# borangundogan/PPO-2DGrid

Measured on AMD Instinct MI355X. Metric: env-steps/sec (rollout+GAE+PPO update), 4096 envs, 16x16 mediumhard, higher is better.
Workload: dtype fp32

## Files before the change

include/merlin_hip.h:

```cpp
#ifndef MERLIN_HIP_H
#define MERLIN_HIP_H

#include <stdint.h>

#ifdef __cplusplus
extern "C" {
#endif

#define MERLIN_ABI_VERSION 3

#define MERLIN_OK 0
#define MERLIN_E_INVALID 1
#define MERLIN_E_HIP 2
#define MERLIN_E_DEVICE 3
#define MERLIN_E_UNSUPPORTED 4

#define MERLIN_EASY 0
#define MERLIN_MEDIUM 1
#define MERLIN_MEDIUMHARD 2
#define MERLIN_HARD 3
#define MERLIN_HARDEST 4

#define MERLIN_DEVERR_BAD_ACTION 1u
#define MERLIN_DEVERR_PLACE_OBJ 2u
// ... 114 lines not shown
int merlin_tower_conv2_lut_fwd(const uint32_t *codes_dev, const int64_t *index_dev, int64_t n,
                               const float *tables_dev, int32_t towers, float *Z2_dev,
                               void *stream);
int merlin_tower_conv2_lut_bwd(const uint32_t *codes_dev, int64_t n, const float *dZ2c_dev,
                               const uint32_t *absmax_dev, int32_t towers, float *dtables_dev,
                               void *stream);
int merlin_tower_conv2_lut_fwd_grouped(const uint32_t *codes_dev, int64_t n, int64_t group_frames,
                                       const float *tables_dev, int32_t towers, float *Z2_dev, void *stream);
int64_t merlin_tower_conv2_lut_slab_bytes(int32_t towers, int64_t group_frames);
int merlin_tower_conv2_lut_bwd_grouped(const uint32_t *codes_dev, int64_t group_frames, const float *dZ2c_dev,
                                       const uint32_t *absmax_dev, int32_t towers, float *dtables_dev,
                                       void *slabs_dev, void *stream);

int merlin_tower_window_lut(const int32_t *rows_dev, int64_t n_windows, const float *tables_dev,
                            int32_t towers, float *Z2w_dev, void *stream);
int merlin_minibatch_patch_maps(const int32_t *kid_dev, const int64_t *group_keys_dev, int64_t n_groups,
                                int64_t n_frames, const int64_t *group_offsets_dev, int32_t n_patches, int32_t *kmap_dev,
                                int32_t *rmap_dev, int32_t *rep_row_dev, void *stream);
int merlin_tower_window_lut_bias_relu(const int32_t *rows_dev, int64_t n_windows, const float *tables_dev,
                                      int32_t towers, const float *b2_dev, float *a2w_dev, void *stream);
int merlin_tower_window_conv3(const float *Q_dev, int64_t n_windows, const int32_t *wid_dev,
                              const int64_t *groups_dev, int64_t n, const float *b3_dev,
                              int32_t towers, float *Y3_dev, void *stream);
int64_t merlin_tower_all_windows(void);
int merlin_tower_codes_conv3(const uint32_t *codes_dev, int64_t n, const float *Qall_dev,
                             const float *b3_dev, int32_t towers, float *Y3_dev, void *stream);
int merlin_tower_codes_conv3_amax(const uint32_t *codes_dev, int64_t n, const float *Qall_dev,
                                  const float *b3_dev, int32_t towers, float *Y3_dev, uint32_t *amax_dev,
                                  void *stream);
int merlin_tower_errors(uint32_t *flags, void *stream);
int merlin_tower_window_conv3_bits(const float *Q_dev, int64_t n_windows, const int32_t *wid_dev,
                                   const int64_t *groups_dev, int64_t n, const float *b3_dev,
                                   int32_t towers, float *Y3_dev, uint64_t *relu_bits_dev, uint32_t *amax_dev,
                                   void *stream);
int merlin_tower_window_conv3_reuse(const float *Q_dev, int64_t n_windows, const int32_t *wid_dev,
                                    const int64_t *groups_dev, int64_t n, const float *b3_dev,
                                    int32_t towers, float *Y3_dev, uint64_t *relu_bits_dev, uint32_t *amax_dev,
                                    const int32_t *rep_row_dev, int32_t copy, void *stream);
int merlin_tower_window_conv3_planes(const float *Q_dev, int64_t nw, const int32_t *wid_dev, const int64_t *groups_dev,
                                     int64_t n, const float *b3_dev, int32_t towers, void *Y3_planes_dev,
                                     uint64_t *relu_bits_dev, const int32_t *rep_row_dev, uint32_t *colmax_ws_dev,
                                     uint32_t *bound_dev, void *stream);
int merlin_segment_sum(const float *src_dev, int64_t src_rows, const int32_t *idx_dev,
                       const int32_t *key_dev, int64_t nnz, const int32_t *slot_dev, int32_t sub,
                       int64_t item_len, const int32_t *fix_dev, int64_t n_fix, int32_t towers,
                       float *out_dev, int64_t out_rows, float *carry_dev, int32_t accumulate,
                       void *stream);
#define MERLIN_SEG_ACCUMULATE 1
#define MERLIN_SEG_NO_FILL 2
#define MERLIN_SEG_MASK_BITS 4
#define MERLIN_SEG_ROLE_SHIFT 8
#define MERLIN_SEG_ROLE_MASK (7 << MERLIN_SEG_ROLE_SHIFT)
int merlin_segment_sum_masked(const float *src_dev, const void *mask_dev, int64_t src_rows,
                              const int32_t *idx_dev, const int32_t *key_dev, int64_t nnz,
                              const int32_t *slot_dev, int32_t sub, int64_t item_len,
                              const int32_t *fix_dev, int64_t n_fix, int32_t towers, float *out_dev,
                              int64_t out_rows, float *carry_dev, int32_t flags, void *stream);
int merlin_segment_sum_marked(const float *src_dev, const void *mask_dev, int64_t src_rows,
                              const int32_t *idx_dev, const int32_t *key_dev, int64_t nnz,
                              const int32_t *slot_dev, int32_t sub, int64_t item_len,
                              const int32_t *fix_dev, int64_t n_fix, int32_t towers, float *out_dev,
                              int64_t out_rows, float *carry_dev, int32_t flags, int32_t *mark_dev,
                              void *stream);
int merlin_segment_sum_fused(const float *src_dev, const void *mask_dev, int64_t src_rows,
                             const int32_t *idx_dev, const int32_t *key_dev, int64_t nnz,
                             const int32_t *slot_dev, int32_t sub, int64_t item_len,
                             const int32_t *fix_dev, int64_t n_fix, int32_t towers, float *out_dev,
                             int64_t out_rows, float *carry_dev, int32_t flags, int32_t *mark_dev,
                             const int32_t *head_fix_dev, int32_t *counters_dev, void *stream);
int merlin_segment_sum_mask_rows(const float *src_dev, const void *mask_dev, int64_t src_rows, const int32_t *idx_dev,
                                 const int32_t *key_dev, int64_t nnz, const int32_t *slot_dev, int32_t sub,
                                 int64_t item_len, const int32_t *fix_dev, int64_t n_fix, int32_t towers, float *out_dev,
                                 int64_t out_rows, float *carry_dev, int32_t flags, int32_t *mark_dev,
                                 const int32_t *head_fix_dev, int32_t *counters_dev, const int32_t *mask_rows_dev,
                                 void *stream);

int merlin_act_heads(const float *z_dev, const float *b4_dev, int64_t n, int32_t hidden,
                     const float *w_actor_dev, const float *b_actor_dev, const float *w_critic_dev,
                     const float *b_critic_dev, int32_t act_dim, int32_t deterministic, uint64_t seed,
                     const int64_t *epoch_dev, int64_t step, int64_t env_offset, int64_t *action_dev,
                     float *logp_dev,
                     float *value_dev, void *stream);

int64_t merlin_ppo_loss_workspace(int64_t n_samples);
int merlin_ppo_loss(const float *logits_dev, const float *value_dev, const float *bias_actor_dev,
                    const float *bias_critic_dev, int64_t n_frames, int32_t act_dim, const int32_t *offs_dev,
                    const int32_t *order_dev, const int64_t *frame_of_dev, int64_t n_samples,
                    const int64_t *sample_index_dev, const int64_t *actions_dev, const float *logp_old_dev,
                    const float *adv_dev, const float *ret_dev, double clip_eps, double vf_coef, double ent_coef,
                    float *dlogits_dev, float *dvalue_dev, float *dbias_actor_dev, float *dbias_critic_dev,
                    float *loss_dev, double *stats_dev, double *workspace_dev, void *stream);
int merlin_ppo_loss_absmax(const float *logits_dev, const float *value_dev, const float *bias_actor_dev,
                           const float *bias_critic_dev, int64_t n_frames, int32_t act_dim, const int32_t *offs_dev,
                           const int32_t *order_dev, const int64_t *frame_of_dev, int64_t n_samples,
                           const int64_t *sample_index_dev, const int64_t *actions_dev, const float *logp_old_dev,
                           const float *adv_dev, const float *ret_dev, double clip_eps, double vf_coef,
                           double ent_coef, float *dlogits_dev, float *dvalue_dev, float *dbias_actor_dev,
                           float *dbias_critic_dev, float *loss_dev, double *stats_dev, double *workspace_dev,
                           uint32_t *grad_absmax_dev, void *stream);

int merlin_tower_bias_relu(float *z_dev, const float *bias_dev, int64_t rows, int32_t cols, int32_t towers,
                           void *stream);
int merlin_tower_relu_bwd(const float *y_dev, const float *dy_dev, float *dz_dev, int64_t rows, int32_t cols,
                          int32_t towers, float *dbias_dev, void *stream);
int merlin_tower_colsum(const float *x_dev, int64_t rows, int32_t cols, int64_t row_stride, int64_t tower_stride,
                        int32_t towers, float *out_dev, void *stream);
int merlin_tower_head_bwd(const float *h_dev, const float *dlogits_dev, const float *dvalue_dev,
                          const float *w_actor_dev, const float *w_critic_dev, int64_t n, int32_t hidden,
                          int32_t act_dim, float *dz_dev, float *dbias_dev, float *dw_actor_dev,
                          float *dw_critic_dev, uint32_t *amax_dev, void *stream);
int merlin_tower_head_bwd_planes(const float *h_dev, const float *dlogits_dev, const float *dvalue_dev,
                                 const float *w_actor_dev, const float *w_critic_dev, int64_t n, int32_t hidden,
                                 int32_t act_dim, void *dz_planes_dev, float *dbias_dev, float *dw_actor_dev,
                                 float *dw_critic_dev, const uint32_t *grad_absmax_dev, uint32_t *dz_bound_dev,
                                 void *stream);
int merlin_tower_heads_fwd(const float *h_dev, int64_t n, int32_t hidden, const float *w_actor_dev,
                           int32_t act_dim, const float *w_critic_dev, const float *b_actor_dev,
                           const float *b_critic_dev, float *logits_dev, float *value_dev, void *stream);

int merlin_x6_split(const float *x_dev, int64_t n, void *planes_dev, void *stream);
int merlin_x6_join(const void *planes_dev, int64_t n, float *x_dev, void *stream);
int merlin_x6_gemm_nt(const float *A_dev, const void *B_dev, int64_t M, int32_t N, int32_t K, int32_t towers,
                      int64_t a_stride, int64_t b_stride, const float *bias_dev, float *C_dev, int64_t c_stride,
                      int32_t cfg, void *stream);
int64_t merlin_x6_tn_slab_floats(int32_t M, int32_t N, int32_t towers, int32_t splits);
int merlin_x6_gemm_tn(const float *A_dev, const float *B_dev, int64_t Kd, int32_t M, int32_t N, int32_t towers,
                      int64_t a_stride, int64_t b_stride, int32_t splits, float *slab_dev, float *out_dev, int32_t cfg,
                      void *stream);

int merlin_h3_amax(const float *x_dev, int64_t n, int32_t towers, int64_t stride, uint32_t *amax_dev, void *stream);
int merlin_h3_split(const float *x_dev, int64_t n, int32_t towers, const uint32_t *amax_dev, void *planes_dev,
                    void *stream);
int merlin_h3_gemm_nt(const float *A_dev, const uint32_t *amax_a_dev, const void *B_dev, const uint32_t *amax_b_dev,
                      int64_t M, int32_t N, int32_t K, int32_t towers, int64_t a_stride, int64_t b_stride,
                      const float *bias_dev, float *C_dev, int64_t c_stride, void *a_planes_dev, int32_t cfg,
                      void *stream);
int merlin_h3_gemm_tn(const float *A_dev, const uint32_t *amax_a_dev, const float *B_dev, const uint32_t *amax_b_dev,
                      int64_t Kd, int32_t M, int32_t N, int32_t towers, int64_t a_stride, int64_t b_stride,
                      int32_t splits, float *slab_dev, float *out_dev, int32_t cfg, void *stream);
int merlin_h3_gemm_tn_planes(const void *A_planes_dev, const uint32_t *amax_a_dev, const void *B_planes_dev,
                             const uint32_t *amax_b_dev, int64_t Kd, int32_t M, int32_t N, int32_t towers,
                             int64_t a_stride, int64_t b_stride, int32_t splits, float *slab_dev, float *out_dev,
                             int32_t cfg, void *stream);
int merlin_h3_gemm_nt_gather(const float *A_dev, const uint32_t *amax_a_dev, const void *B_dev,
                             const uint32_t *amax_b_dev, int64_t M, int32_t N, int32_t K, int32_t towers,
                             int64_t a_stride, int64_t b_stride, const float *bias_dev, float *C_dev, int64_t c_stride,
                             const int32_t *a_rows_dev, int32_t cfg, void *stream);
int merlin_h3_gemm_nt_heads(const float *A_dev, const uint32_t *amax_a_dev, const void *B_dev,
                            const uint32_t *amax_b_dev, int64_t M, int32_t N, int32_t K, int64_t a_stride,
                            int64_t b_stride, const float *bias_dev, float *C_dev, int64_t c_stride,
                            const int32_t *a_rows_dev, const float *head_w0_dev, int32_t n_actions,
                            const float *head_w1_dev, float *head_partials_dev, int32_t cfg, void *stream);
int32_t merlin_h3_heads_parts(int32_t N, int32_t cfg);
int merlin_h3_gemm_nt_planes(const void *A_planes_dev, const uint32_t *amax_a_dev, const void *B_dev,
                             const uint32_t *amax_b_dev, int64_t M, int32_t N, int32_t K, int32_t towers,
                             int64_t a_stride, int64_t b_stride, const float *bias_dev, float *C_dev, int64_t c_stride,
                             int32_t cfg, void *stream);
int merlin_h3_gemm_nt_heads_planes(const void *A_planes_dev, const uint32_t *amax_a_dev, const void *B_dev,
                                   const uint32_t *amax_b_dev, int64_t M, int32_t N, int32_t K, int64_t a_stride,
                                   int64_t b_stride, const float *bias_dev, float *C_dev, int64_t c_stride,
                                   const int32_t *a_rows_dev, const float *head_w0_dev, int32_t n_actions,
                                   const float *head_w1_dev, float *head_partials_dev, int32_t cfg, void *stream);
int merlin_h3_gemm_tn_gather_planes(const void *A_planes_dev, const uint32_t *amax_a_dev, const void *B_planes_dev,
                                    const uint32_t *amax_b_dev, int64_t Kd, int32_t M, int32_t N, int32_t towers,
                                    int64_t a_stride, int64_t b_stride, int32_t splits, float *slab_dev,
                                    float *out_dev, const int32_t *b_rows_dev, int32_t cfg, void *stream);
int merlin_h3_gemm_tn_gather_planes_a(const void *A_planes_dev, const uint32_t *amax_a_dev, const float *B_dev,
                                      const uint32_t *amax_b_dev, int64_t Kd, int32_t M, int32_t N, int32_t towers,
                                      int64_t a_stride, int64_t b_stride, int32_t splits, float *slab_dev,
                                      float *out_dev, const int32_t *b_rows_dev, int32_t cfg, void *stream);
int merlin_act_draw(const float *partials_dev, int32_t parts, int64_t n, const float *b_actor_dev,
                    const float *b_critic_dev, int32_t n_actions, int32_t deterministic, uint64_t seed,
                    const int64_t *epoch_dev, int64_t step, int64_t env_offset, int64_t *action_dev, float *logp_dev,
                    float *value_dev, void *stream);
int merlin_heads_combine(const float *partials_dev, int32_t parts, int64_t M, int32_t n_actions, float *logits_dev,
                         float *value_dev, void *stream);
int merlin_h3_gemm_tn_gather(const float *A_dev, const uint32_t *amax_a_dev, const float *B_dev,
                             const uint32_t *amax_b_dev, int64_t Kd, int32_t M, int32_t N, int32_t towers,
                             int64_t a_stride, int64_t b_stride, int32_t splits, float *slab_dev, float *out_dev,
                             const int32_t *b_rows_dev, int32_t cfg, void *stream);

int merlin_window_gemm_fwd(const float *a2w_dev, const float *W3r_dev, int32_t towers, int64_t nw, float *Q_dev,
                           void *stream);
int64_t merlin_window_gemm_bwd_work(int32_t towers, int64_t nw);
int merlin_window_gemm_bwd(const float *a2w_dev, const float *dQ_dev, const float *W3r_dev, int32_t towers, int64_t nw,
                           float *da2w_dev, float *db2_dev, float *dW3r_dev, float *db3_dev, float *work_dev,
                           int64_t work_floats, void *stream);
int merlin_stage_tables_fwd(const float *W1_dev, const float *b1_dev, const float *W2_dev, const float *atlas_dev,
                            const int16_t *idx_dev, int32_t towers, float *HT_dev, float *T2_dev, void *stream);
int merlin_stage_tables_bwd(const float *W2_dev, const float *HT_dev, const float *dT2_dev, const float *atlas_dev,
                            const int16_t *koff_dev, const int16_t *kv_dev, int32_t towers, float *dH_dev,
                            float *dW1_dev, float *db1_dev, float *dW2_dev, void *stream);

int64_t merlin_clip_adam_workspace(int32_t n_tensors, const int64_t *numel);
int merlin_clip_adam(int32_t n_tensors, float *const *params, float *const *grads, float *const *exp_avg,
                     float *const *exp_avg_sq, float *const *steps, const int64_t *numel, double lr, double beta1,
                     double beta2, double eps, float max_norm, float *norm_out, double *workspace, void *stream);

int64_t merlin_group_clip_sgd_workspace(int32_t n_tensors, const int64_t *numel, int32_t G);
int merlin_group_clip_sgd(int32_t n_tensors, float *const *params, float *const *grads, const int64_t *numel,
                          int32_t G, float lr, float max_norm, float *norm_out, double *workspace, void *stream);

int merlin_episode_loss(const float *reward_dev, const float *value_dev, const float *new_logp_dev,
                        const float *new_value_dev, const int32_t *length_dev, int32_t T, int32_t n, double gamma,
                        double lam, float *workspace_dev, float *loss_dev, void *stream);

int merlin_episode_class_stats(const float *done_dev, const double *ep_return_dev, const int32_t *ep_length_dev,
                               const uint8_t *class_dev, int32_t T, int32_t N, int32_t n_classes,
                               double *out_dev, int32_t accumulate, void *stream);

#ifdef __cplusplus
}
#endif
#endif
```

ppo-2dgrid_amd/csrc/merlin_capi.hip:

```cpp
#include <math.h>
#include <string.h>

#include <mutex>
#include <string>
#include <vector>

#include <algorithm>

#include "merlin_internal.h"

struct merlin_env {
    merlin::EnvDev dev;
    int device;
    bool has_state;
    int steps_since_refill;
    int refill_every;
    bool no_fallback = false;
    bool seed_slots_full = false;
    uint8_t *diff_buf = nullptr;
};

namespace {

thread_local std::string g_err;
// ... 1111 lines not shown
    return MERLIN_OK;
}

int merlin_tower_heads_fwd(const float *h, int64_t n, int32_t hidden, const float *w_actor, int32_t act_dim,
                           const float *w_critic, const float *b_actor, const float *b_critic, float *logits,
                           float *value, void *stream) {
    if ((!h || !w_actor || !w_critic || !logits || !value) && n > 0) return fail(MERLIN_E_INVALID, "null argument");
    if (n < 0) return fail(MERLIN_E_INVALID, "n must be >= 0");
    if (act_dim < 1 || act_dim > merlin::epilogue_max_act()) return fail(MERLIN_E_UNSUPPORTED, "act_dim must be 1..8");
    if (hidden != 512) return fail(MERLIN_E_UNSUPPORTED, "hidden must be 512");
    HIP_TRY(merlin::launch_heads_fwd(h, n, hidden, w_actor, act_dim, w_critic, b_actor, b_critic, logits, value,
                                     (hipStream_t)stream));
    return MERLIN_OK;
}

int merlin_x6_split(const float *x, int64_t n, void *planes, void *stream) {
    if ((!x || !planes) && n > 0) return fail(MERLIN_E_INVALID, "null argument");
    if (n < 0 || n % 8) return fail(MERLIN_E_INVALID, "n must be a non-negative multiple of 8");
    HIP_TRY(merlin::launch_x6_split(x, n, planes, (hipStream_t)stream));
    return MERLIN_OK;
}

int merlin_stage_tables_fwd(const float *W1, const float *b1, const float *W2, const float *atlas, const int16_t *idx,
                            int32_t towers, float *HT, float *T2, void *stream) {
    if (!W1 || !b1 || !W2 || !atlas || !idx || !HT || !T2) return fail(MERLIN_E_INVALID, "null argument");
    if (towers < 1 || towers > 2) return fail(MERLIN_E_INVALID, "towers must be 1 or 2");
    HIP_TRY(merlin::launch_stage_fwd(W1, b1, W2, atlas, idx, towers, HT, T2, (hipStream_t)stream));
    return MERLIN_OK;
}

int merlin_stage_tables_bwd(const float *W2, const float *HT, const float *dT2, const float *atlas,
                            const int16_t *koff, const int16_t *kv, int32_t towers, float *dH, float *dW1, float *db1,
                            float *dW2, void *stream) {
    if (!W2 || !HT || !dT2 || !atlas || !koff || !kv || !dH || !dW1 || !db1 || !dW2)
        return fail(MERLIN_E_INVALID, "null argument");
    if (towers < 1 || towers > 2) return fail(MERLIN_E_INVALID, "towers must be 1 or 2");
    DeviceWs *ws = nullptr;
    int rc = device_ws(&ws);
    if (rc != MERLIN_OK) return rc;
    HIP_TRY(merlin::launch_stage_bwd(W2, HT, dT2, atlas, koff, kv, towers, dH, dW1, db1, dW2, ws->stage_part,
                                     (hipStream_t)stream));
    return MERLIN_OK;
}

int merlin_window_gemm_fwd(const float *a2w, const float *W3r, int32_t towers, int64_t nw, float *Q, void *stream) {
    if (!a2w || !W3r || !Q) return fail(MERLIN_E_INVALID, "null argument");
    if (towers < 1 || towers > 2) return fail(MERLIN_E_INVALID, "towers must be 1 or 2");
    if (nw < 0) return fail(MERLIN_E_INVALID, "nw must be >= 0");
    HIP_TRY(merlin::launch_winfwd(a2w, W3r, towers, nw, Q, (hipStream_t)stream));
    return MERLIN_OK;
}

int64_t merlin_window_gemm_bwd_work(int32_t towers, int64_t nw) {
    if (towers < 1 || towers > 2 || nw <= 0) return -1;
    return merlin::winbwd_work_floats(towers, nw);
}

int merlin_window_gemm_bwd(const float *a2w, const float *dQ, const float *W3r, int32_t towers, int64_t nw,
                           float *da2w, float *db2, float *dW3r, float *db3, float *work, int64_t work_floats,
                           void *stream) {
    if (!a2w || !dQ || !W3r || !da2w || !db2 || !dW3r || !work) return fail(MERLIN_E_INVALID, "null argument");
    if (towers < 1 || towers > 2) return fail(MERLIN_E_INVALID, "towers must be 1 or 2");
    if (nw <= 0) return fail(MERLIN_E_INVALID, "nw must be > 0");
    if (work_floats < merlin::winbwd_work_floats(towers, nw)) return fail(MERLIN_E_INVALID, "work too small");
    HIP_TRY(merlin::launch_winbwd(a2w, dQ, W3r, towers, nw, da2w, db2, dW3r, work, (hipStream_t)stream, db3));
    return MERLIN_OK;
}

int merlin_x6_join(const void *planes, int64_t n, float *x, void *stream) {
    if ((!x || !planes) && n > 0) return fail(MERLIN_E_INVALID, "null argument");
    if (n < 0 || n % 8) return fail(MERLIN_E_INVALID, "n must be a non-negative multiple of 8");
    HIP_TRY(merlin::launch_x6_join(planes, n, x, (hipStream_t)stream));
    return MERLIN_OK;
}

int merlin_x6_gemm_nt(const float *A, const void *B, int64_t M, int32_t N, int32_t K, int32_t towers, int64_t a_stride,
                      int64_t b_stride, const float *bias, float *C, int64_t c_stride, int32_t cfg, void *stream) {
    if (M < 0 || N <= 0 || K <= 0) return fail(MERLIN_E_INVALID, "bad shape");
    if (M > 0 && (!A || !B || !C)) return fail(MERLIN_E_INVALID, "null argument");
    if (K % 32) return fail(MERLIN_E_UNSUPPORTED, "K must be a multiple of 32");
    if (towers < 1 || towers > 2) return fail(MERLIN_E_INVALID, "towers must be 1 or 2");
    if (a_stride % 4 || b_stride % 8) return fail(MERLIN_E_INVALID, "tower strides: A multiple of 4, B of 8");
    const hipError_t e = merlin::launch_x6_gemm_nt(A, B, M, N, K, towers, a_stride, b_stride, bias, C, c_stride, cfg,
                                                   (hipStream_t)stream);
    if (e == hipErrorInvalidValue) return fail(MERLIN_E_UNSUPPORTED, "N not a multiple of the tile width / bad cfg");
    HIP_TRY(e);
    return MERLIN_OK;
}

int64_t merlin_x6_tn_slab_floats(int32_t M, int32_t N, int32_t towers, int32_t splits) {
    return (int64_t)std::max(1, splits) * towers * M * N;
}

int merlin_x6_gemm_tn(const float *A, const float *B, int64_t Kd, int32_t M, int32_t N, int32_t towers, int64_t a_stride,
                      int64_t b_stride, int32_t splits, float *slab, float *out, int32_t cfg, void *stream) {
    if (Kd < 0 || M <= 0 || N <= 0) return fail(MERLIN_E_INVALID, "bad shape");
    if (!out || (Kd > 0 && (!A || !B || !slab))) return fail(MERLIN_E_INVALID, "null argument");
    if (towers < 1 || towers > 2) return fail(MERLIN_E_INVALID, "towers must be 1 or 2");
    if (splits < 1 || splits > merlin::x6_tn_max_splits()) return fail(MERLIN_E_INVALID, "splits out of range");
    if (M % 8 || N % 8 || a_stride % 4 || b_stride % 4) return fail(MERLIN_E_INVALID, "M, N: multiples of 8");
    const hipError_t e = merlin::launch_x6_gemm_tn(A, B, Kd, M, N, towers, a_stride, b_stride, splits, slab, out, cfg,
                                                   (hipStream_t)stream);
    if (e == hipErrorInvalidValue) return fail(MERLIN_E_UNSUPPORTED, "M / N not multiples of the tile / bad cfg");
    HIP_TRY(e);
    return MERLIN_OK;
}

int merlin_h3_amax(const float *x, int64_t n, int32_t towers, int64_t stride, uint32_t *amax, void *stream) {
    if (!amax || (n > 0 && !x)) return fail(MERLIN_E_INVALID, "null argument");
    if (towers < 1 || (n > 0 && towers > 2) || towers > (1 << 20))
        return fail(MERLIN_E_INVALID, "towers must be 1 or 2");
    if (n < 0 || n % 4 || stride % 4 || (towers > 1 && stride < n)) return fail(MERLIN_E_INVALID, "n, stride: multiples of 4");
    HIP_TRY(merlin::launch_h3_amax(x, n, towers, stride, amax, (hipStream_t)stream));
    return MERLIN_OK;
}

int merlin_h3_split(const float *x, int64_t n, int32_t towers, const uint32_t *amax, void *planes, void *stream) {
    if ((!x || !planes || !amax) && n > 0) return fail(MERLIN_E_INVALID, "null argument");
    if (towers < 1 || towers > 2) return fail(MERLIN_E_INVALID, "towers must be 1 or 2");
    if (n < 0 || n % 8) return fail(MERLIN_E_INVALID, "n must be a non-negative multiple of 8");
    HIP_TRY(merlin::launch_h3_split(x, n, towers, amax, planes, (hipStream_t)stream));
    return MERLIN_OK;
}

static int h3_gemm_nt(const float *A, const uint32_t *amax_a, const void *B, const uint32_t *amax_b, int64_t M,
                      int32_t N, int32_t K, int32_t towers, int64_t a_stride, int64_t b_stride, const float *bias,
                      float *C, int64_t c_stride, void *a_planes, const int32_t *a_rows, int32_t cfg, void *stream,
                      const float *head_w0 = nullptr, int32_t n_actions = 0, const float *head_w1 = nullptr,
                      float *head_part = nullptr, bool a_is_planes = false) {
    if (M < 0 || N <= 0 || K <= 0) return fail(MERLIN_E_INVALID, "bad shape");
    if (M > 0 && (!A || !B || (!C && !head_part) || !amax_a || !amax_b)) return fail(MERLIN_E_INVALID, "null argument");
    if (K % 32) return fail(MERLIN_E_UNSUPPORTED, "K must be a multiple of 32");
    if (towers < 1 || towers > 2) return fail(MERLIN_E_INVALID, "towers must be 1 or 2");
    if (a_stride % 4 || b_stride % 8) return fail(MERLIN_E_INVALID, "tower strides: A multiple of 4, B of 8");
    const hipError_t e = merlin::launch_h3_gemm_nt(A, amax_a, B, amax_b, M, N, K, towers, a_stride, b_stride, bias, C,
                                                   c_stride, a_planes, cfg, (hipStream_t)stream, a_rows, head_w0,
                                                   n_actions, head_w1, head_part, a_is_planes);
    if (e == hipErrorInvalidValue)
        return fail(MERLIN_E_UNSUPPORTED, "N not a multiple of the tile width / bad cfg / unsupported gather");
    HIP_TRY(e);
    return MERLIN_OK;
}

int merlin_h3_gemm_nt(const float *A, const uint32_t *amax_a, const void *B, const uint32_t *amax_b, int64_t M,
                      int32_t N, int32_t K, int32_t towers, int64_t a_stride, int64_t b_stride, const float *bias,
                      float *C, int64_t c_stride, void *a_planes, int32_t cfg, void *stream) {
    return h3_gemm_nt(A, amax_a, B, amax_b, M, N, K, towers, a_stride, b_stride, bias, C, c_stride, a_planes, nullptr,
                      cfg, stream);
}

int merlin_h3_gemm_nt_planes(const void *A_planes, const uint32_t *amax_a, const void *B, const uint32_t *amax_b,
                             int64_t M, int32_t N, int32_t K, int32_t towers, int64_t a_stride, int64_t b_stride,
                             const float *bias, float *C, int64_t c_stride, int32_t cfg, void *stream) {
    if (cfg < 60 || cfg >= 70) return fail(MERLIN_E_UNSUPPORTED, "plane-operand cfgs are 60..69");
    return h3_gemm_nt(static_cast<const float *>(A_planes), amax_a, B, amax_b, M, N, K, towers, a_stride, b_stride,
                      bias, C, c_stride, nullptr, nullptr, cfg, stream);
}

int merlin_h3_gemm_nt_gather(const float *A, const uint32_t *amax_a, const void *B, const uint32_t *amax_b, int64_t M,
                             int32_t N, int32_t K, int32_t towers, int64_t a_stride, int64_t b_stride,
                             const float *bias, float *C, int64_t c_stride, const int32_t *a_rows, int32_t cfg,
                             void *stream) {
    if (M > 0 && !a_rows) return fail(MERLIN_E_INVALID, "null argument");
    if (K % 64) return fail(MERLIN_E_UNSUPPORTED, "gathered rows: K must be a multiple of 64");
    return h3_gemm_nt(A, amax_a, B, amax_b, M, N, K, towers, a_stride, b_stride, bias, C, c_stride, nullptr, a_rows,
                      cfg, stream);
}

static int h3_gemm_tn(const void *A, const uint32_t *amax_a, const void *B, const uint32_t *amax_b, int64_t Kd,
                      int32_t M, int32_t N, int32_t towers, int64_t a_stride, int64_t b_stride, int32_t splits,
                      float *slab, float *out, bool planes, int32_t cfg, void *stream, const int32_t *b_rows = nullptr,
                      bool a_planes = false, bool b_planes = false) {
    if (Kd < 0 || M <= 0 || N <= 0) return fail(MERLIN_E_INVALID, "bad shape");
    if (!out || (Kd > 0 && (!A || !B || !slab || !amax_a || !amax_b))) return fail(MERLIN_E_INVALID, "null argument");
    if (towers < 1 || towers > 2) return fail(MERLIN_E_INVALID, "towers must be 1 or 2");
    if (splits < 1 || splits > merlin::x6_tn_max_splits()) return fail(MERLIN_E_INVALID, "splits out of range");
    if (M % 8 || N % 8 || a_stride % 4 || b_stride % 4) return fail(MERLIN_E_INVALID, "M, N: multiples of 8");
    const hipError_t e = merlin::launch_h3_gemm_tn(A, amax_a, B, amax_b, Kd, M, N, towers, a_stride, b_stride, splits,
                                                   slab, out, planes, cfg, (hipStream_t)stream, b_rows, a_planes,
                                                   b_planes);
    if (e == hipErrorInvalidValue) return fail(MERLIN_E_UNSUPPORTED, "M / N not multiples of the tile / bad cfg");
    HIP_TRY(e);
    return MERLIN_OK;
}

int merlin_h3_gemm_tn(const float *A, const uint32_t *amax_a, const float *B, const uint32_t *amax_b, int64_t Kd,
                      int32_t M, int32_t N, int32_t towers, int64_t a_stride, int64_t b_stride, int32_t splits,
                      float *slab, float *out, int32_t cfg, void *stream) {
    return h3_gemm_tn(A, amax_a, B, amax_b, Kd, M, N, towers, a_stride, b_stride, splits, slab, out, false, cfg,
                      stream);
}

int merlin_h3_gemm_nt_heads(const float *A, const uint32_t *amax_a, const void *B, const uint32_t *amax_b, int64_t M,
                            int32_t N, int32_t K, int64_t a_stride, int64_t b_stride, const float *bias, float *C,
                            int64_t c_stride, const int32_t *a_rows, const float *head_w0, int32_t n_actions,
                            const float *head_w1, float *head_partials, int32_t cfg, void *stream) {
    if (M > 0 && (!bias || !head_w0 || !head_w1 || !head_partials)) return fail(MERLIN_E_INVALID, "null argument");
    if (n_actions < 1 || n_actions > 4) return fail(MERLIN_E_UNSUPPORTED, "heads epilogue: 1..4 actions");
    if (merlin::h3_heads_parts(N, cfg) == 0) return fail(MERLIN_E_UNSUPPORTED, "heads epilogue: cfg 10, 12 or 13");
    if (a_rows && K % 64) return fail(MERLIN_E_UNSUPPORTED, "gathered rows: K must be a multiple of 64");
    return h3_gemm_nt(A, amax_a, B, amax_b, M, N, K, 2, a_stride, b_stride, bias, C, c_stride, nullptr, a_rows, cfg,
                      stream, head_w0, n_actions, head_w1, head_partials);
}

int32_t merlin_h3_heads_parts(int32_t N, int32_t cfg) { return merlin::h3_heads_parts(N, cfg); }

int merlin_act_draw(const float *partials, int32_t parts, int64_t n, const float *b_actor, const float *b_critic,
                    int32_t n_actions, int32_t deterministic, uint64_t seed, const int64_t *epoch, int64_t step,
                    int64_t env_offset, int64_t *action, float *logp, float *value, void *stream) {
    if (n < 0 || parts < 1 || n_actions < 1 || n_actions > 4) return fail(MERLIN_E_INVALID, "bad shape");
    if (n > 0 && (!partials || !b_actor || !b_critic || !action || !logp || !value))
        return fail(MERLIN_E_INVALID, "null argument");
    HIP_TRY(merlin::launch_act_draw(partials, parts, n, b_actor, b_critic, n_actions, deterministic, seed, epoch, step,
                                    env_offset, action, logp, value, (hipStream_t)stream));
    return MERLIN_OK;
}

int merlin_heads_combine(const float *partials, int32_t parts, int64_t M, int32_t n_actions, float *logits,
                         float *value, void *stream) {
    if (M < 0 || parts < 1 || n_actions < 1 || n_actions > 4) return fail(MERLIN_E_INVALID, "bad shape");
    if (M > 0 && (!partials || !logits || !value)) return fail(MERLIN_E_INVALID, "null argument");
    HIP_TRY(merlin::launch_heads_combine(partials, parts, M, n_actions, logits, value, (hipStream_t)stream));
    return MERLIN_OK;
}

int merlin_h3_gemm_tn_gather(const float *A, const uint32_t *amax_a, const float *B, const uint32_t *amax_b, int64_t Kd,
                             int32_t M, int32_t N, int32_t towers, int64_t a_stride, int64_t b_stride, int32_t splits,
                             float *slab, float *out, const int32_t *b_rows, int32_t cfg, void *stream) {
    if (Kd > 0 && !b_rows) return fail(MERLIN_E_INVALID, "null argument");
    if (N % 64) return fail(MERLIN_E_UNSUPPORTED, "gathered rows: N must be a multiple of 64");
    return h3_gemm_tn(A, amax_a, B, amax_b, Kd, M, N, towers, a_stride, b_stride, splits, slab, out, false, cfg, stream,
                      b_rows);
}

int merlin_h3_gemm_nt_heads_planes(const void *A_planes, const uint32_t *amax_a, const void *B,
                                   const uint32_t *amax_b, int64_t M, int32_t N, int32_t K, int64_t a_stride,
                                   int64_t b_stride, const float *bias, float *C, int64_t c_stride,
                                   const int32_t *a_rows, const float *head_w0, int32_t n_actions,
                                   const float *head_w1, float *head_partials, int32_t cfg, void *stream) {
    if (M > 0 && (!bias || !C || !a_rows || (head_partials && (!head_w0 || !head_w1))))
        return fail(MERLIN_E_INVALID, "null argument");
    if (head_partials && (n_actions < 1 || n_actions > 4))
        return fail(MERLIN_E_UNSUPPORTED, "heads epilogue: 1..4 actions");
    if (merlin::h3_heads_parts(N, cfg) == 0) return fail(MERLIN_E_UNSUPPORTED, "planes forward: cfg 10, 12 or 13");
    if (K % 64) return fail(MERLIN_E_UNSUPPORTED, "gathered rows: K must be a multiple of 64");
    return h3_gemm_nt(static_cast<const float *>(A_planes), amax_a, B, amax_b, M, N, K, 2, a_stride, b_stride, bias,
                      C, c_stride, nullptr, a_rows, cfg, stream, head_w0, n_actions, head_w1, head_partials, true);
}

int merlin_h3_gemm_tn_gather_planes(const void *A_planes, const uint32_t *amax_a, const void *B_planes,
                                    const uint32_t *amax_b, int64_t Kd, int32_t M, int32_t N, int32_t towers,
                                    int64_t a_stride, int64_t b_stride, int32_t splits, float *slab, float *out,
                                    const int32_t *b_rows, int32_t cfg, void *stream) {
    if (Kd > 0 && !b_rows) return fail(MERLIN_E_INVALID, "null argument");
    if (N % 64) return fail(MERLIN_E_UNSUPPORTED, "gathered rows: N must be a multiple of 64");
    return h3_gemm_tn(A_planes, amax_a, B_planes, amax_b, Kd, M, N, towers, a_stride, b_stride, splits, slab, out,
                      false, cfg, stream, b_rows, true, true);
}

int merlin_h3_gemm_tn_gather_planes_a(const void *A_planes, const uint32_t *amax_a, const float *B,
                                      const uint32_t *amax_b, int64_t Kd, int32_t M, int32_t N, int32_t towers,
                                      int64_t a_stride, int64_t b_stride, int32_t splits, float *slab, float *out,
                                      const int32_t *b_rows, int32_t cfg, void *stream) {
    if (Kd > 0 && !b_rows) return fail(MERLIN_E_INVALID, "null argument");
    if (N % 64) return fail(MERLIN_E_UNSUPPORTED, "gathered rows: N must be a multiple of 64");
    return h3_gemm_tn(A_planes, amax_a, B, amax_b, Kd, M, N, towers, a_stride, b_stride, splits, slab, out, false, cfg,
                      stream, b_rows, true);
}

int merlin_h3_gemm_tn_planes(const void *A, const uint32_t *amax_a, const void *B, const uint32_t *amax_b, int64_t Kd,
                             int32_t M, int32_t N, int32_t towers, int64_t a_stride, int64_t b_stride, int32_t splits,
                             float *slab, float *out, int32_t cfg, void *stream) {
    return h3_gemm_tn(A, amax_a, B, amax_b, Kd, M, N, towers, a_stride, b_stride, splits, slab, out, true, cfg,
                      stream);
}

int64_t merlin_clip_adam_workspace(int32_t n_tensors, const int64_t *numel) {
    if (n_tensors < 0 || n_tensors > merlin::OPT_MAX_TENSORS || (n_tensors > 0 && !numel)) return -1;
    return std::max<int64_t>(1, merlin::opt_blocks(n_tensors, numel));
}

int merlin_clip_adam(int32_t n_tensors, float *const *params, float *const *grads, float *const *exp_avg,
                     float *const *exp_avg_sq, float *const *steps, const int64_t *numel, double lr, double beta1,
                     double beta2, double eps, float max_norm, float *norm_out, double *workspace, void *stream) {
    if (n_tensors < 1 || n_tensors > merlin::OPT_MAX_TENSORS)
        return fail(MERLIN_E_INVALID, "n_tensors must be in [1, 32]");
    if (!params || !grads || !exp_avg || !exp_avg_sq || !steps || !numel || !workspace)
        return fail(MERLIN_E_INVALID, "null argument");
    int64_t blocks = 0;
    for (int i = 0; i < n_tensors; i++) {
        if (numel[i] <= 0) return fail(MERLIN_E_INVALID, "every tensor needs numel > 0");
        if (!params[i] || !grads[i] || !exp_avg[i] || !exp_avg_sq[i] || !steps[i])
            return fail(MERLIN_E_INVALID, "null tensor pointer");
    }
    blocks = merlin::opt_blocks(n_tensors, numel);
    if (blocks > INT32_MAX / 2) return fail(MERLIN_E_INVALID, "too many elements");
    HIP_TRY(merlin::launch_clip_adam(n_tensors, params, grads, exp_avg, exp_avg_sq, steps, numel, lr, beta1, beta2, eps,
                                     max_norm, norm_out, workspace, (hipStream_t)stream));
    return MERLIN_OK;
}

int64_t merlin_group_clip_sgd_workspace(int32_t n_tensors, const int64_t *numel, int32_t G) {
    if (n_tensors < 0 || n_tensors > merlin::OPT_MAX_TENSORS || G < 0 || (n_tensors > 0 && !numel)) return -1;
    for (int i = 0; i < n_tensors; i++)
        if (numel[i] <= 0) return -1;
    return std::max<int64_t>(1, merlin::group_blocks(n_tensors, numel) * (int64_t)G);
}

int merlin_group_clip_sgd(int32_t n_tensors, float *const *params, float *const *grads, const int64_t *numel,
                          int32_t G, float lr, float max_norm, float *norm_out, double *workspace, void *stream) {
    if (n_tensors < 0 || n_tensors > merlin::OPT_MAX_TENSORS)
        return fail(MERLIN_E_INVALID, "n_tensors must be in [0, 32]");
    if (G < 0 || G > 65535) return fail(MERLIN_E_INVALID, "G must be in [0, 65535]");
    if (n_tensors == 0 || G == 0) return MERLIN_OK;
    if (!params || !grads || !numel || !workspace) return fail(MERLIN_E_INVALID, "null argument");
    for (int i = 0; i < n_tensors; i++) {
        if (numel[i] <= 0) return fail(MERLIN_E_INVALID, "every tensor needs numel > 0");
        if (!params[i] || !grads[i]) return fail(MERLIN_E_INVALID, "null tensor pointer");
    }
    if (merlin::group_blocks(n_tensors, numel) > INT32_MAX / 2) return fail(MERLIN_E_INVALID, "too many elements");
    HIP_TRY(merlin::launch_group_clip_sgd(n_tensors, params, grads, numel, G, lr, max_norm, norm_out, workspace,
                                          (hipStream_t)stream));
    return MERLIN_OK;
}

int merlin_episode_loss(const float *reward, const float *value, const float *new_logp, const float *new_value,
                        const int32_t *length, int32_t T, int32_t n, double gamma, double lam, float *workspace,
                        float *loss, void *stream) {
    if (T < 1 || n < 0) return fail(MERLIN_E_INVALID, "episode_loss needs T >= 1 and n >= 0");
    if (n == 0) return MERLIN_OK;
    if (!reward || !value || !new_logp || !new_value || !length || !workspace || !loss)
        return fail(MERLIN_E_INVALID, "null argument");
    HIP_TRY(merlin::launch_episode_loss(reward, value, new_logp, new_value, length, T, n, gamma, lam, workspace, loss,
                                        (hipStream_t)stream));
    return MERLIN_OK;
}

int merlin_episode_class_stats(const float *done, const double *ep_return, const int32_t *ep_length,
                               const uint8_t *cls, int32_t T, int32_t N, int32_t n_classes, double *out,
                               int32_t accumulate, void *stream) {
    if (T < 0 || N < 0) return fail(MERLIN_E_INVALID, "episode_class_stats needs T >= 0 and N >= 0");
    if (n_classes < 1 || n_classes > merlin::EPS_MAX_CLASSES)
        return fail(MERLIN_E_INVALID, "episode_class_stats needs n_classes in [1, 8]");
    if (!out) return fail(MERLIN_E_INVALID, "null argument");
    if (T > 0 && N > 0 && (!done || !ep_return || !ep_length || !cls)) return fail(MERLIN_E_INVALID, "null argument");
    DeviceWs *ws = nullptr;
    int rc = device_ws(&ws);
    if (rc) return rc;
    HIP_TRY(merlin::launch_episode_class_stats(done, ep_return, ep_length, cls, T, N, n_classes, out, accumulate,
                                               ws->eps_part, (hipStream_t)stream));
    return MERLIN_OK;
}

}
```

ppo-2dgrid_amd/csrc/merlin_h3.hip:

```cpp
#include <algorithm>

#include "merlin_internal.h"

namespace merlin {
namespace {

typedef _Float16 f16x8 __attribute__((ext_vector_type(8)));
typedef _Float16 f16x2 __attribute__((ext_vector_type(2)));
typedef __bf16 bf16x4 __attribute__((ext_vector_type(4)));
typedef __bf16 bf16x8 __attribute__((ext_vector_type(8)));
typedef float f32x16 __attribute__((ext_vector_type(16)));
typedef uint32_t u32x4 __attribute__((ext_vector_type(4)));
typedef __attribute__((address_space(3))) bf16x4 lds_bf16x4;
typedef __attribute__((address_space(3))) char lds_char;

constexpr int BK = 32;
constexpr float LO_INV = 1.0f / 2048.0f;

__device__ __forceinline__ f32x16 mfma16(const u32x4 a, const u32x4 b, f32x16 c) {
    return __builtin_amdgcn_mfma_f32_32x32x16_f16(__builtin_bit_cast(f16x8, a), __builtin_bit_cast(f16x8, b), c, 0, 0,
                                                   0);
}

__device__ __forceinline__ float relu_nan(float v) { return v != v ? v : fmaxf(v, 0.0f); }
// ... 1295 lines not shown
    if (hd.part) {
        if constexpr (!PIPE || BN / WGN != 64) {
            return hipErrorInvalidValue;
        } else {
            if (!bias || T != 2 || Pout || hd.na < 1 || hd.na > 4 || !hd.w0 || !hd.w1) return hipErrorInvalidValue;
            if (amap) {
                if (K % 64 || K > 64 * GA_CHUNKS || !C) return hipErrorInvalidValue;
                hipLaunchKernelGGL((k_h3_ntpg<BM, BN, WGM, WGN, 2>), grid, block, 0, s, A, B, amaxA, amaxB, M, N, K,
                                   sA, sB, bias, C, sC, tiles_n, amap, hd);
            } else if (C) {
                hipLaunchKernelGGL((k_h3_ntp<BM, BN, WGM, WGN, 2>), grid, block, 0, s, A, B, amaxA, amaxB, M, N, K, sA,
                                   sB, bias, C, sC, tiles_n, nullptr, hd);
            } else {
                hipLaunchKernelGGL((k_h3_ntp<BM, BN, WGM, WGN, 3>), grid, block, 0, s, A, B, amaxA, amaxB, M, N, K, sA,
                                   sB, bias, nullptr, sC, tiles_n, nullptr, hd);
            }
            return hipGetLastError();
        }
    }
    if (amap) {
        if (!PIPE || Pout || K % 64 || K > 64 * GA_CHUNKS) return hipErrorInvalidValue;
        if (bias)
            hipLaunchKernelGGL((k_h3_ntpg<BM, BN, WGM, WGN, 1>), grid, block, 0, s, A, B, amaxA, amaxB, M, N, K, sA,
                               sB, bias, C, sC, tiles_n, amap, hd);
        else
            hipLaunchKernelGGL((k_h3_ntpg<BM, BN, WGM, WGN, 0>), grid, block, 0, s, A, B, amaxA, amaxB, M, N, K, sA,
                               sB, nullptr, C, sC, tiles_n, amap, hd);
        return hipGetLastError();
    }
    if (PIPE) {
        if (bias)
            hipLaunchKernelGGL((k_h3_ntp<BM, BN, WGM, WGN, 1>), grid, block, 0, s, A, B, amaxA, amaxB, M, N, K, sA, sB,
                               bias, C, sC, tiles_n, Pout, hd);
        else
            hipLaunchKernelGGL((k_h3_ntp<BM, BN, WGM, WGN, 0>), grid, block, 0, s, A, B, amaxA, amaxB, M, N, K, sA, sB,
                               nullptr, C, sC, tiles_n, Pout, hd);
    } else {
        if (bias)
            hipLaunchKernelGGL((k_h3_nt<BM, BN, WGM, WGN, 1>), grid, block, 0, s, A, B, amaxA, amaxB, M, N, K, sA, sB,
                               bias, C, sC, tiles_n, Pout);
        else
            hipLaunchKernelGGL((k_h3_nt<BM, BN, WGM, WGN, 0>), grid, block, 0, s, A, B, amaxA, amaxB, M, N, K, sA, sB,
                               nullptr, C, sC, tiles_n, Pout);
    }
    return hipGetLastError();
}

template <int BM, int BN, int WGM, int WGN, bool KP>
hipError_t ntg_launch(const float *A, const u32x4 *B, const uint32_t *amaxA, const uint32_t *amaxB, int64_t M, int N,
                      int K, int T, int64_t sA, int64_t sB, const float *bias, float *C, int64_t sC, u32x4 *Pout,
                      hipStream_t s) {
    if (N % BN || Pout) return hipErrorInvalidValue;
    if ((int64_t)N * (K / 8) * 2 > INT32_MAX) return hipErrorInvalidValue;
    const int64_t tiles_m = (M + BM - 1) / BM;
    const int tiles_n = N / BN;
    if (tiles_m * tiles_n > INT32_MAX) return hipErrorInvalidValue;
    const dim3 grid((unsigned)(tiles_m * tiles_n), T), block(64 * WGM * WGN);
    if (bias)
        hipLaunchKernelGGL((k_h3_ntg<BM, BN, WGM, WGN, 1, KP>), grid, block, 0, s, A, B, amaxA, amaxB, M, N, K, sA, sB,
                           bias, C, sC, tiles_n);
    else
        hipLaunchKernelGGL((k_h3_ntg<BM, BN, WGM, WGN, 0, KP>), grid, block, 0, s, A, B, amaxA, amaxB, M, N, K, sA, sB,
                           nullptr, C, sC, tiles_n);
    return hipGetLastError();
}

template <int BM, int BN, int WGM, int WGN, int Q>
hipError_t tn_launch(const void *A, const void *B, const uint32_t *amaxA, const uint32_t *amaxB, int64_t Kd, int M,
                     int N, int T, int64_t sA, int64_t sB, int splits, float *slab, int *S_out, const int32_t *bmap,
                     hipStream_t s) {
    if (M % BM || N % BN) return hipErrorInvalidValue;
    if (bmap && ((Q != 0 && Q != 3 && Q != 4) || N % 64)) return hipErrorInvalidValue;
    if (Q >= 3 && !bmap) return hipErrorInvalidValue;
    const int tiles_n = N / BN, tiles = (M / BM) * tiles_n;
    int S = std::max(1, splits);
    int64_t kc = (Kd + S - 1) / S;
    kc = (kc + BK - 1) / BK * BK;
    S = (int)std::max<int64_t>(1, (Kd + kc - 1) / kc);
    *S_out = S;
    if (Q == 1)
        hipLaunchKernelGGL((k_h3_tnq<BM, BN, WGM, WGN>), dim3(tiles * S * T), dim3(64 * WGM * WGN), 0, s,
                           static_cast<const u32x4 *>(A), static_cast<const u32x4 *>(B), amaxA, amaxB, Kd, M, N,
                           sA / 4, sB / 4, kc, tiles_n, tiles, S, slab);
    else if (Q == 2)
        hipLaunchKernelGGL((k_h3_tnp<BM, BN, WGM, WGN>), dim3(tiles * S * T), dim3(64 * WGM * WGN), 0, s,
                           static_cast<const float4 *>(A), static_cast<const float4 *>(B), amaxA, amaxB, Kd, M, N,
                           sA / 4, sB / 4, kc, tiles_n, tiles, S, slab);
    else if (Q == 4)
        hipLaunchKernelGGL((k_h3_tng<BM, BN, WGM, WGN, true, true>), dim3(tiles * S * T), dim3(64 * WGM * WGN), 0, s,
                           static_cast<const float4 *>(A), static_cast<const float4 *>(B), amaxA, amaxB, Kd, M, N,
                           sA / 4, sB / 4, kc, tiles_n, tiles, S, slab, bmap);
    else if (Q == 3)
        hipLaunchKernelGGL((k_h3_tng<BM, BN, WGM, WGN, true>), dim3(tiles * S * T), dim3(64 * WGM * WGN), 0, s,
                           static_cast<const float4 *>(A), static_cast<const float4 *>(B), amaxA, amaxB, Kd, M, N,
                           sA / 4, sB / 4, kc, tiles_n, tiles, S, slab, bmap);
    else if (bmap)
        hipLaunchKernelGGL((k_h3_tng<BM, BN, WGM, WGN>), dim3(tiles * S * T), dim3(64 * WGM * WGN), 0, s,
                           static_cast<const float4 *>(A), static_cast<const float4 *>(B), amaxA, amaxB, Kd, M, N,
                           sA / 4, sB / 4, kc, tiles_n, tiles, S, slab, bmap);
    else
        hipLaunchKernelGGL((k_h3_tn<BM, BN, WGM, WGN>), dim3(tiles * S * T), dim3(64 * WGM * WGN), 0, s,
                           static_cast<const float4 *>(A), static_cast<const float4 *>(B), amaxA, amaxB, Kd, M, N,
                           sA / 4, sB / 4, kc, tiles_n, tiles, S, slab);
    return hipGetLastError();
}

__global__ void k_h3_fill0(float4 *__restrict__ out, int64_t n4) {
    for (int64_t e = (int64_t)blockIdx.x * 256 + threadIdx.x; e < n4; e += (int64_t)gridDim.x * 256)
        out[e] = make_float4(0.0f, 0.0f, 0.0f, 0.0f);
}

}

hipError_t launch_h3_amax(const float *x, int64_t n, int T, int64_t stride, uint32_t *amax, hipStream_t s) {
    hipLaunchKernelGGL(k_h3_zero, dim3((T + 63) / 64), dim3(64), 0, s, amax, T);
    hipError_t e = hipGetLastError();
    if (e != hipSuccess || n <= 0) return e;
    if (n % 4 || stride % 4) return hipErrorInvalidValue;
    const int64_t n4 = n / 4;
    const int grid = (int)std::min<int64_t>((n4 + 255) / 256, 1024);
    hipLaunchKernelGGL(k_h3_amax, dim3(grid, T), dim3(256), 0, s, reinterpret_cast<const float4 *>(x), n4, stride / 4,
                       amax);
    return hipGetLastError();
}

hipError_t launch_h3_split(const float *x, int64_t n, int T, const uint32_t *amax, void *planes, hipStream_t s) {
    if (n % 8) return hipErrorInvalidValue;
    if (n <= 0) return hipSuccess;
    const int64_t g8 = n / 8;
    const int grid = (int)std::min<int64_t>((g8 + 255) / 256, 2048);
    hipLaunchKernelGGL(k_h3_split, dim3(grid, T), dim3(256), 0, s, reinterpret_cast<const float4 *>(x), g8, amax,
                       static_cast<u32x4 *>(planes));
    return hipGetLastError();
}

hipError_t launch_h3_gemm_nt(const float *A, const uint32_t *amaxA, const void *B, const uint32_t *amaxB, int64_t M,
                             int N, int K, int T, int64_t a_stride, int64_t b_stride, const float *bias, float *C,
                             int64_t c_stride, void *a_planes, int cfg, hipStream_t s, const int32_t *a_rows,
                             const float *head_w0, int n_actions, const float *head_w1, float *head_part,
                             bool a_is_planes) {
    const HeadsArg hd{head_w0, head_w1, n_actions, head_part};
    if (M <= 0) return hipSuccess;
    if (K % BK || N <= 0 || a_stride % 4 || b_stride % 8) return hipErrorInvalidValue;
    const u32x4 *b = static_cast<const u32x4 *>(B);
    u32x4 *P = static_cast<u32x4 *>(a_planes);
    const int64_t sB = b_stride / 8 * 2;
#define H3_NT(BM, BN, WM, WN, PIPE) \
    nt_launch<BM, BN, WM, WN, PIPE>(A, b, amaxA, amaxB, M, N, K, T, a_stride, sB, bias, C, c_stride, P, a_rows, hd, s, \
                                    a_is_planes)
#define H3_NTG(BM, BN, WM, WN, KP)                         \
    ((a_rows || head_part) ? hipErrorInvalidValue          \
                           : ntg_launch<BM, BN, WM, WN, KP>(A, b, amaxA, amaxB, M, N, K, T, a_stride, sB, bias, C, \
                                                            c_stride, P, s))
    if (a_is_planes && (cfg < 10 || cfg > 14) && cfg != 60) return hipErrorInvalidValue;
    if (cfg >= 60 && cfg < 70) {
        if (P || ((a_rows || head_part) && !a_is_planes)) return hipErrorInvalidValue;
        return launch_h3p_gemm_nt(A, amaxA, B, amaxB, M, N, K, T, a_stride, b_stride, bias, C, c_stride, cfg, s, a_rows,
                                  head_w0, n_actions, head_w1, head_part);
    }
    switch (cfg) {
        case 0: return H3_NT(256, 128, 4, 2, false);
        case 1: return H3_NT(128, 192, 4, 2, false);
        case 2: return H3_NT(128, 128, 2, 2, false);
        case 3: return H3_NT(128, 256, 2, 4, false);
        case 5: return H3_NT(128, 64, 4, 1, false);
        case 10: return H3_NT(256, 128, 4, 2, true);
        case 11: return H3_NT(128, 192, 4, 2, true);
        case 12: return H3_NT(128, 128, 2, 2, true);
        case 13: return H3_NT(128, 256, 2, 4, true);
        case 14: return H3_NT(64, 128, 2, 2, true);
        case 20: return H3_NTG(256, 128, 4, 2, false);
        case 21: return H3_NTG(128, 192, 4, 2, false);
        case 30: return H3_NTG(256, 128, 4, 2, true);
        case 31: return H3_NTG(128, 192, 4, 2, true);
        default: return hipErrorInvalidValue;
    }
#undef H3_NT
#undef H3_NTG
}

hipError_t launch_h3_gemm_tn(const void *A, const uint32_t *amaxA, const void *B, const uint32_t *amaxB, int64_t Kd,
                             int M, int N, int T, int64_t a_stride, int64_t b_stride, int splits, float *slab,
                             float *out, bool planes, int cfg, hipStream_t s, const int32_t *b_rows, bool a_planes,
                             bool b_planes) {
    if (b_planes && !a_planes) return hipErrorInvalidValue;
    if (M <= 0 || N <= 0) return hipSuccess;
    if (M % 8 || N % 8 || a_stride % 4 || b_stride % 4) return hipErrorInvalidValue;
    const int64_t total = (int64_t)T * M * N;
    if (Kd <= 0) {
        hipLaunchKernelGGL(k_h3_fill0, dim3((unsigned)std::min<int64_t>((total / 4 + 255) / 256, 2048)), dim3(256),
                           0, s, reinterpret_cast<float4 *>(out), total / 4);
        return hipGetLastError();
    }
    int S = 1;
    hipError_t e;
    if (cfg == 20 || cfg == 21) {
        if (!(a_planes && b_planes)) return hipErrorInvalidValue;
        e = launch_h3p_gemm_tn_gather(A, amaxA, B, amaxB, Kd, M, N, T, a_stride, b_stride, splits, slab, b_rows, cfg,
                                      &S, s);
        if (e != hipSuccess) return e;
        return launch_x6_fold(slab, S, total, out, s);
    }
#define H3_TN(BM, BN, WM, WN, PIPE)                                                                              \
    (planes ? tn_launch<BM, BN, WM, WN, 1>(A, B, amaxA, amaxB, Kd, M, N, T, a_stride, b_stride, splits, slab, &S,   \
                                           b_rows, s)                                                              \
     : a_planes ? (b_planes ? tn_launch<BM, BN, WM, WN, 4>(A, B, amaxA, amaxB, Kd, M, N, T, a_stride, b_stride,    \
                                                           splits, slab, &S, b_rows, s)                            \
                           : tn_launch<BM, BN, WM, WN, 3>(A, B, amaxA, amaxB, Kd, M, N, T, a_stride, b_stride,    \
                                                          splits, slab, &S, b_rows, s))                            \
            : tn_launch<BM, BN, WM, WN, PIPE>(A, B, amaxA, amaxB, Kd, M, N, T, a_stride, b_stride, splits, slab, &S, \
                                              b_rows, s))
    switch (cfg) {
        case 0: e = H3_TN(128, 192, 4, 2, 0); break;
        case 1: e = H3_TN(128, 192, 2, 2, 0); break;
        case 2: e = H3_TN(64, 192, 2, 2, 0); break;
        case 10: e = H3_TN(128, 192, 4, 2, 2); break;
        case 11: e = H3_TN(128, 192, 2, 2, 2); break;
        default: return hipErrorInvalidValue;
    }
#undef H3_TN
    if (e != hipSuccess) return e;
    return launch_x6_fold(slab, S, total, out, s);
}

namespace {
__global__ __launch_bounds__(256) void k_heads_combine(const float4 *__restrict__ part, int P, int64_t M, int na,
                                                       float *__restrict__ logits, float *__restrict__ value) {
    const int64_t r = (int64_t)blockIdx.x * 256 + threadIdx.x;
    if (r >= M) return;
    float4 a = part[r], v = part[(int64_t)P * M + r];
    for (int p = 1; p < P; p++) {
        const float4 x = part[(int64_t)p * M + r], y = part[(int64_t)(P + p) * M + r];
        a.x += x.x;
        a.y += x.y;
        a.z += x.z;
        a.w += x.w;
        v.x += y.x;
    }
    const float av[4] = {a.x, a.y, a.z, a.w};
    for (int o = 0; o < na; o++) logits[r * na + o] = av[o];
    value[r] = v.x;
}
}

int h3_heads_parts(int N, int cfg) {
    switch (cfg) {
        case 10: return N % 128 ? 0 : N / 128 * 2;
        case 12: return N % 128 ? 0 : N / 128 * 2;
        case 13: return N % 256 ? 0 : N / 256 * 4;
        case 14: return N % 128 ? 0 : N / 128 * 2;
        case 60: return N % 256 ? 0 : N / 256 * 4;
        default: return 0;
    }
}

hipError_t launch_heads_combine(const float *part, int P, int64_t M, int na, float *logits, float *value,
                                hipStream_t s) {
    if (M <= 0) return hipSuccess;
    if (P < 1 || na < 1 || na > 4) return hipErrorInvalidValue;
    hipLaunchKernelGGL(k_heads_combine, dim3((unsigned)((M + 255) / 256)), dim3(256), 0, s,
                       reinterpret_cast<const float4 *>(part), P, M, na, logits, value);
    return hipGetLastError();
}

}
```

ppo-2dgrid_amd/csrc/merlin_h3p.hip:

```cpp
#include <algorithm>
#include <type_traits>

#include "merlin_internal.h"

namespace merlin {
namespace {

typedef _Float16 p_f16x8 __attribute__((ext_vector_type(8)));
typedef float p_f32x16 __attribute__((ext_vector_type(16)));
typedef uint32_t p_u32x4 __attribute__((ext_vector_type(4)));

constexpr float P_LO_INV = 1.0f / 2048.0f;

__device__ __forceinline__ p_f32x16 p_mfma(const p_u32x4 a, const p_u32x4 b, p_f32x16 c) {
    return __builtin_amdgcn_mfma_f32_32x32x16_f16(__builtin_bit_cast(p_f16x8, a), __builtin_bit_cast(p_f16x8, b), c, 0,
                                                   0, 0);
}
__device__ __forceinline__ float p_relu(float v) { return v != v ? v : fmaxf(v, 0.0f); }
__device__ __forceinline__ int p_xcd_tile(int b, int nb) {
    const int xcd = b & 7, q = nb >> 3, r = nb & 7;
    return (xcd < r ? xcd * (q + 1) : r * (q + 1) + (xcd - r) * q) + (b >> 3);
}
__device__ __forceinline__ int p_exp(uint32_t amax) {
    if (amax == 0u) return 0;
    const int e = (int)((amax >> 23) & 0xffu) - 127;
    return std::min(std::max(14 - e, -120), 115);
}
__device__ __forceinline__ float p_pow2(int e) { return __uint_as_float((uint32_t)(e + 127) << 23); }
__device__ __forceinline__ uint32_t p_amax(const uint32_t *p) {
    return __hip_atomic_load(p, __ATOMIC_RELAXED, __HIP_MEMORY_SCOPE_AGENT);
}
__device__ __forceinline__ int p_swz(int r) { return (r >> 1) & 7; }
__device__ __forceinline__ p_u32x4 p_unscale(const p_u32x4 x) {
    return __builtin_bit_cast(p_u32x4, __builtin_bit_cast(p_f16x8, x) * (_Float16)(1.0f / 2048.0f));
}

template <int V>
using IC = std::integral_constant<int, V>;
template <int N, int I = 0, class F>
__device__ __forceinline__ void static_for(F &&f) {
    if constexpr (I < N) {
        f(IC<I>{});
        static_for<N, I + 1>(f);
    }
}

typedef __attribute__((address_space(3))) p_u32x4 lds_u32x4;
__device__ __forceinline__ void lds_rd(p_u32x4 &d, uint32_t addr) { d = *(const lds_u32x4 *)(uintptr_t)addr; }

template <int BM, int BN, int WGM, int WGN, int EPI, int NK, int NS = 3, bool ONE = false, int ORD = 0>
__global__ __launch_bounds__(64 * WGM * WGN) void k_h3_pq(const p_u32x4 *__restrict__ A, const p_u32x4 *__restrict__ B,
                                                          const uint32_t *__restrict__ amaxA,
                                                          const uint32_t *__restrict__ amaxB, int64_t M, int N, int K,
                                                          int64_t sA, int64_t sB, const float *__restrict__ bias,
                                                          float *__restrict__ C, int64_t sC, int tiles_n) {
    constexpr int NT = 64 * WGM * WGN;
    constexpr int WTM = BM / WGM, WTN = BN / WGN;
    constexpr int TM = WTM / 32, TN = WTN / 32;
    constexpr int NR = 2 * (TM + TN), NM = 3 * TM * TN;
    static_assert(NM >= NR, "a read behind every MFMA");
    constexpr int G = (BM + BN) * 8 / NT;
    static_assert((BM * 8) % NT == 0 && (BN * 8) % NT == 0, "whole DMA instructions per thread");
    constexpr int STG = (BM + BN) * 8;
    constexpr uint32_t STG_B = STG * 16;
    static_assert(NS >= 2 && NS <= 4, "ring depth");
    __shared__ p_u32x4 lds[NS * STG];

    const int t = blockIdx.y;
    const int L = p_xcd_tile(blockIdx.x, gridDim.x);
    const int tm = L / tiles_n, tn = L - tm * tiles_n;
    const int64_t m0 = (int64_t)tm * BM;
    const int n0 = tn * BN;
    const int tid = threadIdx.x, lane = tid & 63, w = tid >> 6;
    const int wm = w / WGN, wn = w - (w / WGN) * WGN;
    const int64_t row_ch = K / 4;

    const int eA = p_exp(p_amax(amaxA + t)), eB = p_exp(p_amax(amaxB + t));
    const p_u32x4 *baseA = A + t * sA + m0 * row_ch, *baseB = B + t * sB + (int64_t)n0 * row_ch;
    uint32_t off[G];
#pragma unroll
    for (int i = 0; i < G; i++) {
        const int q = i * NT + tid, r = q >> 3, c = (q & 7) ^ p_swz(r);
        off[i] = r < BM ? (uint32_t)(std::min<int64_t>(r, M - 1 - m0) * row_ch + c) : (uint32_t)((r - BM) * row_ch + c);
    }
    typedef __attribute__((address_space(3))) void lds_void;
    typedef __attribute__((address_space(1))) void gbl_void;
    auto issue = [&](int kt, int st) __attribute__((always_inline)) {
        p_u32x4 *base = lds + st * STG + w * 64;
#pragma unroll
        for (int i = 0; i < G; i++) {
            const int q0 = i * NT;
            const p_u32x4 *b = (q0 >> 3) < BM ? baseA : baseB;
            __builtin_amdgcn_global_load_lds((gbl_void *)(b + off[i] + kt * 8), (lds_void *)(base + i * NT), 16, 0, 0);
        }
    };

    const int fr = lane & 31, fh = lane >> 5;
    const uint32_t lds0 = (uint32_t)(uintptr_t)(__attribute__((address_space(3))) p_u32x4 *)lds;
    uint32_t adA[2][2], adB[2][2];
    {
        const int ra = wm * WTM + fr, rb = BM + wn * WTN + fr;
#pragma unroll
        for (int kh = 0; kh < 2; kh++)
#pragma unroll
            for (int p = 0; p < 2; p++) {
                const int c = 2 * (2 * kh + fh) + p;
                adA[kh][p] = lds0 + (uint32_t)(ra * 8 + (c ^ p_swz(ra))) * 16u;
                adB[kh][p] = lds0 + (uint32_t)(rb * 8 + (c ^ p_swz(rb))) * 16u;
            }
    }
    struct Frag {
        p_u32x4 a[TM][2], b[TN][2];
    };
    p_f32x16 hi[TM][TN], lo[TM][TN];
#pragma unroll
    for (int i = 0; i < TM; i++)
#pragma unroll
        for (int j = 0; j < TN; j++) {
            hi[i][j] = p_f32x16{};
            lo[i][j] = p_f32x16{};
        }
    auto rd = [&](Frag &g, auto K_, uint32_t so, auto KH) __attribute__((always_inline)) {
        constexpr int k = decltype(K_)::value, kh = decltype(KH)::value;
        if constexpr (k < 2 * TM)
            lds_rd(g.a[k >> 1][k & 1], adA[kh][k & 1] + so + (k >> 1) * 32 * 128);
        else
            lds_rd(g.b[(k - 2 * TM) >> 1][k & 1], adB[kh][k & 1] + so + ((k - 2 * TM) >> 1) * 32 * 128);
    };
    auto mf = [&](const Frag &f, const Frag &u, auto M_) __attribute__((always_inline)) {
        constexpr int m = decltype(M_)::value, tl = ORD ? m % (TM * TN) : m / 3, pr = ORD ? m / (TM * TN) : m % 3;
        constexpr int i = tl / TN, j = tl % TN;
        if constexpr (ONE) {
            if constexpr (pr == 0)
                hi[i][j] = p_mfma(u.a[i][1], f.b[j][0], hi[i][j]);
            else if constexpr (pr == 1)
                hi[i][j] = p_mfma(f.a[i][0], u.b[j][1], hi[i][j]);
            else
                hi[i][j] = p_mfma(f.a[i][0], f.b[j][0], hi[i][j]);
        } else if constexpr (pr == 0)
            lo[i][j] = p_mfma(f.a[i][1], f.b[j][0], lo[i][j]);
        else if constexpr (pr == 1)
            lo[i][j] = p_mfma(f.a[i][0], f.b[j][1], lo[i][j]);
        else
            hi[i][j] = p_mfma(f.a[i][0], f.b[j][0], hi[i][j]);
    };
    auto half = [&](const Frag &f, Frag &g, uint32_t so, auto KH, auto READS) __attribute__((always_inline)) {
        Frag u;
        if constexpr (ONE) {
#pragma unroll
            for (int i = 0; i < TM; i++) u.a[i][1] = p_unscale(f.a[i][1]);
#pragma unroll
            for (int j = 0; j < TN; j++) u.b[j][1] = p_unscale(f.b[j][1]);
        }
        static_for<NM>([&](auto M_) __attribute__((always_inline)) {
            mf(f, u, M_);
            if constexpr (decltype(READS)::value && decltype(M_)::value < NR) rd(g, M_, so, KH);
        });
        if constexpr (decltype(READS)::value) {
            static_for<NR>([&](auto) __attribute__((always_inline)) {
                __builtin_amdgcn_sched_group_barrier(0x008, 1, 0);
                __builtin_amdgcn_sched_group_barrier(0x100, 1, 0);
            });
            if constexpr (NM > NR) __builtin_amdgcn_sched_group_barrier(0x008, NM - NR, 0);
        }
        __builtin_amdgcn_sched_barrier(0);
    };
    auto touch = [&](const Frag &f) __attribute__((always_inline)) {
#pragma unroll
        for (int i = 0; i < TM; i++) asm volatile("" ::"v"(f.a[i][0]), "v"(f.a[i][1]));
#pragma unroll
        for (int j = 0; j < TN; j++) asm volatile("" ::"v"(f.b[j][0]), "v"(f.b[j][1]));
    };

    static_assert(NK >= NS - 1, "the prologue's k steps");
    constexpr int D = NS - 1;
    static_for<D>([&](auto KT) __attribute__((always_inline)) { issue(decltype(KT)::value, decltype(KT)::value); });
    asm volatile("s_waitcnt vmcnt(%0)" ::"n"(G * (D - 1)) : "memory");
    __builtin_amdgcn_s_barrier();
    __builtin_amdgcn_sched_barrier(0);
    Frag f0, f1;
    static_for<NR>([&](auto K_) __attribute__((always_inline)) { rd(f0, K_, 0, IC<0>{}); });
    static_for<NK>([&](auto KT) __attribute__((always_inline)) {
        constexpr int kt = decltype(KT)::value, st = kt % NS, sn = (kt + 1) % NS;
        if constexpr (kt + D < NK) issue(kt + D, (kt + D) % NS);
        __builtin_amdgcn_sched_barrier(0);
        half(f0, f1, (uint32_t)st * STG_B, IC<1>{}, IC<1>{});
        if constexpr (kt + 1 < NK) {
            touch(f1);
            constexpr int later = (NK - 1 < kt + D ? NK - 1 : kt + D) - (kt + 1);
            asm volatile("s_waitcnt vmcnt(%0)" ::"n"(G * later) : "memory");
            __builtin_amdgcn_s_barrier();
            __builtin_amdgcn_sched_barrier(0);
            half(f1, f0, (uint32_t)sn * STG_B, IC<0>{}, IC<1>{});
        } else {
            half(f1, f0, 0u, IC<0>{}, IC<0>{});
        }
    });

    const float inv = p_pow2(-eA), invB = p_pow2(-eB);
    float *Ct = C + t * sC;
#pragma unroll
    for (int j = 0; j < TN; j++) {
        const int col = n0 + wn * WTN + j * 32 + fr;
        const float bv = EPI == 1 ? bias[(int64_t)t * N + col] : 0.0f;
#pragma unroll
        for (int i = 0; i < TM; i++) {
#pragma unroll
            for (int r = 0; r < 16; r++) {
                const int64_t row = m0 + wm * WTM + i * 32 + (r & 3) + 8 * (r >> 2) + 4 * fh;
                if (row < M) {
                    const float v = (ONE ? hi[i][j][r] : hi[i][j][r] + lo[i][j][r] * P_LO_INV) * inv * invB;
                    Ct[row * N + col] = EPI == 1 ? p_relu(v + bv) : v;
                }
            }
        }
    }
}

template <int BM, int BN, int WGM, int WGN, int NS = 3, bool ONE = false, int ORD = 0>
hipError_t pq_launch(const void *A, const void *B, const uint32_t *amaxA, const uint32_t *amaxB, int64_t M, int N,
                     int K, int T, int64_t sA, int64_t sB, const float *bias, float *C, int64_t sC, hipStream_t s) {
    if (N % BN || K % 32 || K < 64) return hipErrorInvalidValue;
    const int64_t tiles_m = (M + BM - 1) / BM;
    const int tiles_n = N / BN;
    if (tiles_m * tiles_n > INT32_MAX) return hipErrorInvalidValue;
    const dim3 grid((unsigned)(tiles_m * tiles_n), T), block(64 * WGM * WGN);
    const auto *a = static_cast<const p_u32x4 *>(A);
    const auto *b = static_cast<const p_u32x4 *>(B);
#define PQ_K(NK)                                                                                                   \
    do {                                                                                                           \
        if (bias)                                                                                                  \
            hipLaunchKernelGGL((k_h3_pq<BM, BN, WGM, WGN, 1, NK, NS, ONE, ORD>), grid, block, 0, s, a, b, amaxA, amaxB, M, N, K, \
                               sA / 4, sB / 4, bias, C, sC, tiles_n);                                              \
        else                                                                                                       \
            hipLaunchKernelGGL((k_h3_pq<BM, BN, WGM, WGN, 0, NK, NS, ONE, ORD>), grid, block, 0, s, a, b, amaxA, amaxB, M, N, K, \
                               sA / 4, sB / 4, nullptr, C, sC, tiles_n);                                           \
    } while (0)
    switch (K) {
        case 576: PQ_K(18); break;
        case 512: PQ_K(16); break;
        default: return hipErrorInvalidValue;
    }
#undef PQ_K
    return hipGetLastError();
}


__device__ uint4 p_zero16[1] = {{0u, 0u, 0u, 0u}};

__device__ __forceinline__ void p_dma16(const void *src, uint32_t lds) {
    uint32_t keep;
    asm volatile("s_mov_b32 %0, m0\n\ts_mov_b32 m0, %2\n\tglobal_load_lds_dwordx4 %1, off\n\ts_mov_b32 m0, %0"
                 : "=&s"(keep)
                 : "v"(src), "s"(lds)
                 : "memory");
}
__device__ __forceinline__ void p_dma4(const void *src, uint32_t lds) {
    uint32_t keep;
    asm volatile("s_mov_b32 %0, m0\n\ts_mov_b32 m0, %2\n\tglobal_load_lds_dword %1, off\n\ts_mov_b32 m0, %0"
                 : "=&s"(keep)
                 : "v"(src), "s"(lds)
                 : "memory");
}

template <int RC>
__device__ __forceinline__ int p_tr_swz(int row) {
    static_assert(RC % 16 == 0 || RC == 24 || RC == 8, "row chunks");
    return RC % 16 == 0 ? (row & 3) << 2 : ((row >> 1) & 1) << 2;
}
typedef __bf16 p_bf16x4 __attribute__((ext_vector_type(4)));
typedef __bf16 p_bf16x8 __attribute__((ext_vector_type(8)));
typedef __attribute__((address_space(3))) p_bf16x4 lds_p_bf16x4;
typedef __attribute__((address_space(3))) int32_t lds_i32;

template <int BM, int BN, int WGM, int WGN>
__global__ __launch_bounds__(64 * WGM * WGN) void k_h3_tq(const p_u32x4 *__restrict__ A, const p_u32x4 *__restrict__ B,
                                                          const uint32_t *__restrict__ amaxA,
                                                          const uint32_t *__restrict__ amaxB, int64_t Kd, int M,
                                                          int N, int64_t sA, int64_t sB, int64_t kc, int tiles_n,
                                                          int tiles, int S, float *__restrict__ slab,
                                                          const int32_t *__restrict__ bmap) {
    constexpr int NT = 64 * WGM * WGN, NW = NT / 64;
    constexpr int WTM = BM / WGM, WTN = BN / WGN;
    constexpr int TM = WTM / 32, TN = WTN / 32;
    constexpr int RCA = BM / 8, RCB = BN / 8;
    constexpr int PSA = 32 * RCA, PSB = 32 * RCB;
    constexpr int STG = 2 * (PSA + PSB);
    constexpr uint32_t STG_B = STG * 16;
    static_assert((2 * PSA) % NT == 0 && (2 * PSB) % NT == 0, "whole DMA instructions per operand");
    constexpr int GA = 2 * PSA / NT, GB = 2 * PSB / NT, G = GA + GB + 1;
    constexpr int JB = BN / 64;
    constexpr int XS = 64 * NW;
    static_assert(32 * JB <= XS, "index slot");
    constexpr int NF = 2 * (TM + TN);
    constexpr int NR = 2 * NF, NM = 3 * TM * TN;
    __shared__ p_u32x4 lds[3 * STG];
    __shared__ int32_t ixr[3 * XS];

    const int P = p_xcd_tile(blockIdx.x, gridDim.x);
    const int t = P / (S * tiles), s = (P / tiles) % S, Lt = P % tiles;
    const int tm = Lt / tiles_n, tn = Lt - tm * tiles_n;
    const int m0 = tm * BM, n0 = tn * BN;
    const int64_t k0 = (int64_t)s * kc, k1 = std::min<int64_t>(Kd, k0 + kc);
    const int eA = p_exp(p_amax(amaxA + t)), eB = p_exp(p_amax(amaxB + t));
    const int tid = threadIdx.x, lane = tid & 63, w = tid >> 6;
    const int wm = w / WGN, wn = w - (w / WGN) * WGN;
    const int nc = N / 64, j0 = n0 / 64;
    const int64_t rowA = M / 4;
    const p_u32x4 *At = A + t * sA, *Bt = B + t * sB;
    const uint32_t lds0 = (uint32_t)(uintptr_t)(__attribute__((address_space(3))) p_u32x4 *)lds;
    const uint32_t ix0 = (uint32_t)(uintptr_t)(__attribute__((address_space(3))) int32_t *)ixr;
    const uint32_t wbase = (uint32_t)__builtin_amdgcn_readfirstlane(w) * 64u;

    int ra[GA], rb[GB], xb[GB];
    uint32_t oa[GA], gp[GB];
#pragma unroll
    for (int i = 0; i < GA; i++) {
        const int q = i * NT + tid, p = q / PSA, rem = q - p * PSA, r = rem / RCA, cs = rem - r * RCA;
        const int c = cs ^ p_tr_swz<RCA>(r);
        ra[i] = r;
        oa[i] = (uint32_t)((m0 / 8 + c) * 2 + p);
    }
#pragma unroll
    for (int i = 0; i < GB; i++) {
        const int q = (GA + i) * NT + tid - 2 * PSA, p = q / PSB, rem = q - p * PSB, r = rem / RCB,
                  cs = rem - r * RCB;
        const int c = cs ^ p_tr_swz<RCB>(r), col = 8 * c;
        rb[i] = r;
        xb[i] = r * JB + (col >> 6);
        gp[i] = (uint32_t)(((col & 63) >> 3) * 2 + p);
    }
    const int xr = tid / JB, xj = j0 + tid % JB;
    const int64_t nk = (k1 - k0 + 31) / 32, nk3 = (nk + 2) / 3 * 3;

    auto issue_ix = [&](int64_t kt, int slot) __attribute__((always_inline)) {
        const int64_t row = std::min<int64_t>(k0 + kt * 32 + (tid < 32 * JB ? xr : 0), k1 - 1);
        p_dma4(bmap + row * nc + (tid < 32 * JB ? xj : j0), ix0 + (uint32_t)(slot * XS) * 4u + wbase * 4u);
    };
    auto read_ix = [&](int slot, int32_t (&x)[GB]) __attribute__((always_inline)) {
        const lds_i32 *xs = (const lds_i32 *)(uintptr_t)(ix0 + (uint32_t)(slot * XS) * 4u);
#pragma unroll
        for (int i = 0; i < GB; i++) x[i] = xs[xb[i]];
    };
    auto issue = [&](int64_t kt, int st, const int32_t (&x)[GB]) __attribute__((always_inline)) {
        const uint32_t base = lds0 + (uint32_t)(st * STG) * 16u + wbase * 16u;
        const int64_t kk = k0 + kt * 32;
        const bool full = kk + 32 <= k1;
#pragma unroll
        for (int i = 0; i < GA; i++) {
            const p_u32x4 *src = full || kk + ra[i] < k1 ? At + (kk + ra[i]) * rowA + oa[i]
                                                          : reinterpret_cast<const p_u32x4 *>(p_zero16);
            p_dma16(src, base + (uint32_t)(i * NT) * 16u);
        }
#pragma unroll
        for (int i = 0; i < GB; i++) {
            const p_u32x4 *src = full || kk + rb[i] < k1 ? Bt + (int64_t)x[i] * 16 + gp[i]
                                                          : reinterpret_cast<const p_u32x4 *>(p_zero16);
            p_dma16(src, base + (uint32_t)((GA + i) * NT) * 16u);
        }
    };

    const int fg = lane >> 4, fq = (lane >> 2) & 3, fp = lane & 3;
    struct Frag {
        p_bf16x4 v[NF][2];
    };
    auto rd = [&](Frag &g, auto K_, uint32_t so, auto KH) __attribute__((always_inline)) {
        constexpr int k = decltype(K_)::value, kh = decltype(KH)::value, f = k >> 1, h2 = k & 1;
        constexpr bool isA = f < 2 * TM;
        constexpr int tile = isA ? f >> 1 : (f - 2 * TM) >> 1, pl = f & 1;
        constexpr int RC = isA ? RCA : RCB;
        const int col0 = isA ? wm * WTM + tile * 32 : wn * WTN + tile * 32;
        const uint32_t img = lds0 + so + (uint32_t)(isA ? pl * PSA : 2 * PSA + pl * PSB) * 16u;
        const int chunk = ((col0 + 16 * (fg & 1)) >> 3) + (fp >> 1);
        const int row = 16 * kh + 8 * (fg >> 1) + 4 * h2 + fq;
        const uint32_t off = img + (uint32_t)((row * RC + (chunk ^ p_tr_swz<RC>(row))) * 16 + (fp & 1) * 8);
        g.v[f][h2] = __builtin_amdgcn_ds_read_tr16_b64_v4bf16((lds_p_bf16x4 *)(uintptr_t)off);
    };
    auto frag = [](const Frag &g, int f) __attribute__((always_inline)) {
        return __builtin_bit_cast(p_u32x4, p_bf16x8{g.v[f][0][0], g.v[f][0][1], g.v[f][0][2], g.v[f][0][3],
                                                   g.v[f][1][0], g.v[f][1][1], g.v[f][1][2], g.v[f][1][3]});
    };
    p_f32x16 hi[TM][TN], lo[TM][TN];
#pragma unroll
    for (int i = 0; i < TM; i++)
#pragma unroll
        for (int j = 0; j < TN; j++) {
            hi[i][j] = p_f32x16{};
            lo[i][j] = p_f32x16{};
        }
    auto mf = [&](const Frag &f, auto M_) __attribute__((always_inline)) {
        constexpr int m = decltype(M_)::value, i = m / (3 * TN), j = (m / 3) % TN, pr = m % 3;
        constexpr int fa0 = 2 * i, fa1 = 2 * i + 1, fb0 = 2 * TM + 2 * j, fb1 = 2 * TM + 2 * j + 1;
        if constexpr (pr == 0)
            lo[i][j] = p_mfma(frag(f, fa1), frag(f, fb0), lo[i][j]);
        else if constexpr (pr == 1)
            lo[i][j] = p_mfma(frag(f, fa0), frag(f, fb1), lo[i][j]);
        else
            hi[i][j] = p_mfma(frag(f, fa0), frag(f, fb0), hi[i][j]);
    };
    constexpr int RPM = (NR + NM - 1) / NM;
    auto half = [&](const Frag &f, Frag &g, uint32_t so, auto KH) __attribute__((always_inline)) {
        static_for<NM>([&](auto M_) __attribute__((always_inline)) {
            mf(f, M_);
            static_for<RPM>([&](auto R_) __attribute__((always_inline)) {
                constexpr int k = decltype(M_)::value * RPM + decltype(R_)::value;
                if constexpr (k < NR) rd(g, IC<k>{}, so, KH);
            });
        });
        static_for<NM>([&](auto M_) __attribute__((always_inline)) {
            constexpr int left = NR - decltype(M_)::value * RPM;
            __builtin_amdgcn_sched_group_barrier(0x008, 1, 0);
            if constexpr (left > 0) __builtin_amdgcn_sched_group_barrier(0x100, left < RPM ? left : RPM, 0);
        });
        __builtin_amdgcn_sched_barrier(0);
    };
    auto touch = [&](const Frag &f) __attribute__((always_inline)) {
#pragma unroll
        for (int q = 0; q < NF; q++) asm volatile("" ::"v"(f.v[q][0]), "v"(f.v[q][1]));
    };
    auto publish = [&](auto CNT) __attribute__((always_inline)) {
        asm volatile("s_waitcnt vmcnt(%0)" ::"n"(decltype(CNT)::value) : "memory");
        __builtin_amdgcn_s_barrier();
        asm volatile("" ::: "memory");
        __builtin_amdgcn_sched_barrier(0);
    };

    int32_t x0[GB], x1[GB], x2[GB];
    issue_ix(0, 0);
    issue_ix(1, 1);
    issue_ix(2, 2);
    publish(IC<0>{});
    read_ix(0, x0);
    read_ix(1, x1);
    read_ix(2, x2);
    issue(0, 0, x0);
    issue(1, 1, x1);
    publish(IC<G - 1>{});
    issue_ix(3, 0);
    Frag f0, f1;
    static_for<NR>([&](auto K_) __attribute__((always_inline)) { rd(f0, K_, 0u, IC<0>{}); });
    auto step = [&](int64_t kt, auto ST, int32_t (&xu)[GB], int32_t (&xn)[GB]) __attribute__((always_inline)) {
        constexpr int st = decltype(ST)::value, sn = (st + 1) % 3, s2 = (st + 2) % 3;
        issue_ix(kt + 4, sn);
        issue(kt + 2, s2, xu);
        __builtin_amdgcn_sched_barrier(0);
        half(f0, f1, (uint32_t)st * STG_B, IC<1>{});
        touch(f1);
        publish(IC<G>{});
        read_ix(st, xn);
        half(f1, f0, (uint32_t)sn * STG_B, IC<0>{});
    };
    for (int64_t kt = 0; kt < nk3; kt += 3) {
        step(kt, IC<0>{}, x2, x0);
        step(kt + 1, IC<1>{}, x0, x1);
        step(kt + 2, IC<2>{}, x1, x2);
    }
    asm volatile("s_waitcnt vmcnt(0)" ::: "memory");

    const float inv = p_pow2(-eA), invB = p_pow2(-eB);
    float *St = slab + ((int64_t)s * (gridDim.x / (S * tiles)) + t) * (int64_t)M * N;
    const int fr = lane & 31, fh = lane >> 5;
#pragma unroll
    for (int i = 0; i < TM; i++)
#pragma unroll
        for (int j = 0; j < TN; j++)
#pragma unroll
            for (int r = 0; r < 16; r++) {
                const int row = m0 + wm * WTM + i * 32 + (r & 3) + 8 * (r >> 2) + 4 * fh;
                St[(int64_t)row * N + n0 + wn * WTN + j * 32 + fr] = (hi[i][j][r] + lo[i][j][r] * P_LO_INV) * inv * invB;
            }
}


template <int BM, int BN, int WGM, int WGN, int EPI>
__global__ __launch_bounds__(64 * WGM * WGN) void k_h3_pqg(const p_u32x4 *__restrict__ A, const p_u32x4 *__restrict__ B,
                                                           const uint32_t *__restrict__ amaxA,
                                                           const uint32_t *__restrict__ amaxB, int64_t M, int N,
                                                           int64_t sA, int64_t sB, const float *__restrict__ bias,
                                                           float *__restrict__ C, int64_t sC, int tiles_n,
                                                           const int32_t *__restrict__ amap,
                                                           const float *__restrict__ hw0, const float *__restrict__ hw1,
                                                           int na, float *__restrict__ hpart) {
    constexpr int K = 576, NK = 18, KC = K / 64;
    constexpr int NT = 64 * WGM * WGN;
    constexpr int WTM = BM / WGM, WTN = BN / WGN;
    constexpr int TM = WTM / 32, TN = WTN / 32;
    constexpr int NR = 2 * (TM + TN), NM = 3 * TM * TN;
    static_assert(NM >= NR, "a read behind every MFMA");
    constexpr int GA = BM * 8 / NT, GB = BN * 8 / NT, G = GA + GB;
    static_assert((BM * 8) % NT == 0 && (BN * 8) % NT == 0, "whole DMA instructions per thread");
    constexpr int STG = (BM + BN) * 8;
    constexpr uint32_t STG_B = STG * 16;
    __shared__ p_u32x4 lds[3 * STG];
    __shared__ int32_t gmap[BM * KC];

    const int t = blockIdx.y;
    const int L = p_xcd_tile(blockIdx.x, gridDim.x);
    const int tm = L / tiles_n, tn = L - tm * tiles_n;
    const int64_t m0 = (int64_t)tm * BM;
    const int n0 = tn * BN;
    const int tid = threadIdx.x, lane = tid & 63, w = tid >> 6;
    const int wm = w / WGN, wn = w - (w / WGN) * WGN;
    const int eA = p_exp(p_amax(amaxA + t)), eB = p_exp(p_amax(amaxB + t));
    for (int e = tid; e < BM * KC; e += NT) {
        const int r = e / KC;
        gmap[e] = amap[std::min<int64_t>(m0 + r, M - 1) * KC + (e - r * KC)];
    }
    __syncthreads();
    const p_u32x4 *At = A + t * sA, *baseB = B + t * sB + (int64_t)n0 * (K / 4);
    int ga[GA];
    uint32_t ca[GA];
    uint32_t offB[GB];
#pragma unroll
    for (int i = 0; i < GA; i++) {
        const int q = i * NT + tid, r = q >> 3;
        ga[i] = r * KC;
        ca[i] = (uint32_t)((q & 7) ^ p_swz(r));
    }
#pragma unroll
    for (int i = 0; i < GB; i++) {
        const int q = i * NT + tid, r = q >> 3;
        offB[i] = (uint32_t)(r * (K / 4) + ((q & 7) ^ p_swz(r)));
    }
    const uint32_t lds0 = (uint32_t)(uintptr_t)(__attribute__((address_space(3))) p_u32x4 *)lds;
    const uint32_t gm0 = (uint32_t)(uintptr_t)(__attribute__((address_space(3))) int32_t *)gmap;
    const uint32_t wbase = (uint32_t)__builtin_amdgcn_readfirstlane(w) * 64u;
    auto read_g = [&](int kt, int32_t (&g)[GA]) __attribute__((always_inline)) {
#pragma unroll
        for (int i = 0; i < GA; i++) g[i] = *(const lds_i32 *)(uintptr_t)(gm0 + (uint32_t)(ga[i] + kt / 2) * 4u);
    };
    auto issue = [&](int kt, int st, const int32_t (&g)[GA]) __attribute__((always_inline)) {
        const uint32_t base = lds0 + (uint32_t)(st * STG) * 16u + wbase * 16u;
#pragma unroll
        for (int i = 0; i < GA; i++)
            p_dma16(At + (int64_t)g[i] * 16 + 8 * (kt & 1) + ca[i], base + (uint32_t)(i * NT) * 16u);
#pragma unroll
        for (int i = 0; i < GB; i++) p_dma16(baseB + offB[i] + kt * 8, base + (uint32_t)((GA + i) * NT) * 16u);
    };

    const int fr = lane & 31, fh = lane >> 5;
    uint32_t adA[2][2], adB[2][2];
    {
        const int ra = wm * WTM + fr, rb = BM + wn * WTN + fr;
#pragma unroll
        for (int kh = 0; kh < 2; kh++)
#pragma unroll
            for (int p = 0; p < 2; p++) {
                const int c = 2 * (2 * kh + fh) + p;
                adA[kh][p] = lds0 + (uint32_t)(ra * 8 + (c ^ p_swz(ra))) * 16u;
                adB[kh][p] = lds0 + (uint32_t)(rb * 8 + (c ^ p_swz(rb))) * 16u;
            }
    }
    struct Frag {
        p_u32x4 a[TM][2], b[TN][2];
    };
    p_f32x16 hi[TM][TN], lo[TM][TN];
#pragma unroll
    for (int i = 0; i < TM; i++)
#pragma unroll
        for (int j = 0; j < TN; j++) {
            hi[i][j] = p_f32x16{};
            lo[i][j] = p_f32x16{};
        }
    auto rd = [&](Frag &g, auto K_, uint32_t so, auto KH) __attribute__((always_inline)) {
        constexpr int k = decltype(K_)::value, kh = decltype(KH)::value;
        if constexpr (k < 2 * TM)
            lds_rd(g.a[k >> 1][k & 1], adA[kh][k & 1] + so + (k >> 1) * 32 * 128);
        else
            lds_rd(g.b[(k - 2 * TM) >> 1][k & 1], adB[kh][k & 1] + so + ((k - 2 * TM) >> 1) * 32 * 128);
    };
    auto mf = [&](const Frag &f, auto M_) __attribute__((always_inline)) {
        constexpr int m = decltype(M_)::value, i = m / (3 * TN), j = (m / 3) % TN, pr = m % 3;
        if constexpr (pr == 0)
            lo[i][j] = p_mfma(f.a[i][1], f.b[j][0], lo[i][j]);
        else if constexpr (pr == 1)
            lo[i][j] = p_mfma(f.a[i][0], f.b[j][1], lo[i][j]);
        else
            hi[i][j] = p_mfma(f.a[i][0], f.b[j][0], hi[i][j]);
    };
    auto half = [&](const Frag &f, Frag &g, uint32_t so, auto KH, auto READS) __attribute__((always_inline)) {
        static_for<NM>([&](auto M_) __attribute__((always_inline)) {
            mf(f, M_);
            if constexpr (decltype(READS)::value && decltype(M_)::value < NR) rd(g, M_, so, KH);
        });
        if constexpr (decltype(READS)::value) {
            static_for<NR>([&](auto) __attribute__((always_inline)) {
                __builtin_amdgcn_sched_group_barrier(0x008, 1, 0);
                __builtin_amdgcn_sched_group_barrier(0x100, 1, 0);
            });
            if constexpr (NM > NR) __builtin_amdgcn_sched_group_barrier(0x008, NM - NR, 0);
        }
        __builtin_amdgcn_sched_barrier(0);
    };
    auto touch = [&](const Frag &f) __attribute__((always_inline)) {
#pragma unroll
        for (int i = 0; i < TM; i++) asm volatile("" ::"v"(f.a[i][0]), "v"(f.a[i][1]));
#pragma unroll
        for (int j = 0; j < TN; j++) asm volatile("" ::"v"(f.b[j][0]), "v"(f.b[j][1]));
    };

    int32_t g0[GA], g1[GA];
    read_g(0, g0);
    issue(0, 0, g0);
    read_g(1, g1);
    issue(1, 1, g1);
    read_g(2, g0);
    asm volatile("s_waitcnt vmcnt(%0)" ::"n"(G) : "memory");
    __builtin_amdgcn_s_barrier();
    asm volatile("" ::: "memory");
    __builtin_amdgcn_sched_barrier(0);
    Frag f0, f1;
    static_for<NR>([&](auto K_) __attribute__((always_inline)) { rd(f0, K_, 0, IC<0>{}); });
    static_for<NK>([&](auto KT) __attribute__((always_inline)) {
        constexpr int kt = decltype(KT)::value, st = kt % 3, sn = (kt + 1) % 3;
        int32_t(&gu)[GA] = (kt % 2 == 0) ? g0 : g1;
        int32_t(&gn)[GA] = (kt % 2 == 0) ? g1 : g0;
        if constexpr (kt + 2 < NK) issue(kt + 2, (kt + 2) % 3, gu);
        __builtin_amdgcn_sched_barrier(0);
        half(f0, f1, (uint32_t)st * STG_B, IC<1>{}, IC<1>{});
        if constexpr (kt + 1 < NK) {
            touch(f1);
            if constexpr (kt + 2 < NK)
                asm volatile("s_waitcnt vmcnt(%0)" ::"n"(G) : "memory");
            else
                asm volatile("s_waitcnt vmcnt(0)" ::: "memory");
            __builtin_amdgcn_s_barrier();
            asm volatile("" ::: "memory");
            __builtin_amdgcn_sched_barrier(0);
            if constexpr (kt + 3 < NK) read_g(kt + 3, gn);
            half(f1, f0, (uint32_t)sn * STG_B, IC<0>{}, IC<1>{});
        } else {
            half(f1, f0, 0u, IC<0>{}, IC<0>{});
        }
    });

    const float inv = p_pow2(-eA), invB = p_pow2(-eB);
    float *Ct = C + t * sC;
    if constexpr (EPI == 2) {
        static_assert(TN == 2 && WTN == 64, "heads epilogue: a wave tile 64 columns wide");
        const float *hw = t == 0 ? hw0 : hw1;
        const int nh = t == 0 ? na : 1;
        float wv[4][TN], bv[TN];
#pragma unroll
        for (int j = 0; j < TN; j++) {
            const int col = n0 + wn * WTN + j * 32 + fr;
            bv[j] = bias[(int64_t)t * N + col];
#pragma unroll
            for (int o = 0; o < 4; o++) {
                const float x = hw[(int64_t)(o < nh ? o : 0) * N + col];
                wv[o][j] = o < nh ? x : 0.0f;
            }
        }
        float *part = hpart + ((int64_t)(t * tiles_n + tn) * WGN + wn) * M * 4;
#pragma unroll
        for (int i = 0; i < TM; i++) {
            float pv[64];
#pragma unroll
            for (int q = 0; q < 64; q++) pv[q] = 0.0f;
#pragma unroll
            for (int j = 0; j < TN; j++) {
                const int col = n0 + wn * WTN + j * 32 + fr;
#pragma unroll
                for (int r = 0; r < 16; r++) {
                    const int64_t row = m0 + wm * WTM + i * 32 + (r & 3) + 8 * (r >> 2) + 4 * fh;
                    const float v = p_relu((hi[i][j][r] + lo[i][j][r] * P_LO_INV) * inv * invB + bv[j]);
                    if (row < M) Ct[row * N + col] = v;
#pragma unroll
                    for (int o = 0; o < 4; o++) pv[o * 16 + r] += v * wv[o][j];
                }
            }
#pragma unroll
            for (int c = 64, off = 16; off >= 1; c >>= 1, off >>= 1) {
                const bool up = (fr & off) != 0;
#pragma unroll
                for (int k = 0; k < c / 2; k++) {
                    const float send = up ? pv[k] : pv[k + c / 2], keep = up ? pv[k + c / 2] : pv[k];
                    pv[k] = keep + __shfl_xor(send, off);
                }
            }
            const int o = fr >> 3;
#pragma unroll
            for (int k = 0; k < 2; k++) {
                const int r = 2 * (fr & 7) + k;
                const int64_t row = m0 + wm * WTM + i * 32 + (r & 3) + 8 * (r >> 2) + 4 * fh;
                if (row < M) part[row * 4 + o] = pv[k];
            }
        }
        return;
    }
#pragma unroll
    for (int j = 0; j < TN; j++) {
        const int col = n0 + wn * WTN + j * 32 + fr;
        const float bv = EPI == 1 ? bias[(int64_t)t * N + col] : 0.0f;
#pragma unroll
        for (int i = 0; i < TM; i++) {
#pragma unroll
            for (int r = 0; r < 16; r++) {
                const int64_t row = m0 + wm * WTM + i * 32 + (r & 3) + 8 * (r >> 2) + 4 * fh;
                if (row < M) {
                    const float v = (hi[i][j][r] + lo[i][j][r] * P_LO_INV) * inv * invB;
                    Ct[row * N + col] = EPI == 1 ? p_relu(v + bv) : v;
                }
            }
        }
    }
}

}

hipError_t launch_h3p_gemm_nt(const void *A, const uint32_t *amaxA, const void *B, const uint32_t *amaxB, int64_t M,
                              int N, int K, int T, int64_t a_stride, int64_t b_stride, const float *bias, float *C,
                              int64_t c_stride, int cfg, hipStream_t s, const int32_t *a_rows, const float *head_w0,
                              int n_actions, const float *head_w1, float *head_part) {
    if (M <= 0) return hipSuccess;
    if (a_stride % 4 || b_stride % 4) return hipErrorInvalidValue;
    if (a_rows) {
        constexpr int BM = 128, BN = 256;
        if (cfg != 60 || K != 576 || N % BN || !bias || !C) return hipErrorInvalidValue;
        if (head_part && (T != 2 || n_actions < 1 || n_actions > 4 || !head_w0 || !head_w1)) return hipErrorInvalidValue;
        const int64_t tiles_m = (M + BM - 1) / BM;
        const int tiles_n = N / BN;
        const dim3 grid((unsigned)(tiles_m * tiles_n), T), block(512);
        const auto *a = static_cast<const p_u32x4 *>(A);
        const auto *b = static_cast<const p_u32x4 *>(B);
        if (head_part)
            hipLaunchKernelGGL((k_h3_pqg<BM, BN, 2, 4, 2>), grid, block, 0, s, a, b, amaxA, amaxB, M, N, a_stride / 4,
                               b_stride / 4, bias, C, c_stride, tiles_n, a_rows, head_w0, head_w1, n_actions,
                               head_part);
        else
            hipLaunchKernelGGL((k_h3_pqg<BM, BN, 2, 4, 1>), grid, block, 0, s, a, b, amaxA, amaxB, M, N, a_stride / 4,
                               b_stride / 4, bias, C, c_stride, tiles_n, a_rows, nullptr, nullptr, 0, nullptr);
        return hipGetLastError();
    }
    switch (cfg) {
        case 60: return pq_launch<128, 256, 2, 4>(A, B, amaxA, amaxB, M, N, K, T, a_stride, b_stride, bias, C, c_stride, s);
        case 62: return pq_launch<128, 192, 4, 2>(A, B, amaxA, amaxB, M, N, K, T, a_stride, b_stride, bias, C, c_stride, s);
        case 63: return pq_launch<128, 192, 4, 2, 4>(A, B, amaxA, amaxB, M, N, K, T, a_stride, b_stride, bias, C, c_stride, s);
        case 65: return pq_launch<256, 192, 4, 2, 2, true>(A, B, amaxA, amaxB, M, N, K, T, a_stride, b_stride, bias, C, c_stride, s);
        case 66: return pq_launch<128, 192, 4, 2, 3, false, 1>(A, B, amaxA, amaxB, M, N, K, T, a_stride, b_stride, bias, C, c_stride, s);
        case 68: return pq_launch<256, 256, 2, 2, 2, true>(A, B, amaxA, amaxB, M, N, K, T, a_stride, b_stride, bias, C, c_stride, s);
        case 69: return pq_launch<192, 192, 3, 2, 3, true>(A, B, amaxA, amaxB, M, N, K, T, a_stride, b_stride, bias, C, c_stride, s);
        default: return hipErrorInvalidValue;
    }
}


hipError_t launch_h3p_gemm_tn_gather(const void *A, const uint32_t *amaxA, const void *B, const uint32_t *amaxB,
                                     int64_t Kd, int M, int N, int T, int64_t a_stride, int64_t b_stride, int splits,
                                     float *slab, const int32_t *b_rows, int cfg, int *S_out, hipStream_t s) {
    const int BM = cfg == 21 ? 64 : 128;
    constexpr int BN = 192, BK = 32;
    if ((cfg != 20 && cfg != 21) || M % BM || N % BN || N % 64 || a_stride % 4 || b_stride % 4 || !b_rows)
        return hipErrorInvalidValue;
    const int tiles_n = N / BN, tiles = (M / BM) * tiles_n;
    int S = std::max(1, splits);
    int64_t kc = (Kd + S - 1) / S;
    kc = (kc + BK - 1) / BK * BK;
    S = (int)std::max<int64_t>(1, (Kd + kc - 1) / kc);
    *S_out = S;
    if (cfg == 21)
        hipLaunchKernelGGL((k_h3_tq<64, BN, 2, 2>), dim3(tiles * S * T), dim3(256), 0, s,
                           static_cast<const p_u32x4 *>(A), static_cast<const p_u32x4 *>(B), amaxA, amaxB, Kd, M, N,
                           a_stride / 4, b_stride / 4, kc, tiles_n, tiles, S, slab, b_rows);
    else
        hipLaunchKernelGGL((k_h3_tq<128, BN, 4, 2>), dim3(tiles * S * T), dim3(512), 0, s,
                           static_cast<const p_u32x4 *>(A), static_cast<const p_u32x4 *>(B), amaxA, amaxB, Kd, M, N,
                           a_stride / 4, b_stride / 4, kc, tiles_n, tiles, S, slab, b_rows);
    return hipGetLastError();
}

}
```

ppo-2dgrid_amd/csrc/merlin_internal.h:

```cpp
#pragma once

#include <hip/hip_runtime.h>
#include <stdint.h>

#include "merlin_hip.h"

namespace merlin {

struct EnvDev {
    int n, size, sp, difficulty, max_steps;
    int stuck_on, max_stay;
    double penalty;
    int explore_on;
    double bonus;
    int reseed;
    uint32_t *walls;
    uint4 *agent;
    ulonglong2 *rng_s;
    ulonglong2 *rng_i;
    uint2 *rng_b;
    double *ep_ret;
    int32_t *ep_len;
    uint32_t *visited;
    uint32_t *err;
// ... 75 lines not shown
    if (!isfinite(lse)) a = -1;
    action[k] = a;
    logp[k] = la;
    value[k] = acc[ACT_MAXA] + bc[0];
    return a;
}


struct ActIn {
    const float4 *part;
    int P;
    const float *ba, *bc;
    int A, det;
    uint64_t seed;
    const int64_t *epoch;
    int64_t step, env_offset;
    int64_t *action;
    float *logp, *value;
};

__device__ __forceinline__ int act_from_parts(const ActIn &c, int64_t n, int64_t k) {
    float4 a, v;
    if (c.P <= ACT_PARTS_UNROLL) {
        float4 xs[ACT_PARTS_UNROLL];
        float ys[ACT_PARTS_UNROLL];
#pragma unroll
        for (int p = 0; p < ACT_PARTS_UNROLL; p++) {
            const int q = p < c.P ? p : 0;
            xs[p] = c.part[(int64_t)q * n + k];
            ys[p] = reinterpret_cast<const float *>(c.part + (int64_t)(c.P + q) * n + k)[0];
        }
        a = xs[0];
        v = make_float4(ys[0], 0.0f, 0.0f, 0.0f);
#pragma unroll
        for (int p = 1; p < ACT_PARTS_UNROLL; p++) {
            if (p < c.P) {
                a.x += xs[p].x;
                a.y += xs[p].y;
                a.z += xs[p].z;
                a.w += xs[p].w;
                v.x += ys[p];
            }
        }
    } else {
        a = c.part[k];
        v = c.part[(int64_t)c.P * n + k];
        for (int p = 1; p < c.P; p++) {
            const float4 x = c.part[(int64_t)p * n + k], y = c.part[(int64_t)(c.P + p) * n + k];
            a.x += x.x;
            a.y += x.y;
            a.z += x.z;
            a.w += x.w;
            v.x += y.x;
        }
    }
    float acc[ACT_MAXA + 1];
#pragma unroll
    for (int j = 0; j <= ACT_MAXA; j++) acc[j] = 0.0f;
    acc[0] = a.x;
    acc[1] = a.y;
    acc[2] = a.z;
    acc[3] = a.w;
    acc[ACT_MAXA] = v.x;
    const uint64_t ep = c.epoch ? (uint64_t)c.epoch[0] : 0ull;
    return act_finish(acc, c.ba, c.bc, c.A, c.det, c.seed, ep, c.step, c.env_offset, k, c.action, c.logp, c.value);
}

__device__ __forceinline__ uint32_t bitrev7(uint32_t v) { return __brev(v) >> 25; }

template <class RowFn>
__device__ __forceinline__ void view_mask(RowFn row, int S, int ax, int ay, int dir, uint32_t V[7], uint32_t m[7]) {
    int tx, ty;
    if (dir == 0) {
        tx = ax;
        ty = ay - 3;
    } else if (dir == 1) {
        tx = ax - 3;
        ty = ay;
    } else if (dir == 2) {
        tx = ax - 6;
        ty = ay - 3;
    } else {
        tx = ax - 3;
        ty = ay - 6;
    }
    const uint64_t hi_ones = ~0ULL << (S + 8);
    uint32_t win[7];
#pragma unroll
    for (int r = 0; r < 7; r++) {
        const int y = ty + r;
        const bool in = (y >= 0) && (y < S);
        const uint32_t bits = in ? row(in ? y : 0) : 0xffffffffu;
        const uint64_t w = ((uint64_t)bits << 8) | 0xffULL | hi_ones;
        win[r] = (uint32_t)(w >> (tx + 8)) & 0x7fu;
    }
    uint32_t tr[7];
#pragma unroll
    for (int x = 0; x < 7; x++) {
        uint32_t v = 0u;
#pragma unroll
        for (int y = 0; y < 7; y++) v |= ((win[y] >> x) & 1u) << y;
        tr[x] = v;
    }
    const int k = (dir + 1) & 3;
    const bool odd = k & 1, flip = (k == 1) || (k == 2), rev = (k >= 2);
#pragma unroll
    for (int b = 0; b < 7; b++) {
        uint32_t t = flip ? (odd ? tr[6 - b] : win[6 - b]) : (odd ? tr[b] : win[b]);
        V[b] = rev ? bitrev7(t) : t;
    }
#pragma unroll
    for (int j = 0; j < 7; j++) m[j] = 0u;
    m[6] = 1u << 3;
#pragma unroll
    for (int j = 6; j >= 0; j--) {
        const uint32_t T = ~V[j] & 0x7fu;
        uint32_t M = m[j];
#pragma unroll
        for (int s = 0; s < 6; s++) M |= (M & T & 0x3fu) << 1;
        const uint32_t e1 = M & T & 0x3fu;
#pragma unroll
        for (int s = 0; s < 6; s++) M |= (M & T & 0x7eu) >> 1;
        const uint32_t e2 = M & T & 0x7eu;
        m[j] = M;
        if (j > 0) m[j - 1] |= e1 | (e1 << 1) | e2 | (e2 >> 1);
    }
}

struct StepOut {
    const int64_t *actions;
    int64_t action_stride;
    int n_steps;
    int autoreset;
    uint32_t *obs;
    float *reward;
    uint8_t *term;
    uint8_t *trunc;
    float *done;
    double *ep_ret_out;
    int32_t *ep_len_out;
    ActIn act;
    int no_fallback;
};

hipError_t zero_async(void *p, size_t bytes, hipStream_t s);
hipError_t launch_group_act(const uint32_t *codes, int G, const float *T2, const float *b2, const float *W3t,
                            const float *b3, const float *W4p, const float *b4, const float *Wa, const float *ba,
                            const float *Wc, const float *bc, int A, float *a3, float *part, bool shared, hipStream_t s);
hipError_t launch_h3p_gemm_nt(const void *A, const uint32_t *amaxA, const void *B, const uint32_t *amaxB, int64_t M,
                              int N, int K, int T, int64_t a_stride, int64_t b_stride, const float *bias, float *C,
                              int64_t c_stride, int cfg, hipStream_t s, const int32_t *a_rows = nullptr,
                              const float *head_w0 = nullptr, int n_actions = 0, const float *head_w1 = nullptr,
                              float *head_part = nullptr);
hipError_t launch_h3p_gemm_tn_gather(const void *A, const uint32_t *amaxA, const void *B, const uint32_t *amaxB,
                                     int64_t Kd, int M, int N, int T, int64_t a_stride, int64_t b_stride, int splits,
                                     float *slab, const int32_t *b_rows, int cfg, int *S_out, hipStream_t s);
hipError_t launch_env_reset(const EnvDev &E, const uint8_t *mask, uint32_t *obs, hipStream_t s);
hipError_t launch_env_step(const EnvDev &E, const StepOut &O, bool refill, hipStream_t s);
hipError_t launch_env_full_obs(const EnvDev &E, uint8_t *out, hipStream_t s);
hipError_t launch_env_refill(const EnvDev &E, bool full, hipStream_t s);
hipError_t upload_atlas(const uint8_t *atlas_host);
hipError_t launch_render_frames(const uint32_t *walls, const int32_t *goal, const int32_t *agent,
                                const int32_t *map_index, int64_t n_frames, int size, int ts, int highlight,
                                const uint8_t *atlas, uint8_t *out, uint32_t *err, hipStream_t s);
hipError_t launch_env_render(const EnvDev &E, const int64_t *index, int64_t n_frames, int ts, int highlight,
                             const uint8_t *atlas, uint8_t *out, hipStream_t s);
hipError_t launch_env_snapshot(const EnvDev &E, uint32_t *walls, int32_t *goal, int32_t *agent, hipStream_t s);
hipError_t launch_shortest_paths(const uint32_t *walls, const int32_t *goal, const int32_t *agent,
                                 const int32_t *map_index, int64_t n, int size, int32_t *dist, int16_t *field,
                                 hipStream_t s);
hipError_t launch_env_optimal_steps(const EnvDev &E, int32_t *dist, int16_t *field, hipStream_t s);
void shortest_paths_host(const uint32_t *walls, const int32_t *goal, const int32_t *agent, int64_t n, int S,
                         int32_t *dist, int16_t *field);
hipError_t launch_obs_expand_f32(const uint32_t *codes, const int64_t *index, int64_t n, float *out,
                                 float scale, int layout, hipStream_t s);
hipError_t launch_obs_expand_u8(const uint32_t *codes, const int64_t *index, int64_t n, uint8_t *out,
                                hipStream_t s);
hipError_t launch_gae(const float *rew, const float *val, const float *done, const float *last,
                      float *adv, float *ret, int T, int N, double gamma, double lam, double *stats,
                      double *partials, int max_partials, hipStream_t s);
hipError_t launch_adv_normalize(const float *adv, int64_t n, const double *stats, float *out,
                                hipStream_t s);
int gae_partials_needed(int T, int N);
int conv1_slab_floats(int towers);
hipError_t launch_conv1_lut_fwd(const uint32_t *codes, const int64_t *index, int64_t n, const float *tables,
                                const float *bias, int towers, float *out, hipStream_t s);
hipError_t launch_conv1_lut_bwd(const uint32_t *codes, const int64_t *index, int64_t n, const float *act,
                                const float *grad, int towers, float *dtables, float *dbias, float *slabs,
                                int max_slabs, hipStream_t s);
hipError_t launch_conv1_im2col_fwd(const uint32_t *codes, const int64_t *index, int64_t n, const float *tables,
                                   const float *bias, int T, float *A2, hipStream_t s);
hipError_t launch_conv1_im2col_bwd(const uint32_t *codes, const int64_t *index, int64_t n, const float *tables,
                                   const float *bias, const float *dA2, int T, float *dtables, float *dbias,
                                   float *slabs, int max_slabs, hipStream_t s);
hipError_t launch_im2col3_fwd(const float *Z2, const float *b2, int64_t n, int T, float *A3, hipStream_t s);
hipError_t launch_col2im3_bwd(const float *dA3, const float *Z2, const float *b2, int64_t n, int T, int chunked,
                              float *dZ2, uint32_t *absmax, hipStream_t s);
int conv2_lut_rows();
int conv2_lut_fblocks(int64_t n);
size_t conv2_lut_slab_bytes(int towers, int fblocks);
hipError_t launch_conv2_lut_fwd(const uint32_t *codes, const int64_t *index, int64_t n, const float *tables,
                                int towers, float *Z2, hipStream_t s, int64_t gstride = 0);
hipError_t launch_conv2_lut_bwd(const uint32_t *codes, int64_t n, const float *dZ2c, const uint32_t *absmax,
                                int towers, float *dT, void *slabs, hipStream_t s, int64_t gstride = 0);

hipError_t launch_patch_maps(const int32_t *kid, const int64_t *gkey, int64_t G, int64_t F, const int64_t *goff, int K,
                             int32_t *kmap, int32_t *rmap, int32_t *rep_row, hipStream_t s);
hipError_t launch_window_lut(const int32_t *rows, int64_t nw, const float *tab, int T, float *Z2w, hipStream_t s,
                             const float *b2 = nullptr);
hipError_t launch_window_conv3(const float *Q, int64_t nw, const int32_t *wid, const int64_t *groups, int64_t n,
                               const float *b3, int T, float *Y3, uint64_t *bits, uint32_t *amax,
                               const int32_t *rrow, int copy, hipStream_t s, uint32_t *colmax = nullptr,
                               uint32_t *bound = nullptr);
hipError_t launch_act_heads(const float *z, const float *b4, int64_t n, int H, const float *wa, const float *ba,
                            const float *wc, const float *bc, int A, int det, uint64_t seed, const int64_t *epoch,
                            int64_t step, int64_t env_offset, int64_t *action, float *logp, float *value,
                            hipStream_t s);
hipError_t launch_act_draw(const float *part, int P, int64_t n, const float *ba, const float *bc, int A, int det,
                           uint64_t seed, const int64_t *epoch, int64_t step, int64_t env_offset, int64_t *action,
                           float *logp, float *value, hipStream_t s);
int64_t ppo_loss_workspace_doubles(int64_t n_samples);
hipError_t launch_ppo_loss(const float *logits, const float *value, const float *bias_a, const float *bias_c,
                           int64_t U, int A, const int32_t *offs, const int32_t *order, const int64_t *inv, int64_t n,
                           const int64_t *sample_index, const int64_t *actions, const float *lp_old, const float *adv,
                           const float *ret, double clip_eps, double vf_coef, double ent_coef, float *dlogits,
                           float *dvalue, float *dbias_a, float *dbias_c, float *loss, double *stats,
                           double *workspace, hipStream_t s, uint32_t *dmax = nullptr);
hipError_t launch_codes_conv3(const uint32_t *codes, int64_t n, const float *Q, const float *b3, int T, float *Y3,
                              uint32_t *amax, uint32_t *err, hipStream_t s);
hipError_t launch_x6_gemm_nt32(const float *A, const void *B, int64_t M, int N, int K, int T, int64_t a_stride,
                               int64_t b_stride, const float *bias, float *C, int64_t c_stride, int cfg, hipStream_t s);
hipError_t launch_x6_gemm_tn32(const float *A, const float *B, int64_t Kd, int M, int N, int T, int64_t a_stride,
                               int64_t b_stride, int splits, float *slab, int cfg, hipStream_t s, int *S_out);
hipError_t launch_stage_fwd(const float *W1, const float *b1, const float *W2, const float *atlas, const int16_t *idx,
                            int T, float *HT, float *T2, hipStream_t s);
hipError_t launch_stage_bwd(const float *W2, const float *HT, const float *dT2, const float *atlas,
                            const int16_t *koff, const int16_t *kv, int T, float *dH, float *dW1, float *db1,
                            float *dW2, double *ws, hipStream_t s);
int64_t winbwd_work_floats(int T, int64_t nw);
hipError_t launch_winbwd(const float *a2w, const float *dQ, const float *W3r, int T, int64_t nw, float *da2w,
                         float *db2, float *dW3r, float *work, hipStream_t s, float *db3 = nullptr);
hipError_t launch_winfwd(const float *a2w, const float *W3r, int T, int64_t nw, float *Q, hipStream_t s);
constexpr size_t STAGE_WS_DOUBLES = 2 * 4 * 10 * 2048;
hipError_t launch_heads_fwd(const float *h, int64_t n, int H, const float *wa, int A, const float *wc, const float *ba,
                            const float *bc, float *logits, float *value, hipStream_t s);
hipError_t launch_seg_sum(const float *src, const void *mask, int mask_bits, int64_t src_rows, const int32_t *idx,
                          const int32_t *key, int64_t nnz, const int32_t *slot, int S, int64_t L, const int32_t *fix,
                          int64_t nfix, int T, float *out, int64_t out_rows, float *carry, int acc_out, int fill, int role,
                          int32_t *mark, const int32_t *hfix, int32_t *cnt, hipStream_t s,
                          const int32_t *mrow = nullptr);

constexpr int EPI_MAX_BLOCKS = 512;
size_t epilogue_work_floats();
bool epilogue_cols_ok(int cols);
int epilogue_max_act();
hipError_t launch_bias_relu(float *Z, const float *b, int64_t rows, int cols, int T, hipStream_t s);
hipError_t launch_relu_bwd_colsum(const float *Y, const float *dY, float *dZ, int64_t rows, int cols, int T,
                                  float *dbias, float *work, hipStream_t s);
hipError_t launch_colsum(const float *X, int64_t rows, int cols, int64_t row_stride, int64_t tower_stride, int T,
                         float *out, float *work, hipStream_t s);
hipError_t launch_head_bwd(const float *h, const float *dlogits, const float *dvalue, const float *wa,
                           const float *wc, int64_t n, int H, int A, float *dz, float *db4, float *dwa, float *dwc,
                           float *work, uint32_t *amax, hipStream_t s, const uint32_t *dmax = nullptr,
                           void *dz_planes = nullptr);

__device__ __forceinline__ void block_amax2(const uint32_t mx[2], int T, uint32_t *amax) {
    __shared__ uint32_t red[2][4];
    uint32_t m0 = mx[0], m1 = mx[1];
    for (int o = 32; o > 0; o >>= 1) {
        m0 = max(m0, (uint32_t)__shfl_xor((int)m0, o));
        m1 = max(m1, (uint32_t)__shfl_xor((int)m1, o));
    }
    if ((threadIdx.x & 63) == 0) {
        red[0][threadIdx.x >> 6] = m0;
        red[1][threadIdx.x >> 6] = m1;
    }
    __syncthreads();
    if (threadIdx.x < (unsigned)T) {
        const uint32_t *r = red[threadIdx.x];
        const uint32_t m = max(max(r[0], r[1]), max(r[2], r[3]));
        if (m && m > __hip_atomic_load(amax + threadIdx.x, __ATOMIC_RELAXED, __HIP_MEMORY_SCOPE_AGENT))
            atomicMax(amax + threadIdx.x, m);
    }
}

constexpr float H3_LO_SCALE = 2048.0f;
__device__ __forceinline__ int h3_exp(uint32_t amax) {
    if (amax == 0u) return 0;
    const int e = (int)((amax >> 23) & 0xffu) - 127;
    return min(max(14 - e, -120), 115);
}
__device__ __forceinline__ float pow2f(int e) { return __uint_as_float((uint32_t)(e + 127) << 23); }

__device__ __forceinline__ void h3_pair(float a, float b, float sc, float sc2, uint32_t &hi, uint32_t &lo) {
    const float m2048 = -H3_LO_SCALE, za = a * sc2, zb = b * sc2;
    uint32_t h, l;
    asm("v_fma_mixlo_f16 %0, %1, %2, 0" : "=v"(h) : "v"(a), "v"(sc));
    asm("v_fma_mixhi_f16 %0, %1, %2, 0" : "+v"(h) : "v"(b), "v"(sc));
    asm("v_fma_mixlo_f16 %0, %1, %2, %3 op_sel_hi:[1,0,0]" : "=v"(l) : "v"(h), "v"(m2048), "v"(za));
    asm("v_fma_mixhi_f16 %0, %1, %2, %3 op_sel:[1,0,0] op_sel_hi:[1,0,0]" : "+v"(l) : "v"(h), "v"(m2048), "v"(zb));
    hi = h;
    lo = l;
}

__device__ __forceinline__ void h3_store4(uint2 *__restrict__ row, int q, const float4 v, float sc, float sc2) {
    uint32_t h0, h1, l0, l1;
// ... 61 lines not shown
```

ppo-2dgrid_amd/merlin/_native.py:

```python
from __future__ import annotations

import contextlib
import ctypes as C
import gc
import os

import torch

PKG_ROOT = os.path.dirname(os.path.dirname(os.path.abspath(__file__)))
LIB_PATH = os.environ.get("MERLIN_HIP_LIB", os.path.join(PKG_ROOT, "lib", "libmerlin_hip.so"))

MERLIN_OK = 0
E_INVALID, E_HIP, E_DEVICE, E_UNSUPPORTED = 1, 2, 3, 4
LAYOUT_NCHW = 0
LAYOUT_NHWC = 1
OBS_WORDS = 8
DEVERR_BAD_ACTION = 1
DEVERR_PLACE_OBJ = 2
DEVERR_BAD_TILE = 4
DEVERR_SLOT_EMPTY = 8
DEVERR_BAD_FRAME = 16
FRAME_TILES = 22

DIFFICULTY_IDS = {"easy": 0, "medium": 1, "mediumhard": 2, "hard": 3, "hardest": 4}
# ... 58 lines not shown
    L.merlin_env_get_state.argtypes = [vp, vp, vp, vp, vp]
    L.merlin_env_full_obs.argtypes = [vp, vp, vp]
    L.merlin_env_errors.argtypes = [vp, C.POINTER(C.c_uint32), C.POINTER(C.c_uint32), vp]
    L.merlin_obs_expand_f32.argtypes = [vp, vp, i64, vp, C.c_float, i32, vp]
    L.merlin_obs_expand_u8.argtypes = [vp, vp, i64, vp, vp]
    L.merlin_gae.argtypes = [vp, vp, vp, vp, vp, vp, i32, i32, C.c_double, C.c_double, vp, vp]
    L.merlin_adv_normalize.argtypes = [vp, i64, vp, vp, vp]
    L.merlin_conv1_lut_fwd.argtypes = [vp, vp, i64, vp, vp, i32, vp, vp]
    L.merlin_conv1_lut_bwd.argtypes = [vp, vp, i64, vp, vp, i32, vp, vp, vp]
    L.merlin_tower_conv2_im2col_fwd.argtypes = [vp, vp, i64, vp, vp, i32, vp, vp]
    L.merlin_tower_conv2_im2col_bwd.argtypes = [vp, vp, i64, vp, vp, vp, i32, vp, vp, vp]
    L.merlin_tower_conv3_im2col_fwd.argtypes = [vp, vp, i64, i32, vp, vp]
    L.merlin_tower_conv3_col2im_bwd.argtypes = [vp, vp, vp, i64, i32, vp, vp]
    L.merlin_tower_conv3_col2im_bwd_chunked.argtypes = [vp, vp, vp, i64, i32, vp, vp, vp]
    L.merlin_tower_conv2_lut_rows.restype = C.c_int
    L.merlin_tower_conv2_lut_fwd.argtypes = [vp, vp, i64, vp, i32, vp, vp]
    L.merlin_tower_conv2_lut_bwd.argtypes = [vp, i64, vp, vp, i32, vp, vp]
    L.merlin_tower_conv2_lut_fwd_grouped.argtypes = [vp, i64, i64, vp, i32, vp, vp]
    L.merlin_tower_conv2_lut_slab_bytes.argtypes = [i32, i64]
    L.merlin_tower_conv2_lut_slab_bytes.restype = i64
    L.merlin_tower_conv2_lut_bwd_grouped.argtypes = [vp, i64, vp, vp, i32, vp, vp, vp]
    L.merlin_tower_window_lut.argtypes = [vp, i64, vp, i32, vp, vp]
    L.merlin_tower_window_conv3.argtypes = [vp, i64, vp, vp, i64, vp, i32, vp, vp]
    L.merlin_tower_window_lut_bias_relu.argtypes = [vp, i64, vp, i32, vp, vp, vp]
    L.merlin_minibatch_patch_maps.argtypes = [vp, vp, i64, i64, vp, i32, vp, vp, vp, vp]
    L.merlin_tower_window_conv3_bits.argtypes = [vp, i64, vp, vp, i64, vp, i32, vp, vp, vp, vp]
    L.merlin_tower_window_conv3_reuse.argtypes = [vp, i64, vp, vp, i64, vp, i32, vp, vp, vp, vp, i32, vp]
    L.merlin_tower_all_windows.restype = i64
    L.merlin_tower_codes_conv3.argtypes = [vp, i64, vp, vp, i32, vp, vp]
    L.merlin_tower_codes_conv3_amax.argtypes = [vp, i64, vp, vp, i32, vp, vp, vp]
    L.merlin_tower_errors.argtypes = [C.POINTER(C.c_uint32), vp]
    L.merlin_segment_sum.argtypes = [vp, i64, vp, vp, i64, vp, i32, i64, vp, i64, i32, vp, i64, vp, i32, vp]
    L.merlin_segment_sum_masked.argtypes = [vp, vp, i64, vp, vp, i64, vp, i32, i64, vp, i64, i32, vp, i64, vp, i32,
                                            vp]
    L.merlin_tower_heads_fwd.argtypes = [vp, i64, i32, vp, i32, vp, vp, vp, vp, vp, vp]
    L.merlin_segment_sum_marked.argtypes = [vp, vp, i64, vp, vp, i64, vp, i32, i64, vp, i64, i32, vp, i64, vp, i32,
                                            vp, vp]
    L.merlin_segment_sum_fused.argtypes = [vp, vp, i64, vp, vp, i64, vp, i32, i64, vp, i64, i32, vp, i64, vp, i32,
                                           vp, vp, vp, vp]
    L.merlin_segment_sum_mask_rows.argtypes = [vp, vp, i64, vp, vp, i64, vp, i32, i64, vp, i64, i32, vp, i64, vp, i32,
                                               vp, vp, vp, vp, vp]
    L.merlin_tower_bias_relu.argtypes = [vp, vp, i64, i32, i32, vp]
    L.merlin_tower_relu_bwd.argtypes = [vp, vp, vp, i64, i32, i32, vp, vp]
    L.merlin_tower_colsum.argtypes = [vp, i64, i32, i64, i64, i32, vp, vp]
    L.merlin_tower_head_bwd.argtypes = [vp, vp, vp, vp, vp, i64, i32, i32, vp, vp, vp, vp, vp, vp]
    L.merlin_tower_head_bwd_planes.argtypes = [vp, vp, vp, vp, vp, i64, i32, i32, vp, vp, vp, vp, vp, vp, vp]
    L.merlin_act_heads.argtypes = [vp, vp, i64, i32, vp, vp, vp, vp, i32, i32, C.c_uint64, vp, i64, i64, vp, vp, vp,
                                   vp]
    L.merlin_ppo_loss_workspace.argtypes = [i64]
    L.merlin_ppo_loss_workspace.restype = i64
    L.merlin_clip_adam_workspace.argtypes = [i32, vp]
    L.merlin_clip_adam_workspace.restype = i64
    L.merlin_clip_adam.argtypes = [i32, vp, vp, vp, vp, vp, vp, C.c_double, C.c_double, C.c_double, C.c_double, C.c_float,
                                   vp, vp, vp]
    L.merlin_ppo_loss.argtypes = [vp, vp, vp, vp, i64, i32, vp, vp, vp, i64, vp, vp, vp, vp, vp, C.c_double,
                                  C.c_double, C.c_double, vp, vp, vp, vp, vp, vp, vp, vp]
    L.merlin_ppo_loss_absmax.argtypes = [vp, vp, vp, vp, i64, i32, vp, vp, vp, i64, vp, vp, vp, vp, vp, C.c_double,
                                         C.c_double, C.c_double, vp, vp, vp, vp, vp, vp, vp, vp, vp]
    L.merlin_x6_split.argtypes = [vp, i64, vp, vp]
    L.merlin_x6_join.argtypes = [vp, i64, vp, vp]
    L.merlin_x6_gemm_nt.argtypes = [vp, vp, i64, i32, i32, i32, i64, i64, vp, vp, i64, i32, vp]
    L.merlin_x6_tn_slab_floats.argtypes = [i32, i32, i32, i32]
    L.merlin_x6_tn_slab_floats.restype = i64
    L.merlin_x6_gemm_tn.argtypes = [vp, vp, i64, i32, i32, i32, i64, i64, i32, vp, vp, i32, vp]
    L.merlin_h3_amax.argtypes = [vp, i64, i32, i64, vp, vp]
    L.merlin_h3_split.argtypes = [vp, i64, i32, vp, vp, vp]
    L.merlin_h3_gemm_nt.argtypes = [vp, vp, vp, vp, i64, i32, i32, i32, i64, i64, vp, vp, i64, vp, i32, vp]
    L.merlin_h3_gemm_tn.argtypes = [vp, vp, vp, vp, i64, i32, i32, i32, i64, i64, i32, vp, vp, i32, vp]
    L.merlin_h3_gemm_tn_planes.argtypes = [vp, vp, vp, vp, i64, i32, i32, i32, i64, i64, i32, vp, vp, i32, vp]
    L.merlin_h3_gemm_nt_gather.argtypes = [vp, vp, vp, vp, i64, i32, i32, i32, i64, i64, vp, vp, i64, vp, i32, vp]
    L.merlin_h3_gemm_tn_gather.argtypes = [vp, vp, vp, vp, i64, i32, i32, i32, i64, i64, i32, vp, vp, vp, i32, vp]
    L.merlin_h3_gemm_tn_gather_planes_a.argtypes = [vp, vp, vp, vp, i64, i32, i32, i32, i64, i64, i32, vp, vp, vp, i32,
                                                    vp]
    L.merlin_h3_gemm_nt_planes.argtypes = [vp, vp, vp, vp, i64, i32, i32, i32, i64, i64, vp, vp, i64, i32, vp]
    L.merlin_h3_gemm_nt_heads_planes.argtypes = [vp, vp, vp, vp, i64, i32, i32, i64, i64, vp, vp, i64, vp, vp, i32,
                                                 vp, vp, i32, vp]
    L.merlin_h3_gemm_tn_gather_planes.argtypes = [vp, vp, vp, vp, i64, i32, i32, i32, i64, i64, i32, vp, vp, vp, i32,
                                                  vp]
    L.merlin_tower_window_conv3_planes.argtypes = [vp, i64, vp, vp, i64, vp, i32, vp, vp, vp, vp, vp, vp]
    L.merlin_h3_gemm_nt_heads.argtypes = [vp, vp, vp, vp, i64, i32, i32, i64, i64, vp, vp, i64, vp, vp, i32, vp, vp,
                                          i32, vp]
    L.merlin_h3_heads_parts.argtypes = [i32, i32]
    L.merlin_h3_heads_parts.restype = i32
    L.merlin_heads_combine.argtypes = [vp, i32, i64, i32, vp, vp, vp]
    L.merlin_act_draw.argtypes = [vp, i32, i64, vp, vp, i32, i32, C.c_uint64, vp, i64, i64, vp, vp, vp, vp]
    L.merlin_stage_tables_fwd.argtypes = [vp, vp, vp, vp, vp, i32, vp, vp, vp]
    L.merlin_stage_tables_bwd.argtypes = [vp, vp, vp, vp, vp, vp, i32, vp, vp, vp, vp, vp]
    L.merlin_window_gemm_fwd.argtypes = [vp, vp, i32, i64, vp, vp]
    L.merlin_window_gemm_bwd_work.argtypes = [i32, i64]
    L.merlin_window_gemm_bwd_work.restype = i64
    L.merlin_window_gemm_bwd.argtypes = [vp, vp, vp, i32, i64, vp, vp, vp, vp, vp, i64, vp]
    L.merlin_group_clip_sgd_workspace.argtypes = [i32, vp, i32]
    L.merlin_group_clip_sgd_workspace.restype = i64
    L.merlin_group_clip_sgd.argtypes = [i32, vp, vp, vp, i32, C.c_float, C.c_float, vp, vp, vp]
    L.merlin_episode_loss.argtypes = [vp, vp, vp, vp, vp, i32, i32, C.c_double, C.c_double, vp, vp, vp]
    L.merlin_episode_class_stats.argtypes = [vp, vp, vp, vp, i32, i32, i32, vp, i32, vp]
    L.merlin_frame_atlas.argtypes = [i32, vp]
    L.merlin_render_frames.argtypes = [vp, vp, vp, vp, i64, i32, i32, i32, vp, vp]
    L.merlin_env_render.argtypes = [vp, vp, i64, i32, i32, vp, vp]
    L.merlin_env_snapshot.argtypes = [vp, vp, vp, vp, vp]
    L.merlin_shortest_paths.argtypes = [vp, vp, vp, vp, i64, i32, vp, vp, vp]
    L.merlin_env_optimal_steps.argtypes = [vp, vp, vp, vp]
    L.merlin_shortest_paths_host.argtypes = [vp, vp, vp, i64, i32, vp, vp]
    check_env_config_layout(L)
    _lib = L
    return L


def env_config_layout(L=None):
    L = L or lib()
    nf = len(EnvConfig._fields_)
    offs = (C.c_int64 * nf)()
    size = int(L.merlin_env_config_layout(offs, nf))
    return size, [int(o) for o in offs]


def check_env_config_layout(L) -> None:
    size, offs = env_config_layout(L)
    mine = [getattr(EnvConfig, f).offset for f, _ in EnvConfig._fields_]
    if size != C.sizeof(EnvConfig) or offs != mine:
        raise MerlinNativeError(f"EnvConfig layout mismatch: C sizeof {size} offsets {offs}, "
                                f"ctypes sizeof {C.sizeof(EnvConfig)} offsets {mine}")


EXPORTED_SYMBOLS = (
    "merlin_version", "merlin_last_error", "merlin_tile_atlas", "merlin_env_config_layout", "merlin_env_create",
    "merlin_env_destroy", "merlin_env_seed", "merlin_env_reset", "merlin_env_step", "merlin_env_act_step", "merlin_group_act",
    "merlin_env_set_refill_interval", "merlin_env_refill",
    "merlin_env_get_state", "merlin_env_full_obs", "merlin_env_errors", "merlin_env_set_step_fallback", "merlin_env_num_envs", "merlin_env_size",
    "merlin_obs_expand_f32", "merlin_obs_expand_u8", "merlin_gae", "merlin_adv_normalize",
    "merlin_conv1_lut_fwd", "merlin_conv1_lut_bwd", "merlin_tower_conv2_im2col_fwd",
    "merlin_tower_conv2_im2col_bwd", "merlin_tower_conv3_im2col_fwd", "merlin_tower_conv3_col2im_bwd",
    "merlin_tower_conv3_col2im_bwd_chunked", "merlin_tower_conv2_lut_rows", "merlin_tower_conv2_lut_fwd",
    "merlin_tower_conv2_lut_bwd", "merlin_tower_conv2_lut_fwd_grouped", "merlin_tower_conv2_lut_slab_bytes",
    "merlin_tower_conv2_lut_bwd_grouped", "merlin_tower_window_lut", "merlin_tower_window_lut_bias_relu", "merlin_minibatch_patch_maps", "merlin_segment_sum_mask_rows", "merlin_tower_window_conv3",
    "merlin_tower_window_conv3_bits", "merlin_tower_window_conv3_reuse", "merlin_tower_all_windows", "merlin_tower_codes_conv3",
    "merlin_tower_codes_conv3_amax", "merlin_tower_errors",
    "merlin_segment_sum", "merlin_segment_sum_masked", "merlin_segment_sum_marked", "merlin_segment_sum_fused", "merlin_tower_heads_fwd", "merlin_tower_bias_relu", "merlin_tower_relu_bwd", "merlin_tower_head_bwd",
    "merlin_tower_colsum",
    "merlin_ppo_loss_workspace", "merlin_ppo_loss", "merlin_act_heads",
    "merlin_x6_split", "merlin_x6_join", "merlin_x6_gemm_nt", "merlin_x6_tn_slab_floats", "merlin_x6_gemm_tn",
    "merlin_clip_adam_workspace", "merlin_clip_adam",
    "merlin_h3_amax", "merlin_h3_split", "merlin_h3_gemm_nt", "merlin_h3_gemm_tn",
    "merlin_h3_gemm_tn_planes", "merlin_h3_gemm_nt_gather", "merlin_h3_gemm_tn_gather",
    "merlin_h3_gemm_nt_heads", "merlin_h3_heads_parts", "merlin_heads_combine", "merlin_act_draw",
    "merlin_ppo_loss_absmax", "merlin_tower_head_bwd_planes", "merlin_h3_gemm_nt_planes",
    "merlin_h3_gemm_tn_gather_planes_a", "merlin_h3_gemm_nt_heads_planes", "merlin_h3_gemm_tn_gather_planes",
    "merlin_tower_window_conv3_planes", "merlin_window_gemm_bwd_work", "merlin_window_gemm_bwd",
    "merlin_window_gemm_fwd",
    "merlin_group_clip_sgd_workspace", "merlin_group_clip_sgd", "merlin_episode_loss",
    "merlin_env_set_difficulties", "merlin_episode_class_stats",
    "merlin_frame_atlas", "merlin_render_frames", "merlin_env_render", "merlin_env_snapshot",
    "merlin_shortest_paths", "merlin_env_optimal_steps", "merlin_shortest_paths_host",
)


_CAPTURE_DEPTH = 0
_DEFERRED: list = []

_hip_rt = None
_cu_streams = []


def cu_masked_stream(device, keep) -> torch.cuda.ExternalStream:
    global _hip_rt
    if _hip_rt is None:
        _hip_rt = C.CDLL("libamdhip64.so")
        _hip_rt.hipExtStreamCreateWithCUMask.argtypes = [C.POINTER(C.c_void_p), C.c_uint32, C.POINTER(C.c_uint32)]
    dev = torch.device(device)
    n = torch.cuda.get_device_properties(dev).multi_processor_count
    words = (n + 31) // 32
    mask = (C.c_uint32 * words)()
    for i in range(n):
        if keep(i):
            mask[i // 32] |= 1 << (i % 32)
    if not any(mask):
        raise MerlinNativeError("cu_masked_stream: empty CU mask")
    h = C.c_void_p()
    with torch.cuda.device(dev):
        err = _hip_rt.hipExtStreamCreateWithCUMask(C.byref(h), words, mask)
    if err != 0:
        raise MerlinNativeError(f"hipExtStreamCreateWithCUMask failed ({err})")
    _cu_streams.append(h.value)
    return torch.cuda.ExternalStream(h.value, device=dev)



@contextlib.contextmanager
def capture_guard():
    global _CAPTURE_DEPTH
    drain_deferred()
    gc.collect()
    was_enabled = gc.isenabled()
    gc.disable()
    _CAPTURE_DEPTH += 1
    try:
        yield
    finally:
        _CAPTURE_DEPTH -= 1
        if _CAPTURE_DEPTH == 0:
            if was_enabled:
                gc.enable()
            run_deferred()


def capturing() -> bool:
    if _CAPTURE_DEPTH > 0:
        return True
    try:
        return torch.cuda.is_available() and torch.cuda.is_current_stream_capturing()
    except Exception:
        return False


def defer_release(fn) -> None:
    if capturing():
        _DEFERRED.append(fn)
    else:
        run_deferred()
        fn()


def run_deferred() -> None:
    while _DEFERRED:
        _DEFERRED.pop(0)()


def drain_deferred() -> None:
    if _DEFERRED and not capturing():
        run_deferred()


H3_SPANS: set = set()
X6_SPANS: set = set()


class KernelTimer:

    records: list | None = None
    every = 1
    counts: dict = {}

    @classmethod
    def start(cls, every: int = 1):
        cls.records, cls.every, cls.counts = [], max(1, int(every)), {}

    @classmethod
    def stop(cls):
        recs, cls.records = cls.records, None
        return [(n, e0, e1, nb() if callable(nb) else nb, fl) for n, e0, e1, nb, fl in (recs or [])]

    @classmethod
    def active(cls) -> bool:
        return cls.records is not None

    @classmethod
    def span(cls, name: str, nbytes: int, flops: int = 0):
        if cls.records is None or torch.cuda.is_current_stream_capturing():
            return _NULL_SPAN
        c = cls.counts.get(name, 0)
        cls.counts[name] = c + 1
        if c % cls.every:
            return _NULL_SPAN
        return _Span(name, nbytes, flops)


class _Span:
    def __init__(self, name, nbytes, flops=0):
        self.name, self.nbytes, self.flops = name, nbytes, flops

    def __enter__(self):
        self.e0 = torch.cuda.Event(enable_timing=True)
        self.e0.record()
        return self

    def __exit__(self, *exc):
        e1 = torch.cuda.Event(enable_timing=True)
        e1.record()
        KernelTimer.records.append((self.name, self.e0, e1, self.nbytes, self.flops))
        return False


class _NullSpan:
    def __enter__(self):
        return self

    def __exit__(self, *exc):
        return False


_NULL_SPAN = _NullSpan()


def check(rc: int, what: str = "") -> None:
    if rc != MERLIN_OK:
        msg = lib().merlin_last_error().decode(errors="replace")
        err = MerlinNativeError(f"{what or 'merlin call'} failed (code {rc}): {msg}")
        err.code = int(rc)
        raise err


def ptr(t: torch.Tensor | None):
    if t is None:
        return None
    if not t.is_cuda:
        raise MerlinNativeError("merlin HIP kernels need device (cuda/hip) tensors; got a CPU tensor")
# ... 672 lines not shown
X6_TN_SPLITS = 32


def x6_split(x: torch.Tensor, out: torch.Tensor | None = None) -> torch.Tensor:
    assert x.dtype == torch.float32 and x.shape[-1] % 8 == 0
    x = x.contiguous()
    if out is None:
        out = torch.empty((*x.shape[:-1], 3 * x.shape[-1]), dtype=torch.int16, device=x.device)
    with KernelTimer.span("k_x6_split", x.numel() * 10):
        check(lib().merlin_x6_split(ptr(x), x.numel(), ptr(out), stream_of(x)), "merlin_x6_split")
    return out


def x6_join(planes: torch.Tensor) -> torch.Tensor:
    assert planes.dtype == torch.int16 and planes.shape[-1] % 24 == 0
    out = torch.empty((*planes.shape[:-1], planes.shape[-1] // 3), dtype=torch.float32, device=planes.device)
    check(lib().merlin_x6_join(ptr(planes), out.numel(), ptr(out), stream_of(planes)), "merlin_x6_join")
    return out


def x6_gemm_nt(A: torch.Tensor, B: torch.Tensor, bias: torch.Tensor | None = None, cfg: int = 0,
               out: torch.Tensor | None = None, name: str = "x6_gemm_nt") -> torch.Tensor:
    X6_SPANS.add(name)
    T, M, K = (int(v) for v in A.shape)
    assert A.dtype == torch.float32
    N = int(B.shape[1])
    assert B.dtype == torch.int16 and B.shape == (T, N, 3 * K)
    assert A.is_contiguous() and B.is_contiguous()
    if bias is not None:
        assert bias.shape == (T, N) and bias.dtype == torch.float32
        bias = bias.detach().contiguous()
    if out is None:
        out = torch.empty((T, M, N), dtype=torch.float32, device=A.device)
    assert out.shape == (T, M, N) and out.is_contiguous()
    with KernelTimer.span(name, 0, 2 * T * M * N * K):
        check(lib().merlin_x6_gemm_nt(ptr(A), ptr(B), M, N, K, T, M * K, N * K, ptr(bias), ptr(out), M * N, int(cfg),
                                      stream_of(A)), "merlin_x6_gemm_nt")
    return out


def x6_gemm_tn(A: torch.Tensor, B: torch.Tensor, splits: int | None = None, cfg: int | None = None,
               name: str = "x6_gemm_tn", out: torch.Tensor | None = None) -> torch.Tensor:
    X6_SPANS.add(name)
    splits = X6_TN_SPLITS if splits is None else splits
    cfg = X6_TN_CFG if cfg is None else cfg
    T, Kd, M = (int(v) for v in A.shape)
    N = int(B.shape[2])
    assert A.dtype == B.dtype == torch.float32
    assert B.shape[:2] == (T, Kd)
    assert A.is_contiguous() and B.is_contiguous()
    if out is None:
        out = torch.empty((T, M, N), dtype=torch.float32, device=A.device)
    assert out.shape == (T, M, N) and out.dtype == torch.float32 and out.is_contiguous()
    slab = torch.empty(int(lib().merlin_x6_tn_slab_floats(M, N, T, int(splits))), dtype=torch.float32,
                       device=A.device)
    with KernelTimer.span(name, 0, 2 * T * M * N * Kd):
        check(lib().merlin_x6_gemm_tn(ptr(A), ptr(B), Kd, M, N, T, Kd * M, Kd * N, int(splits), ptr(slab), ptr(out),
                                      int(cfg), stream_of(A)), "merlin_x6_gemm_tn")
    return out


H3_NT_CFG = {"fwd": 13, "dgrad": 11, "rollout": 12, "qall": 1, "qwin": 11, "qwin_dgrad": 5, "dgrad_planes": 62, "fwd_planes": 60}
H3_TN_CFG = 0
H3_TN_CFG_PLANES = 20
H3_HEADS_EPILOGUE = True
H3_TN_CFG_WIN = 2
H3_TN_SPLITS = 32


def group_act(codes, T2, b2, W3t, b3, W4p, b4, Wa, ba, Wc, bc, a3_ws=None, part=None):
    G = int(codes.shape[0])
    A = int(Wa.shape[1])
    W = int(T2.shape[0]) // 2
    shared = W == 1 and G > 1
    assert W == G or shared
    assert codes.dtype == torch.int32 and codes.shape == (G, OBS_WORDS) and codes.is_contiguous()
    assert T2.shape == (2 * W, 2720, 64) and W3t.shape == (2 * W, 576, 64) and W4p.shape == (2 * W, 512, 576)
    assert b2.numel() == 2 * W * 64 and b3.numel() == 2 * W * 64 and b4.numel() == 2 * W * 512
    assert Wa.shape == (W, A, 512) and ba.numel() == W * A and Wc.numel() == W * 512 and bc.numel() == W
    for t in (T2, b2, W3t, b3, W4p, b4, Wa, ba, Wc, bc):
        assert t.dtype == torch.float32 and t.is_contiguous()
    if a3_ws is None:
        a3_ws = torch.empty((2 * G, 576), dtype=torch.float32, device=codes.device)
    if part is None:
        part = torch.empty((2, 8, G, 4), dtype=torch.float32, device=codes.device)
    with KernelTimer.span("k_group_act", G * 2 * (25 * 16 * 256 + 576 * 64 * 4 + 512 * 576 * 4)):
        check(lib().merlin_group_act(ptr(codes), G, ptr(T2), ptr(b2), ptr(W3t), ptr(b3), ptr(W4p), ptr(b4), ptr(Wa),
                                     ptr(ba), ptr(Wc), ptr(bc), A, ptr(a3_ws), ptr(part), int(shared),
                                     stream_of(codes)),
              "merlin_group_act")
    return part


def h3_amax(x: torch.Tensor, out: torch.Tensor | None = None) -> torch.Tensor:
    assert x.dtype == torch.float32 and x.is_contiguous()
    T = int(x.shape[0])
    n = x.numel() // max(T, 1)
    if out is None:
        out = torch.empty(T, dtype=torch.int32, device=x.device)
    assert out.dtype == torch.int32 and out.numel() >= T and out.is_contiguous()
    with KernelTimer.span("k_h3_amax", 4 * T * n):
        check(lib().merlin_h3_amax(ptr(x), n, T, n, ptr(out), stream_of(x)), "merlin_h3_amax")
    return out


def h3_zero(amax: torch.Tensor) -> torch.Tensor:
    assert amax.dtype == torch.int32 and amax.is_contiguous()
    check(lib().merlin_h3_amax(None, 0, int(amax.numel()), 0, ptr(amax), stream_of(amax)), "merlin_h3_amax")
    return amax


def h3_split(x: torch.Tensor, amax: torch.Tensor, out: torch.Tensor | None = None) -> torch.Tensor:
    assert x.dtype == torch.float32 and x.shape[-1] % 8 == 0 and amax.dtype == torch.int32
    x = x.contiguous()
    T = int(x.shape[0])
    if out is None:
        out = torch.empty(x.shape[:-1] + (2 * x.shape[-1],), dtype=torch.int16, device=x.device)
    check(lib().merlin_h3_split(ptr(x), x.numel() // T, T, ptr(amax), ptr(out), stream_of(x)), "merlin_h3_split")
    return out


def h3_gemm_nt(A: torch.Tensor, amaxA: torch.Tensor, B: torch.Tensor, amaxB: torch.Tensor,
               bias: torch.Tensor | None = None, cfg: int = 0, out: torch.Tensor | None = None,
               name: str = "h3_gemm_nt", planes_out: torch.Tensor | None = None,
               rows: torch.Tensor | None = None) -> torch.Tensor:
    H3_SPANS.add(name)
    T, M, K = (int(v) for v in A.shape)
    N = int(B.shape[1])
    assert A.dtype == torch.float32 and B.dtype == torch.int16 and B.shape == (T, N, 2 * K)
    assert A.is_contiguous() and B.is_contiguous() and amaxA.dtype == amaxB.dtype == torch.int32
    if out is None:
        out = torch.empty((T, M, N), dtype=torch.float32, device=A.device)
    assert out.shape == (T, M, N) and out.is_contiguous()
    if bias is not None:
        assert bias.shape == (T, N) and bias.is_contiguous()
    if planes_out is not None:
        assert planes_out.dtype == torch.int16 and planes_out.shape == (T, M, 2 * K) and planes_out.is_contiguous()
    if rows is not None:
        assert planes_out is None and rows.dtype == torch.int32 and rows.is_contiguous() and K % 64 == 0
        assert rows.numel() == M * K // 64
        with KernelTimer.span(name, 0, 2 * T * M * N * K):
            check(lib().merlin_h3_gemm_nt_gather(ptr(A), ptr(amaxA), ptr(B), ptr(amaxB), M, N, K, T, M * K, N * K,
                                                 ptr(bias) if bias is not None else None, ptr(out), M * N, ptr(rows),
                                                 int(cfg), stream_of(A)), "merlin_h3_gemm_nt_gather")
        return out
    with KernelTimer.span(name, 0, 2 * T * M * N * K):
        check(lib().merlin_h3_gemm_nt(ptr(A), ptr(amaxA), ptr(B), ptr(amaxB), M, N, K, T, M * K, N * K,
                                      ptr(bias) if bias is not None else None, ptr(out), M * N,
                                      ptr(planes_out) if planes_out is not None else None, int(cfg),
                                      stream_of(A)), "merlin_h3_gemm_nt")
    return out


def h3_gemm_nt_planes(Ap: torch.Tensor, amaxA: torch.Tensor, B: torch.Tensor, amaxB: torch.Tensor,
                      bias: torch.Tensor | None = None, cfg: int = 62, out: torch.Tensor | None = None,
                      name: str = "h3_gemm_nt") -> torch.Tensor:
    H3_SPANS.add(name)
    T, M, K2 = (int(v) for v in Ap.shape)
    K = K2 // 2
    N = int(B.shape[1])
    assert Ap.dtype == B.dtype == torch.int16 and B.shape == (T, N, 2 * K) and Ap.is_contiguous() and B.is_contiguous()
    assert amaxA.dtype == amaxB.dtype == torch.int32
    if out is None:
        out = torch.empty((T, M, N), dtype=torch.float32, device=Ap.device)
    assert out.shape == (T, M, N) and out.is_contiguous()
    if bias is not None:
        assert bias.shape == (T, N) and bias.is_contiguous()
    with KernelTimer.span(name, 0, 2 * T * M * N * K):
        check(lib().merlin_h3_gemm_nt_planes(ptr(Ap), ptr(amaxA), ptr(B), ptr(amaxB), M, N, K, T, M * K, N * K,
                                             ptr(bias) if bias is not None else None, ptr(out), M * N, int(cfg),
                                             stream_of(Ap)), "merlin_h3_gemm_nt_planes")
    return out


def h3_gemm_nt_heads(A: torch.Tensor, amaxA: torch.Tensor, B: torch.Tensor, amaxB: torch.Tensor, bias: torch.Tensor,
                     Wa: torch.Tensor, Wc: torch.Tensor, cfg: int, rows: torch.Tensor | None = None,
                     name: str = "h3_gemm_nt", partials_only: bool = False) -> tuple:
    H3_SPANS.add(name)
    T, M, K = (int(v) for v in A.shape)
    ap = A.dtype == torch.int16
    if ap:
        K //= 2
        assert rows is not None and not partials_only
    N = int(B.shape[1])
    NA = int(Wa.shape[0])
    assert T == 2 and A.dtype in (torch.float32, torch.int16) and B.dtype == torch.int16 and B.shape == (T, N, 2 * K)
    assert A.is_contiguous() and B.is_contiguous() and bias.shape == (T, N) and bias.is_contiguous()
    assert Wa.shape == (NA, N) and Wa.is_contiguous() and Wc.numel() == N and Wc.is_contiguous() and 1 <= NA <= 4
    P = int(lib().merlin_h3_heads_parts(N, int(cfg)))
    assert P > 0, f"cfg {cfg}: no heads epilogue"
    if rows is not None:
        assert rows.dtype == torch.int32 and rows.is_contiguous() and rows.numel() == M * K // 64
    out = None if partials_only else torch.empty((T, M, N), dtype=torch.float32, device=A.device)
    part = torch.empty((T, P, M, 4), dtype=torch.float32, device=A.device)
    fn = lib().merlin_h3_gemm_nt_heads_planes if ap else lib().merlin_h3_gemm_nt_heads
    with KernelTimer.span(name, 0, 2 * T * M * N * K):
        check(fn(ptr(A), ptr(amaxA), ptr(B), ptr(amaxB), M, N, K, M * K, N * K, ptr(bias), ptr(out), M * N, ptr(rows),
                 ptr(Wa), NA, ptr(Wc), ptr(part), int(cfg), stream_of(A)), "merlin_h3_gemm_nt_heads")
    if partials_only:
        return part
    logits = torch.empty((M, NA), dtype=torch.float32, device=A.device)
    value = torch.empty(M, dtype=torch.float32, device=A.device)
    with KernelTimer.span("k_heads_fwd", T * P * M * 16 + M * (NA + 1) * 4):
        check(lib().merlin_heads_combine(ptr(part), P, M, NA, ptr(logits), ptr(value), stream_of(A)),
              "merlin_heads_combine")
    return out, logits, value


def act_draw(part, b_actor, b_critic, deterministic=False, seed=0, epoch=None, step=0, out=None, env_offset=0):
    T, P, n, _ = (int(x) for x in part.shape)
    A = int(b_actor.numel())
    assert T == 2 and part.dtype == torch.float32 and part.is_contiguous() and 1 <= A <= 4 and b_critic.numel() == 1
    if not deterministic and epoch is None:
        raise ValueError("act_draw: a sampled action needs an epoch counter tensor (int64[1] on the device)")
    dev = part.device
    if out is None:
        out = (torch.empty(n, dtype=torch.int64, device=dev), torch.empty(n, dtype=torch.float32, device=dev),
               torch.empty(n, dtype=torch.float32, device=dev))
    action, logp, value = out
    assert action.dtype == torch.int64 and logp.dtype == value.dtype == torch.float32
    assert action.numel() == logp.numel() == value.numel() == n
    with KernelTimer.span("k_act_heads", part.numel() * 4 + n * 16):
        check(lib().merlin_act_draw(ptr(part), P, n, ptr(b_actor), ptr(b_critic), A, int(bool(deterministic)),
                                    int(seed) & 0xFFFFFFFFFFFFFFFF, ptr(epoch), int(step), int(env_offset), ptr(action),
                                    ptr(logp), ptr(value), stream_of(part)), "merlin_act_draw")
    return action, logp, value


def h3_gemm_tn(A: torch.Tensor, amaxA: torch.Tensor, B: torch.Tensor, amaxB: torch.Tensor,
               splits: int | None = None, cfg: int | None = None, name: str = "h3_gemm_tn",
               out: torch.Tensor | None = None, rows: torch.Tensor | None = None) -> torch.Tensor:
    H3_SPANS.add(name)
    splits = H3_TN_SPLITS if splits is None else splits
    cfg = H3_TN_CFG if cfg is None else cfg
    planes = A.dtype == torch.int16
    a_planes = planes and (B.dtype == torch.float32 or rows is not None)
    b_planes = a_planes and B.dtype == torch.int16
    if a_planes:
        planes = False
    T, Kd, M = (int(v) for v in A.shape)
    if a_planes:
        M //= 2
    N = int(B.shape[2]) // (2 if b_planes else 1)
    if a_planes:
        assert rows is not None and M % 8 == 0, "A planes: the gathered form only"
    elif planes:
        assert B.dtype == torch.int16 and M % 2 == 0 and N % 2 == 0
        M, N = M // 2, N // 2
    else:
        assert A.dtype == B.dtype == torch.float32
    assert B.shape[:2] == (T, Kd)
    assert A.is_contiguous() and B.is_contiguous() and amaxA.dtype == amaxB.dtype == torch.int32
    if out is None:
        out = torch.empty((T, M, N), dtype=torch.float32, device=A.device)
    assert out.shape == (T, M, N) and out.dtype == torch.float32 and out.is_contiguous()
    slab = torch.empty(int(lib().merlin_x6_tn_slab_floats(M, N, T, int(splits))), dtype=torch.float32,
                       device=A.device)
    if rows is not None:
        assert not planes and rows.dtype == torch.int32 and rows.is_contiguous() and N % 64 == 0
        assert rows.numel() == Kd * N // 64
        fn = (lib().merlin_h3_gemm_tn_gather_planes if b_planes else lib().merlin_h3_gemm_tn_gather_planes_a
              if a_planes else lib().merlin_h3_gemm_tn_gather)
        with KernelTimer.span(name, 0, 2 * T * M * N * Kd):
            check(fn(ptr(A), ptr(amaxA), ptr(B), ptr(amaxB), Kd, M, N, T, Kd * M, Kd * N, int(splits), ptr(slab),
                     ptr(out), ptr(rows), int(cfg), stream_of(A)), "merlin_h3_gemm_tn_gather")
        return out
    fn = lib().merlin_h3_gemm_tn_planes if planes else lib().merlin_h3_gemm_tn
    with KernelTimer.span(name, 0, 2 * T * M * N * Kd):
        check(fn(ptr(A), ptr(amaxA), ptr(B), ptr(amaxB), Kd, M, N, T, Kd * M, Kd * N, int(splits), ptr(slab),
                 ptr(out), int(cfg), stream_of(A)), "merlin_h3_gemm_tn")
    return out


def stage_tables_fwd(W1, b1, W2, atlas, idx, HT=None, T2=None):
    T = int(W1.shape[0])
    assert W1.shape == (T, 32, 3, 8, 8) and b1.shape == (T, 32) and W2.shape == (T, 64, 32, 4, 4)
    assert all(x.dtype == torch.float32 and x.is_contiguous() for x in (W1, b1, W2, atlas))
    assert idx.dtype == torch.int16 and idx.shape == (680, 4) and atlas.shape == (5, 3, 8, 8)
    HT = torch.empty((T, 680, 32), dtype=torch.float32, device=W1.device) if HT is None else HT
    T2 = torch.empty((T, LUT2_ROWS, 64), dtype=torch.float32, device=W1.device) if T2 is None else T2
    check(lib().merlin_stage_tables_fwd(ptr(W1), ptr(b1), ptr(W2), ptr(atlas), ptr(idx), T, ptr(HT), ptr(T2),
                                        stream_of(W1)), "merlin_stage_tables_fwd")
    return HT, T2


def stage_tables_bwd(W2, HT, dT2, atlas, koff, kv, dW1=None, db1=None, dW2=None, dH=None):
    T = int(W2.shape[0])
    dev = W2.device
    assert dT2.shape == (T, LUT2_ROWS, 64) and HT.shape == (T, 680, 32) and dT2.is_contiguous()
    assert koff.dtype == kv.dtype == torch.int16 and koff.numel() == 81 and kv.numel() == 2720
    dW1 = torch.empty((T, 32, 3, 8, 8), dtype=torch.float32, device=dev) if dW1 is None else dW1
    db1 = torch.empty((T, 32), dtype=torch.float32, device=dev) if db1 is None else db1
    dW2 = torch.empty((T, 64, 32, 4, 4), dtype=torch.float32, device=dev) if dW2 is None else dW2
    dH = torch.empty((T, 680, 32), dtype=torch.float32, device=dev) if dH is None else dH
    assert all(x.is_contiguous() for x in (dW1, db1, dW2, dH))
    check(lib().merlin_stage_tables_bwd(ptr(W2), ptr(HT), ptr(dT2), ptr(atlas), ptr(koff), ptr(kv), T, ptr(dH),
                                        ptr(dW1), ptr(db1), ptr(dW2), stream_of(W2)), "merlin_stage_tables_bwd")
    return dW1, db1, dW2


def clip_adam(params, grads, exp_avgs, exp_avg_sqs, steps, lr, beta1, beta2, eps, max_norm, norm_out=None,
              workspace=None):
    n = len(params)
    if not (len(grads) == len(exp_avgs) == len(exp_avg_sqs) == len(steps) == n):
        raise ValueError("clip_adam: parameter / state lists differ in length")
    for group in (params, grads, exp_avgs, exp_avg_sqs, steps):
        for t in group:
            if t.dtype != torch.float32:
                raise MerlinNativeError("clip_adam: float32 tensors only")
    for p, g, m, v in zip(params, grads, exp_avgs, exp_avg_sqs):
        if not (p.numel() == g.numel() == m.numel() == v.numel()):
            raise ValueError("clip_adam: a parameter and its gradient / state differ in size")
    numel = (C.c_int64 * n)(*[int(p.numel()) for p in params])
    arr = lambda ts: (C.c_void_p * n)(*[ptr(t).value for t in ts])
    dev = params[0].device
    if workspace is None:
        workspace = torch.empty(int(lib().merlin_clip_adam_workspace(n, numel)), dtype=torch.float64, device=dev)
    if norm_out is None:
        norm_out = torch.empty((), dtype=torch.float32, device=dev)
    check(lib().merlin_clip_adam(n, arr(params), arr(grads), arr(exp_avgs), arr(exp_avg_sqs), arr(steps), numel,
                                 float(lr), float(beta1), float(beta2), float(eps), float(max_norm), ptr(norm_out),
                                 ptr(workspace), stream_of(params[0])), "merlin_clip_adam")
    return norm_out


def group_clip_sgd(params, grads, lr, max_norm, norm_out=None, workspace=None):
    n = len(params)
    if len(grads) != n:
        raise ValueError("group_clip_sgd: parameter / gradient lists differ in length")
    if n == 0:
        return norm_out
    if n > 32:
        raise ValueError("group_clip_sgd: at most 32 tensors")
    G = int(params[0].shape[0])
    for p, g in zip(params, grads):
        if p.dtype != torch.float32 or g.dtype != torch.float32:
            raise MerlinNativeError("group_clip_sgd: float32 tensors only")
        if p.dim() < 1 or p.shape != g.shape or int(p.shape[0]) != G:
            raise ValueError("group_clip_sgd: every parameter and gradient is [G, *shape] with the same G")
    dev = params[0].device
    if norm_out is None:
        norm_out = torch.empty(G, dtype=torch.float32, device=dev)
    if G == 0:
        return norm_out
    if norm_out.dtype != torch.float32 or norm_out.numel() != G:
        raise ValueError("group_clip_sgd: norm_out is float32[G]")
    numel = (C.c_int64 * n)(*[int(p.numel() // G) for p in params])
    arr = lambda ts: (C.c_void_p * n)(*[ptr(t).value for t in ts])
    need = int(lib().merlin_group_clip_sgd_workspace(n, numel, G))
    if need < 0:
        raise ValueError("group_clip_sgd: empty tensors are not supported")
    if workspace is None:
        workspace = torch.empty(need, dtype=torch.float64, device=dev)
# ... 54 lines not shown
```

Baseline: 4.661 million.

## Add persistent tile-walking variants of the plane GEMM kernels for forward and dgrad

Converts the plane-operand GEMM kernels (pq and gathered pqg) into device tile functions and adds a persistent 'walk' mode. In this mode a fixed number of blocks (one per CU by default) loop over tiles in XCD-aware order and prefetch the next tile's operands via global_load_lds DMA while the current tile finishes. The walk path is enabled by default for cfg 60 forward and cfg 62 dgrad, with new cfgs 75-78 to select either variant. The aim is to cut launch/tail overhead and overlap the epilogue with the next tile's loads, at the cost of more complexity and a risk of load imbalance or register pressure.

```diff
diff --git a/include/merlin_hip.h b/include/merlin_hip.h
--- a/include/merlin_hip.h
+++ b/include/merlin_hip.h
@@ -290,6 +290,7 @@
                             const int32_t *a_rows_dev, const float *head_w0_dev, int32_t n_actions,
                             const float *head_w1_dev, float *head_partials_dev, int32_t cfg, void *stream);
 int32_t merlin_h3_heads_parts(int32_t N, int32_t cfg);
+int merlin_h3_walk_blocks(int32_t blocks);
 int merlin_h3_gemm_nt_planes(const void *A_planes_dev, const uint32_t *amax_a_dev, const void *B_dev,
                              const uint32_t *amax_b_dev, int64_t M, int32_t N, int32_t K, int32_t towers,
                              int64_t a_stride, int64_t b_stride, const float *bias_dev, float *C_dev, int64_t c_stride,
diff --git a/ppo-2dgrid_amd/csrc/merlin_capi.hip b/ppo-2dgrid_amd/csrc/merlin_capi.hip
--- a/ppo-2dgrid_amd/csrc/merlin_capi.hip
+++ b/ppo-2dgrid_amd/csrc/merlin_capi.hip
@@ -1287,7 +1287,8 @@
 int merlin_h3_gemm_nt_planes(const void *A_planes, const uint32_t *amax_a, const void *B, const uint32_t *amax_b,
                              int64_t M, int32_t N, int32_t K, int32_t towers, int64_t a_stride, int64_t b_stride,
                              const float *bias, float *C, int64_t c_stride, int32_t cfg, void *stream) {
-    if (cfg < 60 || cfg >= 70) return fail(MERLIN_E_UNSUPPORTED, "plane-operand cfgs are 60..69");
+    if (cfg < 60 || (cfg >= 70 && cfg != 77 && cfg != 78))
+        return fail(MERLIN_E_UNSUPPORTED, "plane-operand cfgs are 60..69, 77 and 78");
     return h3_gemm_nt(static_cast<const float *>(A_planes), amax_a, B, amax_b, M, N, K, towers, a_stride, b_stride,
                       bias, C, c_stride, nullptr, nullptr, cfg, stream);
 }
@@ -1340,6 +1341,12 @@
 
 int32_t merlin_h3_heads_parts(int32_t N, int32_t cfg) { return merlin::h3_heads_parts(N, cfg); }
 
+int merlin_h3_walk_blocks(int32_t blocks) {
+    if (blocks < 0) return fail(MERLIN_E_INVALID, "blocks must be 0 (one per CU) or positive");
+    merlin::set_h3p_walk_blocks(blocks);
+    return MERLIN_OK;
+}
+
 int merlin_act_draw(const float *partials, int32_t parts, int64_t n, const float *b_actor, const float *b_critic,
                     int32_t n_actions, int32_t deterministic, uint64_t seed, const int64_t *epoch, int64_t step,
                     int64_t env_offset, int64_t *action, float *logp, float *value, void *stream) {
diff --git a/ppo-2dgrid_amd/csrc/merlin_h3.hip b/ppo-2dgrid_amd/csrc/merlin_h3.hip
--- a/ppo-2dgrid_amd/csrc/merlin_h3.hip
+++ b/ppo-2dgrid_amd/csrc/merlin_h3.hip
@@ -1471,8 +1471,8 @@
     ((a_rows || head_part) ? hipErrorInvalidValue          \
                            : ntg_launch<BM, BN, WM, WN, KP>(A, b, amaxA, amaxB, M, N, K, T, a_stride, sB, bias, C, \
                                                             c_stride, P, s))
-    if (a_is_planes && (cfg < 10 || cfg > 14) && cfg != 60) return hipErrorInvalidValue;
-    if (cfg >= 60 && cfg < 70) {
+    if (a_is_planes && (cfg < 10 || cfg > 14) && cfg != 60 && cfg != 75 && cfg != 76) return hipErrorInvalidValue;
+    if ((cfg >= 60 && cfg < 70) || (cfg >= 75 && cfg < 79)) {
         if (P || ((a_rows || head_part) && !a_is_planes)) return hipErrorInvalidValue;
         return launch_h3p_gemm_nt(A, amaxA, B, amaxB, M, N, K, T, a_stride, b_stride, bias, C, c_stride, cfg, s, a_rows,
                                   head_w0, n_actions, head_w1, head_part);
@@ -1568,7 +1568,9 @@
         case 12: return N % 128 ? 0 : N / 128 * 2;
         case 13: return N % 256 ? 0 : N / 256 * 4;
         case 14: return N % 128 ? 0 : N / 128 * 2;
-        case 60: return N % 256 ? 0 : N / 256 * 4;
+        case 60:
+        case 75:
+        case 76: return N % 256 ? 0 : N / 256 * 4;
         default: return 0;
     }
 }
diff --git a/ppo-2dgrid_amd/csrc/merlin_h3p.hip b/ppo-2dgrid_amd/csrc/merlin_h3p.hip
--- a/ppo-2dgrid_amd/csrc/merlin_h3p.hip
+++ b/ppo-2dgrid_amd/csrc/merlin_h3p.hip
@@ -48,12 +48,12 @@
 typedef __attribute__((address_space(3))) p_u32x4 lds_u32x4;
 __device__ __forceinline__ void lds_rd(p_u32x4 &d, uint32_t addr) { d = *(const lds_u32x4 *)(uintptr_t)addr; }
 
-template <int BM, int BN, int WGM, int WGN, int EPI, int NK, int NS = 3, bool ONE = false, int ORD = 0>
-__global__ __launch_bounds__(64 * WGM * WGN) void k_h3_pq(const p_u32x4 *__restrict__ A, const p_u32x4 *__restrict__ B,
-                                                          const uint32_t *__restrict__ amaxA,
-                                                          const uint32_t *__restrict__ amaxB, int64_t M, int N, int K,
-                                                          int64_t sA, int64_t sB, const float *__restrict__ bias,
-                                                          float *__restrict__ C, int64_t sC, int tiles_n) {
+template <int BM, int BN, int WGM, int WGN, int EPI, int NK, int NS, bool ONE, int ORD>
+__device__ __forceinline__ void pq_tile(const p_u32x4 *__restrict__ A, const p_u32x4 *__restrict__ B,
+                                        const uint32_t *__restrict__ amaxA, const uint32_t *__restrict__ amaxB,
+                                        int64_t M, int N, int K, int64_t sA, int64_t sB,
+                                        const float *__restrict__ bias, float *__restrict__ C, int64_t sC,
+                                        int tiles_n) {
     constexpr int NT = 64 * WGM * WGN;
     constexpr int WTM = BM / WGM, WTN = BN / WGN;
     constexpr int TM = WTM / 32, TN = WTN / 32;
@@ -216,35 +216,6 @@
         }
     }
 }
-
-template <int BM, int BN, int WGM, int WGN, int NS = 3, bool ONE = false, int ORD = 0>
-hipError_t pq_launch(const void *A, const void *B, const uint32_t *amaxA, const uint32_t *amaxB, int64_t M, int N,
-                     int K, int T, int64_t sA, int64_t sB, const float *bias, float *C, int64_t sC, hipStream_t s) {
-    if (N % BN || K % 32 || K < 64) return hipErrorInvalidValue;
-    const int64_t tiles_m = (M + BM - 1) / BM;
-    const int tiles_n = N / BN;
-    if (tiles_m * tiles_n > INT32_MAX) return hipErrorInvalidValue;
-    const dim3 grid((unsigned)(tiles_m * tiles_n), T), block(64 * WGM * WGN);
-    const auto *a = static_cast<const p_u32x4 *>(A);
-    const auto *b = static_cast<const p_u32x4 *>(B);
-#define PQ_K(NK)                                                                                                   \
-    do {                                                                                                           \
-        if (bias)                                                                                                  \
-            hipLaunchKernelGGL((k_h3_pq<BM, BN, WGM, WGN, 1, NK, NS, ONE, ORD>), grid, block, 0, s, a, b, amaxA, amaxB, M, N, K, \
-                               sA / 4, sB / 4, bias, C, sC, tiles_n);                                              \
-        else                                                                                                       \
-            hipLaunchKernelGGL((k_h3_pq<BM, BN, WGM, WGN, 0, NK, NS, ONE, ORD>), grid, block, 0, s, a, b, amaxA, amaxB, M, N, K, \
-                               sA / 4, sB / 4, nullptr, C, sC, tiles_n);                                           \
-    } while (0)
-    switch (K) {
-        case 576: PQ_K(18); break;
-        case 512: PQ_K(16); break;
-        default: return hipErrorInvalidValue;
-    }
-#undef PQ_K
-    return hipGetLastError();
-}
-
 
 __device__ uint4 p_zero16[1] = {{0u, 0u, 0u, 0u}};
 
@@ -473,14 +444,12 @@
 
 
 template <int BM, int BN, int WGM, int WGN, int EPI>
-__global__ __launch_bounds__(64 * WGM * WGN) void k_h3_pqg(const p_u32x4 *__restrict__ A, const p_u32x4 *__restrict__ B,
-                                                           const uint32_t *__restrict__ amaxA,
-                                                           const uint32_t *__restrict__ amaxB, int64_t M, int N,
-                                                           int64_t sA, int64_t sB, const float *__restrict__ bias,
-                                                           float *__restrict__ C, int64_t sC, int tiles_n,
-                                                           const int32_t *__restrict__ amap,
-                                                           const float *__restrict__ hw0, const float *__restrict__ hw1,
-                                                           int na, float *__restrict__ hpart) {
+__device__ __forceinline__ void pqg_tile(const p_u32x4 *__restrict__ A, const p_u32x4 *__restrict__ B,
+                                         const uint32_t *__restrict__ amaxA, const uint32_t *__restrict__ amaxB,
+                                         int64_t M, int N, int64_t sA, int64_t sB, const float *__restrict__ bias,
+                                         float *__restrict__ C, int64_t sC, int tiles_n,
+                                         const int32_t *__restrict__ amap, const float *__restrict__ hw0,
+                                         const float *__restrict__ hw1, int na, float *__restrict__ hpart) {
     constexpr int K = 576, NK = 18, KC = K / 64;
     constexpr int NT = 64 * WGM * WGN;
     constexpr int WTM = BM / WGM, WTN = BN / WGN;
@@ -706,8 +675,639 @@
     }
 }
 
-}
-
+#define P_VMCNT(n) asm volatile("s_waitcnt vmcnt(%0)" ::"n"(n) : "memory")
+__device__ __forceinline__ void p_dma16s(const void *sbase, uint32_t voff, uint32_t lds) {
+    uint32_t keep;
+    asm volatile("s_mov_b32 %0, m0\n\ts_mov_b32 m0, %3\n\tglobal_load_lds_dwordx4 %1, %2\n\ts_mov_b32 m0, %0"
+                 : "=&s"(keep)
+                 : "v"(voff), "s"(sbase), "s"(lds)
+                 : "memory");
+}
+__device__ __forceinline__ void p_dma4s(const void *sbase, uint32_t voff, uint32_t lds) {
+    uint32_t keep;
+    asm volatile("s_mov_b32 %0, m0\n\ts_mov_b32 m0, %3\n\tglobal_load_lds_dword %1, %2\n\ts_mov_b32 m0, %0"
+                 : "=&s"(keep)
+                 : "v"(voff), "s"(sbase), "s"(lds)
+                 : "memory");
+}
+__device__ __forceinline__ void p_drain_loads() { __builtin_amdgcn_s_waitcnt(0x0F70); }
+
+struct PItem {
+    int t, n0, tn;
+    int64_t m0;
+};
+__device__ __forceinline__ PItem p_item(int v, int W, int tiles, int tiles_n, int BM, int BN) {
+    const int it = p_xcd_tile(v, W), t = it / tiles, L = it - t * tiles, tm = L / tiles_n, tn = L - tm * tiles_n;
+    return PItem{t, tn * BN, tn, (int64_t)tm * BM};
+}
+
+template <int BM, int BN, int WGM, int WGN, int EPI, int NK, int ORD>
+__device__ __forceinline__ void pq_walk(const p_u32x4 *__restrict__ A, const p_u32x4 *__restrict__ B,
+                                        const uint32_t *__restrict__ amaxA, const uint32_t *__restrict__ amaxB,
+                                        int64_t M, int N, int K, int64_t sA, int64_t sB,
+                                        const float *__restrict__ bias, float *__restrict__ C, int64_t sC,
+                                        int tiles_n, int tiles, int W) {
+    constexpr int NT = 64 * WGM * WGN;
+    constexpr int WTM = BM / WGM, WTN = BN / WGN;
+    constexpr int TM = WTM / 32, TN = WTN / 32;
+    constexpr int NR = 2 * (TM + TN), NM = 3 * TM * TN;
+    static_assert(NM >= NR, "a read behind every MFMA");
+    static_assert((BM * 8) % NT == 0 && (BN * 8) % NT == 0, "whole DMA instructions per thread");
+    constexpr int GA = BM * 8 / NT, GB = BN * 8 / NT, G = GA + GB;
+    constexpr int STG = (BM + BN) * 8;
+    constexpr uint32_t STG_B = STG * 16;
+    constexpr int S = TM * TN * 16;
+    constexpr int CARRY = S + G < 63 ? S + G : 63;
+    const int N_ = N;
+    static_assert(NK >= 4, "the look-ahead's k steps");
+    __shared__ p_u32x4 lds[3 * STG];
+
+    int v = blockIdx.x;
+    const int nb = gridDim.x;
+    if (v >= W) return;
+    const int tid = threadIdx.x, lane = tid & 63, w = tid >> 6;
+    const int wm = w / WGN, wn = w - (w / WGN) * WGN;
+    const int64_t row_ch = K / 4;
+    const uint32_t lds0 = (uint32_t)(uintptr_t)(__attribute__((address_space(3))) p_u32x4 *)lds;
+    const uint32_t wbase = (uint32_t)__builtin_amdgcn_readfirstlane(w) * 64u * 16u;
+
+    PItem cur = p_item(v, W, tiles, tiles_n, BM, BN);
+    int lt = cur.t, ln = cur.n0;
+    int eA = p_exp(p_amax(amaxA + lt)), eB = p_exp(p_amax(amaxB + lt));
+    float bvv[TN];
+    const int fr = lane & 31, fh = lane >> 5;
+#pragma unroll
+    for (int j = 0; j < TN; j++) bvv[j] = EPI == 1 ? bias[(int64_t)lt * N + ln + wn * WTN + j * 32 + fr] : 0.0f;
+    p_drain_loads();
+
+    uint32_t offA[GA], offB[GB];
+    auto set_offA = [&](const PItem &it) __attribute__((always_inline)) {
+#pragma unroll
+        for (int i = 0; i < GA; i++) {
+            const int q = i * NT + tid, r = q >> 3, c = (q & 7) ^ p_swz(r);
+            offA[i] = (uint32_t)(std::min<int64_t>(r, M - 1 - it.m0) * row_ch + c) * 16u;
+        }
+    };
+#pragma unroll
+    for (int i = 0; i < GB; i++) {
+        const int q = (GA + i) * NT + tid, r = q >> 3, c = (q & 7) ^ p_swz(r);
+        offB[i] = (uint32_t)((r - BM) * row_ch + c) * 16u;
+    }
+    const p_u32x4 *bA, *bB;
+    auto set_base = [&](const PItem &it) __attribute__((always_inline)) {
+        bA = A + it.t * sA + it.m0 * row_ch;
+        bB = B + it.t * sB + (int64_t)it.n0 * row_ch;
+        set_offA(it);
+    };
+    uint32_t sv[3] = {0u, STG_B, 2u * STG_B};
+    auto issue = [&](auto KT, uint32_t so) __attribute__((always_inline)) {
+        constexpr int kt = decltype(KT)::value;
+        const uint32_t base = lds0 + so + wbase;
+#pragma unroll
+        for (int i = 0; i < GA; i++) p_dma16s(bA + kt * 8, offA[i], base + (uint32_t)(i * NT) * 16u);
+#pragma unroll
+        for (int i = 0; i < GB; i++) p_dma16s(bB + kt * 8, offB[i], base + (uint32_t)((GA + i) * NT) * 16u);
+    };
+
+    uint32_t adA[2][2], adB[2][2];
+    {
+        const int ra = wm * WTM + fr, rb = BM + wn * WTN + fr;
+#pragma unroll
+        for (int kh = 0; kh < 2; kh++)
+#pragma unroll
+            for (int p = 0; p < 2; p++) {
+                const int c = 2 * (2 * kh + fh) + p;
+                adA[kh][p] = lds0 + (uint32_t)(ra * 8 + (c ^ p_swz(ra))) * 16u;
+                adB[kh][p] = lds0 + (uint32_t)(rb * 8 + (c ^ p_swz(rb))) * 16u;
+            }
+    }
+    struct Frag {
+        p_u32x4 a[TM][2], b[TN][2];
+    };
+    p_f32x16 hi[TM][TN], lo[TM][TN];
+    auto zero = [&]() __attribute__((always_inline)) {
+#pragma unroll
+        for (int i = 0; i < TM; i++)
+#pragma unroll
+            for (int j = 0; j < TN; j++) {
+                hi[i][j] = p_f32x16{};
+                lo[i][j] = p_f32x16{};
+            }
+    };
+    zero();
+    auto rd = [&](Frag &g, auto K_, uint32_t so, auto KH) __attribute__((always_inline)) {
+        constexpr int k = decltype(K_)::value, kh = decltype(KH)::value;
+        if constexpr (k < 2 * TM)
+            lds_rd(g.a[k >> 1][k & 1], adA[kh][k & 1] + so + (k >> 1) * 32 * 128);
+        else
+            lds_rd(g.b[(k - 2 * TM) >> 1][k & 1], adB[kh][k & 1] + so + ((k - 2 * TM) >> 1) * 32 * 128);
+    };
+    auto mf = [&](const Frag &f, auto M_) __attribute__((always_inline)) {
+        constexpr int m = decltype(M_)::value, tl = ORD ? m % (TM * TN) : m / 3, pr = ORD ? m / (TM * TN) : m % 3;
+        constexpr int i = tl / TN, j = tl % TN;
+        if constexpr (pr == 0)
+            lo[i][j] = p_mfma(f.a[i][1], f.b[j][0], lo[i][j]);
+        else if constexpr (pr == 1)
+            lo[i][j] = p_mfma(f.a[i][0], f.b[j][1], lo[i][j]);
+        else
+            hi[i][j] = p_mfma(f.a[i][0], f.b[j][0], hi[i][j]);
+    };
+    auto half = [&](const Frag &f, Frag &g, uint32_t so, auto KH, auto READS) __attribute__((always_inline)) {
+        static_for<NM>([&](auto M_) __attribute__((always_inline)) {
+            mf(f, M_);
+            if constexpr (decltype(READS)::value && decltype(M_)::value < NR) rd(g, M_, so, KH);
+        });
+        if constexpr (decltype(READS)::value) {
+            static_for<NR>([&](auto) __attribute__((always_inline)) {
+                __builtin_amdgcn_sched_group_barrier(0x008, 1, 0);
+                __builtin_amdgcn_sched_group_barrier(0x100, 1, 0);
+            });
+            if constexpr (NM > NR) __builtin_amdgcn_sched_group_barrier(0x008, NM - NR, 0);
+        }
+        __builtin_amdgcn_sched_barrier(0);
+    };
+    auto touch = [&](const Frag &f) __attribute__((always_inline)) {
+#pragma unroll
+        for (int i = 0; i < TM; i++) asm volatile("" ::"v"(f.a[i][0]), "v"(f.a[i][1]));
+#pragma unroll
+        for (int j = 0; j < TN; j++) asm volatile("" ::"v"(f.b[j][0]), "v"(f.b[j][1]));
+    };
+    auto publish = [&]() __attribute__((always_inline)) {
+        __builtin_amdgcn_s_barrier();
+        asm volatile("" ::: "memory");
+        __builtin_amdgcn_sched_barrier(0);
+    };
+    auto store_tile = [&](auto FULL) __attribute__((always_inline)) {
+        const float inv = p_pow2(-eA), invB = p_pow2(-eB);
+        float *Ct = C + cur.t * sC;
+        int64_t N = N_;
+        int rw = wm * WTM + 4 * fh;
+        asm volatile("" : "+s"(N), "+v"(rw));
+#pragma unroll
+        for (int j = 0; j < TN; j++) {
+            const int col = cur.n0 + wn * WTN + j * 32 + fr;
+#pragma unroll
+            for (int i = 0; i < TM; i++) {
+#pragma unroll
+                for (int r = 0; r < 16; r++) {
+                    const int64_t row = cur.m0 + rw + i * 32 + (r & 3) + 8 * (r >> 2);
+                    if (decltype(FULL)::value || row < M) {
+                        const float x = (hi[i][j][r] + lo[i][j][r] * P_LO_INV) * inv * invB;
+                        Ct[row * N + col] = EPI == 1 ? p_relu(x + bvv[j]) : x;
+                    }
+                }
+            }
+        }
+    };
+
+    set_base(cur);
+    issue(IC<0>{}, sv[0]);
+    issue(IC<1>{}, sv[1]);
+    P_VMCNT(G);
+    publish();
+    bool carried = false;
+    for (;;) {
+        const bool more = v + nb < W;
+        const PItem nxt = more ? p_item(v + nb, W, tiles, tiles_n, BM, BN) : cur;
+        Frag f0, f1;
+        static_for<NR>([&](auto K_) __attribute__((always_inline)) { rd(f0, K_, sv[0], IC<0>{}); });
+        static_for<NK>([&](auto KT) __attribute__((always_inline)) {
+            constexpr int kt = decltype(KT)::value, st = kt % 3, sn = (kt + 1) % 3, s2 = (kt + 2) % 3;
+            if constexpr (kt == NK - 2) set_base(nxt);
+            issue(IC<(kt + 2) % NK>{}, sv[s2]);
+            __builtin_amdgcn_sched_barrier(0);
+            half(f0, f1, sv[st], IC<1>{}, IC<1>{});
+            touch(f1);
+            if constexpr (kt == 0) {
+                if (carried)
+                    P_VMCNT(CARRY);
+                else
+                    P_VMCNT(G);
+            } else {
+                P_VMCNT(G);
+            }
+            publish();
+            if constexpr (kt + 1 < NK)
+                half(f1, f0, sv[sn], IC<0>{}, IC<1>{});
+            else
+                half(f1, f0, 0u, IC<0>{}, IC<0>{});
+        });
+        if (cur.t != lt || (EPI == 1 && cur.n0 != ln)) {
+            lt = cur.t, ln = cur.n0;
+            eA = p_exp(p_amax(amaxA + lt)), eB = p_exp(p_amax(amaxB + lt));
+#pragma unroll
+            for (int j = 0; j < TN; j++)
+                bvv[j] = EPI == 1 ? bias[(int64_t)lt * N + ln + wn * WTN + j * 32 + fr] : 0.0f;
+            p_drain_loads();
+        }
+        carried = cur.m0 + BM <= M;
+        if (carried) {
+            store_tile(IC<1>{});
+        } else {
+            store_tile(IC<0>{});
+            P_VMCNT(0);
+        }
+        zero();
+        if (!more) break;
+        v += nb;
+        cur = nxt;
+        if constexpr (NK % 3 == 1) {
+            const uint32_t x = sv[0];
+            sv[0] = sv[1], sv[1] = sv[2], sv[2] = x;
+        } else if constexpr (NK % 3 == 2) {
+            const uint32_t x = sv[2];
+            sv[2] = sv[1], sv[1] = sv[0], sv[0] = x;
+        }
+    }
+    P_VMCNT(0);
+}
+
+template <int BM, int BN, int WGM, int WGN, int EPI>
+__device__ __forceinline__ void pqg_walk(const p_u32x4 *__restrict__ A, const p_u32x4 *__restrict__ B,
+                                         const uint32_t *__restrict__ amaxA, const uint32_t *__restrict__ amaxB,
+                                         int64_t M, int N, int64_t sA, int64_t sB, const float *__restrict__ bias,
+                                         float *__restrict__ C, int64_t sC, int tiles_n, int tiles, int W,
+                                         const int32_t *__restrict__ amap, const float *__restrict__ hw0,
+                                         const float *__restrict__ hw1, int na, float *__restrict__ hpart) {
+    constexpr int K = 576, NK = 18, KC = K / 64;
+    constexpr int NT = 64 * WGM * WGN;
+    constexpr int WTM = BM / WGM, WTN = BN / WGN;
+    constexpr int TM = WTM / 32, TN = WTN / 32;
+    constexpr int NR = 2 * (TM + TN), NM = 3 * TM * TN;
+    static_assert(NM >= NR, "a read behind every MFMA");
+    static_assert((BM * 8) % NT == 0 && (BN * 8) % NT == 0, "whole DMA instructions per thread");
+    constexpr int GA = BM * 8 / NT, GB = BN * 8 / NT, G = GA + GB;
+    constexpr int GX = (BM * KC + NT - 1) / NT, XS = GX * NT;
+    constexpr int STG = (BM + BN) * 8;
+    constexpr uint32_t STG_B = STG * 16;
+    constexpr int S = TM * TN * 16 + (EPI == 2 ? 2 * TM : 0);
+    constexpr int CARRY = S + G < 63 ? S + G : 63;
+    const int N_ = N;
+    static_assert(EPI == 1 || EPI == 2, "bias + ReLU, heads optional");
+    static_assert(EPI != 2 || (TN == 2 && WTN == 64), "heads epilogue: a wave tile 64 columns wide");
+    __shared__ p_u32x4 lds[3 * STG];
+    __shared__ int32_t gmap[2 * XS];
+
+    int v = blockIdx.x;
+    const int nb = gridDim.x;
+    if (v >= W) return;
+    const int tid = threadIdx.x, lane = tid & 63, w = tid >> 6;
+    const int wm = w / WGN, wn = w - (w / WGN) * WGN;
+    const int fr = lane & 31, fh = lane >> 5;
+    const uint32_t lds0 = (uint32_t)(uintptr_t)(__attribute__((address_space(3))) p_u32x4 *)lds;
+    const uint32_t gm0 = (uint32_t)(uintptr_t)(__attribute__((address_space(3))) int32_t *)gmap;
+    const uint32_t wbase = (uint32_t)__builtin_amdgcn_readfirstlane(w) * 64u;
+
+    PItem cur = p_item(v, W, tiles, tiles_n, BM, BN);
+    int lt = -1, ln = -1, eA = 0, eB = 0;
+    float bvv[TN], wv[4][TN];
+    auto load_consts = [&]() __attribute__((always_inline)) {
+        lt = cur.t, ln = cur.n0;
+        eA = p_exp(p_amax(amaxA + lt)), eB = p_exp(p_amax(amaxB + lt));
+        const float *hw = lt == 0 ? hw0 : hw1;
+        const int nh = lt == 0 ? na : 1;
+#pragma unroll
+        for (int j = 0; j < TN; j++) {
+            const int col = ln + wn * WTN + j * 32 + fr;
+            bvv[j] = bias[(int64_t)lt * N + col];
+#pragma unroll
+            for (int o = 0; o < 4; o++) {
+                if constexpr (EPI == 2) {
+                    const float x = hw[(int64_t)(o < nh ? o : 0) * N + col];
+                    wv[o][j] = o < nh ? x : 0.0f;
+                } else {
+                    wv[o][j] = 0.0f;
+                }
+            }
+        }
+        p_drain_loads();
+    };
+    load_consts();
+
+    int ga[GA];
+    uint32_t ca[GA], offB[GB];
+#pragma unroll
+    for (int i = 0; i < GA; i++) {
+        const int q = i * NT + tid, r = q >> 3;
+        ga[i] = r * KC;
+        ca[i] = (uint32_t)((q & 7) ^ p_swz(r)) * 16u;
+    }
+#pragma unroll
+    for (int i = 0; i < GB; i++) {
+        const int q = i * NT + tid, r = q >> 3;
+        offB[i] = (uint32_t)(r * (K / 4) + ((q & 7) ^ p_swz(r))) * 16u;
+    }
+    auto issue_map = [&](int64_t m0, int bf) __attribute__((always_inline)) {
+        int tl = tid;
+        asm volatile("" : "+v"(tl));
+        const int mr = (int)(M - 1 - m0);
+#pragma unroll
+        for (int i = 0; i < GX; i++) {
+            const int e = std::min(i * NT + tl, BM * KC - 1), r = e / KC;
+            p_dma4s(amap + m0 * KC, (uint32_t)(std::min(r, mr) * KC + (e - r * KC)) * 4u,
+                    gm0 + (uint32_t)(bf * XS + i * NT) * 4u + wbase * 4u);
+        }
+    };
+    auto read_g = [&](int kt, uint32_t (&g)[GA], int bf) __attribute__((always_inline)) {
+#pragma unroll
+        for (int i = 0; i < GA; i++)
+            g[i] = (uint32_t)*(const lds_i32 *)(uintptr_t)(gm0 + (uint32_t)(bf * XS + ga[i] + kt / 2) * 4u) * 256u +
+                   ca[i];
+    };
+    const p_u32x4 *At, *baseB;
+    auto set_base = [&](const PItem &it) __attribute__((always_inline)) {
+        At = A + it.t * sA;
+        baseB = B + it.t * sB + (int64_t)it.n0 * (K / 4);
+    };
+    auto issue = [&](auto KT, int st, const uint32_t (&g)[GA]) __attribute__((always_inline)) {
+        constexpr int kt = decltype(KT)::value;
+        const uint32_t base = lds0 + (uint32_t)(st * STG) * 16u + wbase * 16u;
+#pragma unroll
+        for (int i = 0; i < GA; i++) p_dma16s(At + 8 * (kt & 1), g[i], base + (uint32_t)(i * NT) * 16u);
+#pragma unroll
+        for (int i = 0; i < GB; i++) p_dma16s(baseB + kt * 8, offB[i], base + (uint32_t)((GA + i) * NT) * 16u);
+    };
+
+    uint32_t adA[2][2], adB[2][2];
+    {
+        const int ra = wm * WTM + fr, rb = BM + wn * WTN + fr;
+#pragma unroll
+        for (int kh = 0; kh < 2; kh++)
+#pragma unroll
+            for (int p = 0; p < 2; p++) {
+                const int c = 2 * (2 * kh + fh) + p;
+                adA[kh][p] = lds0 + (uint32_t)(ra * 8 + (c ^ p_swz(ra))) * 16u;
+                adB[kh][p] = lds0 + (uint32_t)(rb * 8 + (c ^ p_swz(rb))) * 16u;
+            }
+    }
+    struct Frag {
+        p_u32x4 a[TM][2], b[TN][2];
+    };
+    p_f32x16 hi[TM][TN], lo[TM][TN];
+    auto zero = [&]() __attribute__((always_inline)) {
+#pragma unroll
+        for (int i = 0; i < TM; i++)
+#pragma unroll
+            for (int j = 0; j < TN; j++) {
+                hi[i][j] = p_f32x16{};
+                lo[i][j] = p_f32x16{};
+            }
+    };
+    zero();
+    auto rd = [&](Frag &g, auto K_, uint32_t so, auto KH) __attribute__((always_inline)) {
+        constexpr int k = decltype(K_)::value, kh = decltype(KH)::value;
+        if constexpr (k < 2 * TM)
+            lds_rd(g.a[k >> 1][k & 1], adA[kh][k & 1] + so + (k >> 1) * 32 * 128);
+        else
+            lds_rd(g.b[(k - 2 * TM) >> 1][k & 1], adB[kh][k & 1] + so + ((k - 2 * TM) >> 1) * 32 * 128);
+    };
+    auto mf = [&](const Frag &f, auto M_) __attribute__((always_inline)) {
+        constexpr int m = decltype(M_)::value, i = m / (3 * TN), j = (m / 3) % TN, pr = m % 3;
+        if constexpr (pr == 0)
+            lo[i][j] = p_mfma(f.a[i][1], f.b[j][0], lo[i][j]);
+        else if constexpr (pr == 1)
+            lo[i][j] = p_mfma(f.a[i][0], f.b[j][1], lo[i][j]);
+        else
+            hi[i][j] = p_mfma(f.a[i][0], f.b[j][0], hi[i][j]);
+    };
+    auto half = [&](const Frag &f, Frag &g, uint32_t so, auto KH, auto READS) __attribute__((always_inline)) {
+        static_for<NM>([&](auto M_) __attribute__((always_inline)) {
+            mf(f, M_);
+            if constexpr (decltype(READS)::value && decltype(M_)::value < NR) rd(g, M_, so, KH);
+        });
+        if constexpr (decltype(READS)::value) {
+            static_for<NR>([&](auto) __attribute__((always_inline)) {
+                __builtin_amdgcn_sched_group_barrier(0x008, 1, 0);
+                __builtin_amdgcn_sched_group_barrier(0x100, 1, 0);
+            });
+            if constexpr (NM > NR) __builtin_amdgcn_sched_group_barrier(0x008, NM - NR, 0);
+        }
+        __builtin_amdgcn_sched_barrier(0);
+    };
+    auto touch = [&](const Frag &f) __attribute__((always_inline)) {
+#pragma unroll
+        for (int i = 0; i < TM; i++) asm volatile("" ::"v"(f.a[i][0]), "v"(f.a[i][1]));
+#pragma unroll
+        for (int j = 0; j < TN; j++) asm volatile("" ::"v"(f.b[j][0]), "v"(f.b[j][1]));
+    };
+    auto publish = [&]() __attribute__((always_inline)) {
+        __builtin_amdgcn_s_barrier();
+        asm volatile("" ::: "memory");
+        __builtin_amdgcn_sched_barrier(0);
+    };
+    auto store_tile = [&](auto FULL) __attribute__((always_inline)) {
+        constexpr bool full = decltype(FULL)::value;
+        const float inv = p_pow2(-eA), invB = p_pow2(-eB);
+        float *Ct = C + cur.t * sC;
+        const int64_t m0 = cur.m0;
+        const int n0 = cur.n0;
+        int64_t N = N_;
+        int rw = wm * WTM + 4 * fh, rp = wm * WTM + 4 * fh;
+        asm volatile("" : "+s"(N), "+v"(rw), "+v"(rp));
+        if constexpr (EPI == 2) {
+            float *part = hpart + ((int64_t)(cur.t * tiles_n + cur.tn) * WGN + wn) * M * 4;
+#pragma unroll
+            for (int i = 0; i < TM; i++) {
+                float pv[64];
+#pragma unroll
+                for (int q = 0; q < 64; q++) pv[q] = 0.0f;
+#pragma unroll
+                for (int j = 0; j < TN; j++) {
+                    const int col = n0 + wn * WTN + j * 32 + fr;
+#pragma unroll
+                    for (int r = 0; r < 16; r++) {
+                        const int64_t row = m0 + rw + i * 32 + (r & 3) + 8 * (r >> 2);
+                        const float x = p_relu((hi[i][j][r] + lo[i][j][r] * P_LO_INV) * inv * invB + bvv[j]);
+                        if (full || row < M) Ct[row * N + col] = x;
+#pragma unroll
+                        for (int o = 0; o < 4; o++) pv[o * 16 + r] += x * wv[o][j];
+                    }
+                }
+#pragma unroll
+                for (int c = 64, off = 16; off >= 1; c >>= 1, off >>= 1) {
+                    const bool up = (fr & off) != 0;
+#pragma unroll
+                    for (int k = 0; k < c / 2; k++) {
+                        const float send = up ? pv[k] : pv[k + c / 2], keep = up ? pv[k + c / 2] : pv[k];
+                        pv[k] = keep + __shfl_xor(send, off);
+                    }
+                }
+                const int o = fr >> 3;
+#pragma unroll
+                for (int k = 0; k < 2; k++) {
+                    const int r = 2 * (fr & 7) + k;
+                    const int64_t row = m0 + rp + i * 32 + (r & 3) + 8 * (r >> 2);
+                    if (full || row < M) part[row * 4 + o] = pv[k];
+                }
+            }
+        } else {
+#pragma unroll
+            for (int j = 0; j < TN; j++) {
+                const int col = n0 + wn * WTN + j * 32 + fr;
+#pragma unroll
+                for (int i = 0; i < TM; i++) {
+#pragma unroll
+                    for (int r = 0; r < 16; r++) {
+                        const int64_t row = m0 + rw + i * 32 + (r & 3) + 8 * (r >> 2);
+                        if (full || row < M)
+                            Ct[row * N + col] = p_relu((hi[i][j][r] + lo[i][j][r] * P_LO_INV) * inv * invB + bvv[j]);
+                    }
+                }
+            }
+        }
+    };
+
+    int cb = 0;
+    issue_map(cur.m0, cb);
+    P_VMCNT(0);
+    publish();
+    set_base(cur);
+    uint32_t g0[GA], g1[GA];
+    read_g(0, g0, cb);
+    issue(IC<0>{}, 0, g0);
+    read_g(1, g1, cb);
+    issue(IC<1>{}, 1, g1);
+    read_g(2, g0, cb);
+    P_VMCNT(G);
+    publish();
+    bool carried = false;
+    for (;;) {
+        const bool more = v + nb < W;
+        const PItem nxt = more ? p_item(v + nb, W, tiles, tiles_n, BM, BN) : cur;
+        Frag f0, f1;
+        static_for<NR>([&](auto K_) __attribute__((always_inline)) { rd(f0, K_, 0, IC<0>{}); });
+        static_for<NK>([&](auto KT) __attribute__((always_inline)) {
+            constexpr int kt = decltype(KT)::value, st = kt % 3, sn = (kt + 1) % 3;
+            uint32_t(&gu)[GA] = (kt % 2 == 0) ? g0 : g1;
+            uint32_t(&gn)[GA] = (kt % 2 == 0) ? g1 : g0;
+            if constexpr (kt == NK - 2) set_base(nxt);
+            issue(IC<(kt + 2) % NK>{}, (kt + 2) % 3, gu);
+            if constexpr (kt == 8) issue_map(nxt.m0, cb ^ 1);
+            __builtin_amdgcn_sched_barrier(0);
+            half(f0, f1, (uint32_t)st * STG_B, IC<1>{}, IC<1>{});
+            touch(f1);
+            if constexpr (kt == 0) {
+                if (carried)
+                    P_VMCNT(CARRY);
+                else
+                    P_VMCNT(G);
+            } else if constexpr (kt == 8 || kt == 9) {
+                P_VMCNT(G + GX);
+            } else {
+                P_VMCNT(G);
+            }
+            publish();
+            read_g((kt + 3) % NK, gn, kt + 3 < NK ? cb : cb ^ 1);
+            if constexpr (kt + 1 < NK)
+                half(f1, f0, (uint32_t)sn * STG_B, IC<0>{}, IC<1>{});
+            else
+                half(f1, f0, 0u, IC<0>{}, IC<0>{});
+        });
+        if (cur.t != lt || cur.n0 != ln) load_consts();
+        carried = cur.m0 + BM <= M;
+        if (carried) {
+            store_tile(IC<1>{});
+        } else {
+            store_tile(IC<0>{});
+            P_VMCNT(0);
+        }
+        zero();
+        if (!more) break;
+        v += nb;
+        cur = nxt;
+        cb ^= 1;
+    }
+    P_VMCNT(0);
+}
+
+template <int BM, int BN, int WGM, int WGN, int EPI, int NK, int NS = 3, bool ONE = false, int ORD = 0,
+          bool PERS = false>
+__global__ __launch_bounds__(64 * WGM * WGN) void k_h3_pq(const p_u32x4 *__restrict__ A, const p_u32x4 *__restrict__ B,
+                                                          const uint32_t *__restrict__ amaxA,
+                                                          const uint32_t *__restrict__ amaxB, int64_t M, int N, int K,
+                                                          int64_t sA, int64_t sB, const float *__restrict__ bias,
+                                                          float *__restrict__ C, int64_t sC, int tiles_n, int tiles,
+                                                          int W) {
+    if constexpr (PERS) {
+        static_assert(NS == 3 && !ONE, "the walk: a 3-stage ring, two accumulators");
+        pq_walk<BM, BN, WGM, WGN, EPI, NK, ORD>(A, B, amaxA, amaxB, M, N, K, sA, sB, bias, C, sC, tiles_n, tiles, W);
+    } else {
+        pq_tile<BM, BN, WGM, WGN, EPI, NK, NS, ONE, ORD>(A, B, amaxA, amaxB, M, N, K, sA, sB, bias, C, sC, tiles_n);
+    }
+}
+
+template <int BM, int BN, int WGM, int WGN, int EPI, bool PERS = false>
+__global__ __launch_bounds__(64 * WGM * WGN) void k_h3_pqg(const p_u32x4 *__restrict__ A, const p_u32x4 *__restrict__ B,
+                                                           const uint32_t *__restrict__ amaxA,
+                                                           const uint32_t *__restrict__ amaxB, int64_t M, int N,
+                                                           int64_t sA, int64_t sB, const float *__restrict__ bias,
+                                                           float *__restrict__ C, int64_t sC, int tiles_n, int tiles,
+                                                           int W, const int32_t *__restrict__ amap,
+                                                           const float *__restrict__ hw0, const float *__restrict__ hw1,
+                                                           int na, float *__restrict__ hpart) {
+    if constexpr (PERS)
+        pqg_walk<BM, BN, WGM, WGN, EPI>(A, B, amaxA, amaxB, M, N, sA, sB, bias, C, sC, tiles_n, tiles, W, amap, hw0,
+                                        hw1, na, hpart);
+    else
+        pqg_tile<BM, BN, WGM, WGN, EPI>(A, B, amaxA, amaxB, M, N, sA, sB, bias, C, sC, tiles_n, amap, hw0, hw1, na,
+                                        hpart);
+}
+
+int g_walk_blocks = 0;
+int walk_blocks(int64_t items) {
+    int n = g_walk_blocks;
+    if (n <= 0) {
+        static int cus[64];
+        int dev = 0;
+        if (hipGetDevice(&dev) != hipSuccess || dev < 0 || dev >= 64) return -1;
+        if (!cus[dev] && hipDeviceGetAttribute(&cus[dev], hipDeviceAttributeMultiprocessorCount, dev) != hipSuccess)
+            return -1;
+        n = cus[dev];
+    }
+    return n <= 0 ? -1 : (int)std::min<int64_t>(n, items);
+}
+
+template <int BM, int BN, int WGM, int WGN, int NS = 3, bool ONE = false, int ORD = 0, bool PERS = false>
+hipError_t pq_launch(const void *A, const void *B, const uint32_t *amaxA, const uint32_t *amaxB, int64_t M, int N,
+                     int K, int T, int64_t sA, int64_t sB, const float *bias, float *C, int64_t sC, hipStream_t s) {
+    if (N % BN || K % 32 || K < 64) return hipErrorInvalidValue;
+    const int64_t tiles_m = (M + BM - 1) / BM;
+    const int tiles_n = N / BN;
+    if (tiles_m * tiles_n * T > INT32_MAX) return hipErrorInvalidValue;
+    const int tiles = (int)(tiles_m * tiles_n), W = tiles * T;
+    dim3 grid((unsigned)tiles, T);
+    const dim3 block(64 * WGM * WGN);
+    if constexpr (PERS) {
+        const int nb = walk_blocks(W);
+        if (nb < 1) return hipErrorInvalidValue;
+        grid = dim3(nb);
+    }
+    const auto *a = static_cast<const p_u32x4 *>(A);
+    const auto *b = static_cast<const p_u32x4 *>(B);
+#define PQ_K(NK)                                                                                                    \
+    do {                                                                                                            \
+        if (bias)                                                                                                   \
+            hipLaunchKernelGGL((k_h3_pq<BM, BN, WGM, WGN, 1, NK, NS, ONE, ORD, PERS>), grid, block, 0, s, a, b, amaxA, \
+                               amaxB, M, N, K, sA / 4, sB / 4, bias, C, sC, tiles_n, tiles, W);                     \
+        else                                                                                                        \
+            hipLaunchKernelGGL((k_h3_pq<BM, BN, WGM, WGN, 0, NK, NS, ONE, ORD, PERS>), grid, block, 0, s, a, b, amaxA, \
+                               amaxB, M, N, K, sA / 4, sB / 4, nullptr, C, sC, tiles_n, tiles, W);                  \
+    } while (0)
+    switch (K) {
+        case 576: PQ_K(18); break;
+        case 512: PQ_K(16); break;
+        default: return hipErrorInvalidValue;
+    }
+#undef PQ_K
+    return hipGetLastError();
+}
+
+
+}
+
+void set_h3p_walk_blocks(int n) { g_walk_blocks = n > 0 ? n : 0; }
+
+constexpr bool H3P_FWD_WALK = true, H3P_DGRAD_WALK = true;
 hipError_t launch_h3p_gemm_nt(const void *A, const uint32_t *amaxA, const void *B, const uint32_t *amaxB, int64_t M,
                               int N, int K, int T, int64_t a_stride, int64_t b_stride, const float *bias, float *C,
                               int64_t c_stride, int cfg, hipStream_t s, const int32_t *a_rows, const float *head_w0,
@@ -716,25 +1316,41 @@
     if (a_stride % 4 || b_stride % 4) return hipErrorInvalidValue;
     if (a_rows) {
         constexpr int BM = 128, BN = 256;
-        if (cfg != 60 || K != 576 || N % BN || !bias || !C) return hipErrorInvalidValue;
+        if ((cfg != 60 && cfg != 75 && cfg != 76) || K != 576 || N % BN || !bias || !C) return hipErrorInvalidValue;
         if (head_part && (T != 2 || n_actions < 1 || n_actions > 4 || !head_w0 || !head_w1)) return hipErrorInvalidValue;
         const int64_t tiles_m = (M + BM - 1) / BM;
         const int tiles_n = N / BN;
-        const dim3 grid((unsigned)(tiles_m * tiles_n), T), block(512);
+        if (tiles_m * tiles_n * T > INT32_MAX) return hipErrorInvalidValue;
+        const int tiles = (int)(tiles_m * tiles_n), W = tiles * T;
+        const bool walk = cfg == 76 || (cfg == 60 && H3P_FWD_WALK);
+        if (walk && (a_stride > (INT64_C(1) << 30) || M * 9 > (INT64_C(1) << 30))) return hipErrorInvalidValue;
+        const int nb = walk ? walk_blocks(W) : 0;
+        if (walk && nb < 1) return hipErrorInvalidValue;
+        const dim3 grid = walk ? dim3(nb) : dim3((unsigned)tiles, T), block(512);
         const auto *a = static_cast<const p_u32x4 *>(A);
         const auto *b = static_cast<const p_u32x4 *>(B);
-        if (head_part)
-            hipLaunchKernelGGL((k_h3_pqg<BM, BN, 2, 4, 2>), grid, block, 0, s, a, b, amaxA, amaxB, M, N, a_stride / 4,
-                               b_stride / 4, bias, C, c_stride, tiles_n, a_rows, head_w0, head_w1, n_actions,
-                               head_part);
+#define PQG(EPI, PERS, ...)                                                                                          \
+    hipLaunchKernelGGL((k_h3_pqg<BM, BN, 2, 4, EPI, PERS>), grid, block, 0, s, a, b, amaxA, amaxB, M, N, a_stride / 4, \
+                       b_stride / 4, bias, C, c_stride, tiles_n, tiles, W, a_rows, __VA_ARGS__)
+        if (head_part && walk)
+            PQG(2, true, head_w0, head_w1, n_actions, head_part);
+        else if (head_part)
+            PQG(2, false, head_w0, head_w1, n_actions, head_part);
+        else if (walk)
+            PQG(1, true, nullptr, nullptr, 0, nullptr);
         else
-            hipLaunchKernelGGL((k_h3_pqg<BM, BN, 2, 4, 1>), grid, block, 0, s, a, b, amaxA, amaxB, M, N, a_stride / 4,
-                               b_stride / 4, bias, C, c_stride, tiles_n, a_rows, nullptr, nullptr, 0, nullptr);
+            PQG(1, false, nullptr, nullptr, 0, nullptr);
+#undef PQG
         return hipGetLastError();
     }
     switch (cfg) {
         case 60: return pq_launch<128, 256, 2, 4>(A, B, amaxA, amaxB, M, N, K, T, a_stride, b_stride, bias, C, c_stride, s);
-        case 62: return pq_launch<128, 192, 4, 2>(A, B, amaxA, amaxB, M, N, K, T, a_stride, b_stride, bias, C, c_stride, s);
+        case 62:
+            if (H3P_DGRAD_WALK)
+                return pq_launch<128, 192, 4, 2, 3, false, 0, true>(A, B, amaxA, amaxB, M, N, K, T, a_stride, b_stride, bias, C, c_stride, s);
+            return pq_launch<128, 192, 4, 2>(A, B, amaxA, amaxB, M, N, K, T, a_stride, b_stride, bias, C, c_stride, s);
+        case 77: return pq_launch<128, 192, 4, 2>(A, B, amaxA, amaxB, M, N, K, T, a_stride, b_stride, bias, C, c_stride, s);
+        case 78: return pq_launch<128, 192, 4, 2, 3, false, 0, true>(A, B, amaxA, amaxB, M, N, K, T, a_stride, b_stride, bias, C, c_stride, s);
         case 63: return pq_launch<128, 192, 4, 2, 4>(A, B, amaxA, amaxB, M, N, K, T, a_stride, b_stride, bias, C, c_stride, s);
         case 65: return pq_launch<256, 192, 4, 2, 2, true>(A, B, amaxA, amaxB, M, N, K, T, a_stride, b_stride, bias, C, c_stride, s);
         case 66: return pq_launch<128, 192, 4, 2, 3, false, 1>(A, B, amaxA, amaxB, M, N, K, T, a_stride, b_stride, bias, C, c_stride, s);
diff --git a/ppo-2dgrid_amd/csrc/merlin_internal.h b/ppo-2dgrid_amd/csrc/merlin_internal.h
--- a/ppo-2dgrid_amd/csrc/merlin_internal.h
+++ b/ppo-2dgrid_amd/csrc/merlin_internal.h
@@ -251,6 +251,7 @@
                               int64_t c_stride, int cfg, hipStream_t s, const int32_t *a_rows = nullptr,
                               const float *head_w0 = nullptr, int n_actions = 0, const float *head_w1 = nullptr,
                               float *head_part = nullptr);
+void set_h3p_walk_blocks(int n);
 hipError_t launch_h3p_gemm_tn_gather(const void *A, const uint32_t *amaxA, const void *B, const uint32_t *amaxB,
                                      int64_t Kd, int M, int N, int T, int64_t a_stride, int64_t b_stride, int splits,
                                      float *slab, const int32_t *b_rows, int cfg, int *S_out, hipStream_t s);
diff --git a/ppo-2dgrid_amd/merlin/_native.py b/ppo-2dgrid_amd/merlin/_native.py
--- a/ppo-2dgrid_amd/merlin/_native.py
+++ b/ppo-2dgrid_amd/merlin/_native.py
@@ -234,6 +234,7 @@
     "merlin_env_set_difficulties", "merlin_episode_class_stats",
     "merlin_frame_atlas", "merlin_render_frames", "merlin_env_render", "merlin_env_snapshot",
     "merlin_shortest_paths", "merlin_env_optimal_steps", "merlin_shortest_paths_host",
+    "merlin_h3_walk_blocks",
 )
 
 
@@ -1212,6 +1213,17 @@
     return out
 
 
+@contextlib.contextmanager
+def h3_walk_blocks(blocks: int):
+    fn = lib().merlin_h3_walk_blocks
+    fn.argtypes, fn.restype = [C.c_int32], C.c_int
+    check(fn(int(blocks)), "merlin_h3_walk_blocks")
+    try:
+        yield
+    finally:
+        check(fn(0), "merlin_h3_walk_blocks")
+
+
 def h3_gemm_nt_planes(Ap: torch.Tensor, amaxA: torch.Tensor, B: torch.Tensor, amaxB: torch.Tensor,
                       bias: torch.Tensor | None = None, cfg: int = 62, out: torch.Tensor | None = None,
                       name: str = "h3_gemm_nt") -> torch.Tensor:
@@ -1235,13 +1247,14 @@
 
 def h3_gemm_nt_heads(A: torch.Tensor, amaxA: torch.Tensor, B: torch.Tensor, amaxB: torch.Tensor, bias: torch.Tensor,
                      Wa: torch.Tensor, Wc: torch.Tensor, cfg: int, rows: torch.Tensor | None = None,
-                     name: str = "h3_gemm_nt", partials_only: bool = False) -> tuple:
+                     name: str = "h3_gemm_nt", partials_only: bool = False, heads: bool = True) -> tuple:
     H3_SPANS.add(name)
     T, M, K = (int(v) for v in A.shape)
     ap = A.dtype == torch.int16
     if ap:
         K //= 2
         assert rows is not None and not partials_only
+    assert heads or ap
     N = int(B.shape[1])
     NA = int(Wa.shape[0])
     assert T == 2 and A.dtype in (torch.float32, torch.int16) and B.dtype == torch.int16 and B.shape == (T, N, 2 * K)
@@ -1252,13 +1265,15 @@
     if rows is not None:
         assert rows.dtype == torch.int32 and rows.is_contiguous() and rows.numel() == M * K // 64
     out = None if partials_only else torch.empty((T, M, N), dtype=torch.float32, device=A.device)
-    part = torch.empty((T, P, M, 4), dtype=torch.float32, device=A.device)
+    part = torch.empty((T, P, M, 4), dtype=torch.float32, device=A.device) if heads else None
     fn = lib().merlin_h3_gemm_nt_heads_planes if ap else lib().merlin_h3_gemm_nt_heads
     with KernelTimer.span(name, 0, 2 * T * M * N * K):
         check(fn(ptr(A), ptr(amaxA), ptr(B), ptr(amaxB), M, N, K, M * K, N * K, ptr(bias), ptr(out), M * N, ptr(rows),
                  ptr(Wa), NA, ptr(Wc), ptr(part), int(cfg), stream_of(A)), "merlin_h3_gemm_nt_heads")
     if partials_only:
         return part
+    if not heads:
+        return out
     logits = torch.empty((M, NA), dtype=torch.float32, device=A.device)
     value = torch.empty(M, dtype=torch.float32, device=A.device)
     with KernelTimer.span("k_heads_fwd", T * P * M * 16 + M * (NA + 1) * 4):
```

Result: faster. 4.847 million (median of 6 runs) (+4.0%).
